# HeewoongNoh/DOSTransformer

Measured on AMD Instinct MI355X. Metric: crystals/sec training throughput (Phonon DOS, hidden=128), higher is better.
Workload: dtype f32; 1 GPU; phonon_h128_b64: phonon DOSTransformer layers=3 transformer=2 hidden=128, 64 crystals/GPU, full train step (fwd+loss+bwd+AdamW), 8 distinct pre-collated HBM-resident batches; global_batch=64, parallelism=dp1, launch=replay

## Files before the change

### dostransformer_amd/_lib.py

```python
from __future__ import annotations

import ctypes as C
import os
from typing import Optional

_HERE = os.path.dirname(os.path.abspath(__file__))


def from_environ(name: str, default: str = "") -> str:
    return os.environ.get(name, default)


LIB_PATH = from_environ("DOSX_LIB") or os.path.join(_HERE, "csrc", "libdosx.so")

c_float_p = C.POINTER(C.c_float)
c_int_p = C.POINTER(C.c_int32)
BIG = 1 << 30


class DosxUnavailable(RuntimeError):
    pass


class DosxError(RuntimeError):
# ... 61 lines not shown
        ("dkv_accumulate", C.c_int32),
        ("partials_q", C.c_void_p), ("partials_kv", C.c_void_p), ("drop_mask", C.c_void_p), ("dkv_part", C.c_void_p), ("dkv_cnt", C.c_void_p),
        ("ln1_gamma", C.c_void_p), ("ln1_beta", C.c_void_p), ("ln1_out", C.c_void_p),
        ("key_ptr", C.c_void_p),
    ]


class FfnBwd(C.Structure):
    _fields_ = [
        ("M", C.c_int32), ("H", C.c_int32),
        ("dy", C.c_void_p), ("lddy", C.c_int32),
        ("h", C.c_void_p), ("ldh", C.c_int32),
        ("x", C.c_void_p), ("ldx", C.c_int32),
        ("stats", C.c_void_p),
        ("gamma", C.c_void_p),
        ("w1", C.c_void_p), ("w2", C.c_void_p),
        ("dh", C.c_void_p), ("lddh", C.c_int32),
        ("dx", C.c_void_p), ("lddx", C.c_int32),
        ("partials", C.c_void_p), ("partial_ld", C.c_int32),
        ("fin_gamma", C.c_void_p), ("fin_xhat", C.c_void_p), ("fin_rstd", C.c_void_p),
        ("fin_dy", C.c_void_p),
        ("fin_ddos", C.c_void_p), ("fin_w", C.c_void_p), ("fin_beta", C.c_void_p),
        ("fin_S", C.c_int32), ("fin_Bq", C.c_int32),
        ("att_x", C.c_void_p), ("att_ldxin", C.c_int32),
        ("att_kvhat", C.c_void_p), ("att_gamma0", C.c_void_p), ("att_beta0", C.c_void_p),
        ("att_probs", C.c_void_p), ("att_qstats", C.c_void_p), ("att_mask", C.c_void_p),
        ("att_dxin", C.c_void_p), ("att_lddxin", C.c_int32),
        ("att_partials_q", C.c_void_p), ("att_partials_kv", C.c_void_p), ("att_dkv_part", C.c_void_p), ("att_dkv_cnt", C.c_void_p),
        ("att_dkvhat", C.c_void_p), ("att_dkv_accumulate", C.c_int32),
        ("att_Nk", C.c_int32), ("att_Bk", C.c_int32), ("att_Bq", C.c_int32), ("att_Sq", C.c_int32), ("att_qs", C.c_int32), ("att_qb", C.c_int32),
        ("att_key_ptr", C.c_void_p),
    ]


class Ffn(C.Structure):
    _fields_ = [
        ("M", C.c_int32), ("H", C.c_int32),
        ("x", C.c_void_p), ("ldx", C.c_int32),
        ("stats", C.c_void_p),
        ("gamma", C.c_void_p), ("beta", C.c_void_p),
        ("w1", C.c_void_p), ("b1", C.c_void_p),
        ("w2", C.c_void_p), ("b2", C.c_void_p),
        ("h", C.c_void_p), ("ldh", C.c_int32),
        ("out", C.c_void_p), ("ldo", C.c_int32),
        ("fin_gamma", C.c_void_p), ("fin_beta", C.c_void_p),
        ("fin_xhat", C.c_void_p), ("fin_rstd", C.c_void_p),
        ("fin_w", C.c_void_p), ("fin_b", C.c_void_p), ("fin_dos", C.c_void_p),
        ("fin_S", C.c_int32), ("fin_Bq", C.c_int32),
        ("att_kvhat", C.c_void_p), ("att_gamma0", C.c_void_p), ("att_beta0", C.c_void_p), ("att_mask", C.c_void_p),
        ("att_probs", C.c_void_p), ("att_qstats", C.c_void_p), ("att_x1", C.c_void_p), ("att_st1", C.c_void_p),
        ("att_Nk", C.c_int32), ("att_Bk", C.c_int32), ("att_Bq", C.c_int32), ("att_Sq", C.c_int32),
        ("att_qs", C.c_int32), ("att_qb", C.c_int32), ("att_ldx1", C.c_int32), ("att_aligned", C.c_int32),
        ("att_key_ptr", C.c_void_p),
    ]


class MlpLn(C.Structure):
    _fields_ = [
        ("M", C.c_int32), ("K", C.c_int32), ("NH", C.c_int32), ("NO", C.c_int32), ("k0", C.c_int32),
        ("a0", C.c_void_p), ("lda0", C.c_int32),
        ("a1", C.c_void_p), ("lda1", C.c_int32),
        ("w1", C.c_void_p), ("b1", C.c_void_p),
        ("gamma", C.c_void_p), ("beta", C.c_void_p),
        ("alpha", C.c_void_p),
        ("w2", C.c_void_p), ("b2", C.c_void_p),
        ("res", C.c_void_p), ("ldres", C.c_int32),
        ("xhat", C.c_void_p), ("rstd", C.c_void_p),
        ("out", C.c_void_p), ("ldo", C.c_int32),
        ("w3", C.c_void_p), ("ldw3", C.c_int32), ("n3", C.c_int32), ("nb3", C.c_int32),
        ("pq", C.c_void_p), ("ldpq", C.c_int32),
        ("cs_buf", C.c_void_p), ("cs_cnt", C.c_void_p),
    ]


class MlpLnBwd(C.Structure):
    _fields_ = [
        ("M", C.c_int32), ("K", C.c_int32), ("NH", C.c_int32), ("NO", C.c_int32),
        ("dy", C.c_void_p), ("lddy", C.c_int32),
        ("xhat", C.c_void_p), ("rstd", C.c_void_p),
        ("w1", C.c_void_p), ("w2", C.c_void_p),
        ("gamma", C.c_void_p), ("beta", C.c_void_p), ("alpha", C.c_void_p),
        ("dz", C.c_void_p),
        ("dcat", C.c_void_p), ("lddcat", C.c_int32),
        ("partials", C.c_void_p), ("partial_ld", C.c_int32), ("add_dy", C.c_int32),
        ("cs_buf", C.c_void_p), ("cs_cnt", C.c_void_p),
        ("pre", C.c_int32), ("pre_dy", C.c_void_p),
        ("pre_dz", C.c_void_p), ("pre_rowptr_src", C.c_void_p), ("pre_perm_src", C.c_void_p), ("pre_aggd", C.c_void_p),
        ("pre_w", C.c_void_p), ("pre_ldw", C.c_int32),
        ("pre_res", C.c_void_p), ("pre_ldres", C.c_int32), ("pre_res2", C.c_void_p), ("pre_ldres2", C.c_int32),
        ("pre_aggs", C.c_void_p),
        ("pre_dkv", C.c_void_p), ("pre_kvhat", C.c_void_p), ("pre_rstd_nodes", C.c_void_p), ("pre_dense_row", C.c_void_p),
        ("pre_dpool", C.c_void_p), ("pre_ld_dpool", C.c_int32), ("pre_node_graph", C.c_void_p), ("pre_num_graphs", C.c_int32),
        ("pre_ghost_row", C.c_int32),
    ]


class EncCs(C.Structure):
    _fields_ = [
        ("M", C.c_int32), ("Fa", C.c_int32), ("H", C.c_int32),
        ("x", C.c_void_p), ("ldx", C.c_int32),
        ("w0", C.c_void_p), ("ldw0", C.c_int32), ("b0", C.c_void_p),
        ("alpha", C.c_void_p),
        ("w2", C.c_void_p), ("b2", C.c_void_p),
        ("z", C.c_void_p), ("out", C.c_void_p), ("ldo", C.c_int32),
        ("w3", C.c_void_p), ("ldw3", C.c_int32), ("n3", C.c_int32), ("nb3", C.c_int32),
        ("pq", C.c_void_p), ("ldpq", C.c_int32),
# ... 139 lines not shown
    "dosx_gemm_kernel_name": [C.POINTER(Gemm), C.c_char_p, _I],
    "dosx_wgrad_splits": [_I, _I, _I],
    "dosx_wgrad_tiles": [_I, _I],
    "dosx_wgrad_scratch_floats": [_I, _I, _I],
    "dosx_wgrad": [C.POINTER(Wgrad), _P],
    "dosx_grad_flush": [C.POINTER(Wgrad), _I, C.POINTER(ReduceJob), _I, _P],
    "dosx_wgrad_grouped": [C.POINTER(Wgrad), _I, _P],
    "dosx_reduce_partials": [C.POINTER(ReduceJob), _I, _P],
    "dosx_edge_feat_sh1": [_P, _P, _I, _F, _P],
    "dosx_edge_embed_sh1": [_P, _P, _P, _P, _P, _I, _I, _F, _P],
    "dosx_segment_reduce": [_P, _P, _P, _P, _P, _P, _I, _I, _I, _P],
    "dosx_segment_reduce_perm": [_P, _P, _P, _P, _I, _I, _I, _P],
    "dosx_edge_grad_combine": [_P, _I, _P, _I, _P, _P, _P, _I, _I, _P],
    "dosx_gather_bwd": [_P, _P, _I, _P, _P, _P, _P, _P, _P, _P, _I, _I, _I, _P],
    "dosx_graph_pool": [_P, _P, _P, _I, _I, _I, _P],
    "dosx_graph_pool_bwd": [_P, _I, _P, _P, _I, _I, _I, _I, _P],
    "dosx_dense_normalize": [_P, _P, _P, _P, _I, _I, _I, _P],
    "dosx_dense_normalize_slots": [_P, _P, _P, _P, _I, _I, _I, _P],
    "dosx_dense_normalize_bwd": [_P, _P, _P, _P, _P, _I, _I, _I, _I, _P],
    "dosx_dense_normalize_pool_bwd": [_P, _P, _P, _P, _P, _I, _P, _I, _P, _I, _I, _I, _I, _P],
    "dosx_dense_slots": [_P, _P, _P, _I, _I, _I, _P],
    "dosx_dense_slots_bwd": [_P, _P, _P, _I, _I, _I, _I, _P],
    "dosx_ln_prelu_bwd": [_P, _P, _P, _P, _P, _P, _P, _P, _I, _I, _P],
    "dosx_ln_prelu_bwd_gather": [_P, _P, _P, _P, _P, _P, _P, _P, _P, _P, _I, _I, _P],
    "dosx_act_segment_sum": [_P, _P, _P, _P, _P, _P, _P, _P, _P, _I, _I, _I, _P],
    "dosx_seg_count_scale": [_P, _I, _P, _I, _P, _I, _I, _P],
    "dosx_gather_add_rownorm": [_P, _P, _I, _P, _I, _P, _P, _P, _P, _I, _I, _P],
    "dosx_rownorm": [_P, _P, _P, _I, _I, _P],
    "dosx_rownorm_bwd": [_P, _P, _P, _P, _I, _I, _I, _P],
    "dosx_mask_residual": [_P, _I, _P, _P, _I, _P, _I, _P, _I, _I, _P],
    "dosx_rownorm_bwd_act": [_P, _P, _P, _P, _P, _F, _P, _I, _I, _P],
    "dosx_layernorm": [_P, _P, _P, _P, _P, _P, _I, _I, _P],
    "dosx_layernorm_bwd": [_P, _P, _P, _P, _P, _P, _I, _I, _P],
    "dosx_attention_pkv_supported": [_I, _I],
    "dosx_attention_aligned_mode": [_I],
    "dosx_attention_fwd": [C.POINTER(Attn), _P],
    "dosx_attention_bwd": [C.POINTER(Attn), _P],
    "dosx_attn_pv": [_P, _P, _P, _P, _I, _I, _I, _I, _I, _P],
    "dosx_attn_tv": [_P, _P, _P, _P, _I, _I, _I, _I, _I, _I, _P],
    "dosx_attn_dp": [_P, _P, _P, _I, _I, _I, _I, _I, _P],
    "dosx_softmax_bwd": [_P, _P, _P, _P, _L, _I, _F, _P],
    "dosx_softmax_fwd": [_P, _P, _L, _I, _F, _P],
    "dosx_ln_rowdot": [_P, _P, _P, _P, _P, _P, _P, _P, _I, _I, _I, _P],
    "dosx_ln_rowdot_bwd": [_P, _P, _P, _P, _P, _P, _P, _P, _I, _I, _I, _P],
    "dosx_rowdot": [_P, _P, _P, _P, _I, _I, _I, _P],
    "dosx_rowdot_bwd": [_P, _P, _P, _P, _P, _I, _I, _I, _P],
    "dosx_sse2": [_P, _P, _P, _P, _I, _P],
    "dosx_loss_phonon_bwd": [_P, _P, _P, _P, _F, _D, _P, _P, _P, _I, _P],
    "dosx_loss_phonon": [_P, _P, _P, _P, _F, _P, _P, _P, _I, _P],
    "dosx_loss_edos": [_P, _P, _P, _F, _I, _I, _I, _P, _P, _P, _P],
    "dosx_sum": [_P, _I, _P, _P],
    "dosx_adamw": [_P, _P, _P, _P, _L, _F, _F, _F, _F, _F, _I, _F, _P],
    "dosx_ffn_supported": [_I],
    "dosx_ffn_att_supported": [_I, _I],
    "dosx_ffn_att_aligned_supported": [_I, _I],
    "dosx_ffn_fwd": [C.POINTER(Ffn), _P],
    "dosx_ffn_fwd_multi": [C.POINTER(Ffn), _I, _P],
    "dosx_ffn_bwd_partial_rows": [_I],
    "dosx_ffn_att_bwd_supported": [_I, _I, _I, _I],
    "dosx_ffn_att_bwd_partial_rows": [_I, _I],
    "dosx_ffn_att_aligned_rows": [_I, _I],
    "dosx_ffn_bwd": [C.POINTER(FfnBwd), _P],
    "dosx_mlp_ln_supported": [_I, _I, _I],
    "dosx_mlp_ln_cs_supported": [_I, _I, _I],
    "dosx_mlp_ln_cs_tiles": [_I],
    "dosx_mlp_ln_cs_scratch_floats": [_I, _I],
    "dosx_mlp_ln_fwd": [C.POINTER(MlpLn), _P],
    "dosx_mlp_ln_bwd_partial_rows": [_I],
    "dosx_mlp_ln_bwd": [C.POINTER(MlpLnBwd), _P],
    "dosx_enc_cs_supported": [_I, _I],
    "dosx_enc_cs_fwd": [C.POINTER(EncCs), _P],
    "dosx_edge_enc_supported": [_I],
    "dosx_edge_enc_fwd": [C.POINTER(EdgeEnc), _P],
    "dosx_heads_bwd_supported": [_I],
    "dosx_heads_bwd": [C.POINTER(HeadsBwd), _P],
    "dosx_gemm_bf16x3_supported": [_I, _I, _I],
    "dosx_gemm_bf16x3": [_P, _I, _P, _I, _I, _P, _P, _I, _I, _I, _I, _I, _P, _I, _P, _I, _P],
    "dosx_edge_mlp_supported": [_I],
    "dosx_edge_mlp_fwd": [C.POINTER(EdgeMlp), _P],
    "dosx_edge_mlp_bwd": [C.POINTER(EdgeMlpBwd), _P],
    "dosx_node_grad": [C.POINTER(NodeGrad), _P],
    "dosx_csr_workspace_bytes": [_I, C.POINTER(C.c_size_t)],
    "dosx_csr_build": [_P, _P, _I, _I, _I, _P, _P, _P, _P, _P, _P, _P, _P, _P, _P, _P, _P, C.c_size_t, _P],
    "dosx_collate": [_P] * 5 + [_I] * 3 + [_P] * 18 + [_P],
    "dosx_collate_padded": [C.POINTER(Collate), _P],
    "dosx_collate_padded_f64": [C.POINTER(Collate), _P],
    "dosx_neighbor_count": [_P, _P, _P, _P, _I, _L, _D, _I, _I, _P, _P],
    "dosx_neighbor_fill": [_P, _P, _P, _P, _I, _L, _D, _I, _I, _P, _P, _P, _P, _P, _P, _P],
    "dosx_knn_graph": [C.POINTER(Knn), _P],
    "dosx_replay_op": [C.c_char_p, C.POINTER(C.c_int), C.POINTER(C.c_int)],
    "dosx_replay": [C.POINTER(Call), _I, C.POINTER(C.c_int)],
    "dosx_replay_timed": [C.POINTER(Call), _I, C.POINTER(C.c_float), C.POINTER(C.c_int)],
    "dosx_dropout_mask": [_P, _L, _F, _P, _L, _P],
    "dosx_copy_many": [C.POINTER(CopyJob), _I, _P],
    "dosx_fill": [_P, _F, _L, _P],
    "dosx_embed_rows": [_P, _P, _P, _I, _I, _P],
    "dosx_embed_rows_bwd": [_P, _I, _P, _P, _I, _I, _I, _P],
    "dosx_reduce_rows": [_P, _I, _P, _I, _I, _I, _I, _I, _I, _I, _P],
    "dosx_act_bwd": [_P, _P, _F, _P, _L, _P],
    "dosx_gemm_f64": [C.POINTER(Gemm64), _P],
    "dosx_wgrad_f64": [C.POINTER(Wgrad64), _P],
    "dosx_colsum_f64": [_P, _I, _I, _I, _P, _P, _I, _P],
    "dosx_layernorm_f64": [_P, _P, _P, _P, _P, _P, _P, _I, _I, _P],
    "dosx_layernorm_bwd_f64": [_P, _P, _P, _P, _P, _P, _P, _P, _I, _I, _P],
    "dosx_act_bwd_f64": [_P, _P, _I, _I, _P, _P, _P, _I, _I, _P],
    "dosx_edge_feat_sh1_f64": [_P, _P, _I, _D, _P],
# ... 63 lines not shown
```

### dostransformer_amd/_models.py

```python
from __future__ import annotations

from typing import Optional, Tuple

import torch

from . import functional as Fn
from . import functional64 as F64
from ._fused import FusedModel, is_dead_param
from ._lib import DosxError


_SEED_MOD = 2 ** 62


def rank_seed_offset() -> int:
    import torch.distributed as td
    if td.is_available() and td.is_initialized():
        return (0x9E3779B97F4A7C15 * (td.get_rank() + 1)) % _SEED_MOD
    return 0


def dos_device(P):
    return P["embeddings.weight"].device

# ... 28 lines not shown
                            f"Predictor(model, per_crystal_keys=True) and Trainer(model, per_crystal_keys=True)")
        object.__setattr__(self, "_per_crystal_keys", bool(flag))
        return self

    def _check_f64_program(self) -> None:
        name = type(self).__name__
        if self._cfg.kind != "phonon":
            raise DosxError(f"{name}: only DOSTransformer_phonon has a float64 program (the eDOS reference trains in fp32)")
        dts = {p.dtype for n, p in self.named_parameters() if not is_dead_param(n)}
        if dts != {torch.float64}:
            raise DosxError(f"{name}: the float64 program needs every live parameter float64 (.double()), got "
                            f"{sorted(str(d) for d in dts)}")
        if self._cfg.H > F64.MAX_HIDDEN:
            raise DosxError(f"{name}: the float64 program takes hidden <= {F64.MAX_HIDDEN}, got {self._cfg.H}")

    def _flat_dtype(self, g=None) -> torch.dtype:
        if self._program_dtype != torch.float64:
            return torch.float32
        self._check_f64_program()
        return torch.float64

    def _wanted_flat_dtype(self):
        return self._program_dtype

    def _require_fp32_program(self, who: str) -> None:
        if self._program_dtype == torch.float64:
            raise DosxError(f"{who} runs the fp32 program; {type(self).__name__} is set to float64 (set_program_dtype): train "
                            f"it with train64.Trainer64, or with model(batch), loss.backward() and torch.optim.AdamW")

    def _require_f64_program(self, who: str) -> None:
        ours = isinstance(self, DOSTransformerBase)
        if not (ours and self._cfg.kind == "phonon" and self._program_dtype == torch.float64):
            raise DosxError(f"{who} drives a DOSTransformer_phonon set to the float64 program "
                            f"(model.double().set_program_dtype(torch.float64)), got {type(self).__name__}"
                            + (f" with program_dtype {self._program_dtype}" if ours else "")
                            + ": the fp32 program is train.Trainer's / predict.Predictor's")

    def _check_train_flags(self):
        pass

    def _dropout(self, device, bump: bool):
        p = float(getattr(self, "_attn_drop", 0.0) or 0.0)
        if not self.training or p <= 0.0:
            return None
        seed = getattr(self, "_drop_seed", None)
        if seed is None or seed.device != device:
            val = (int(torch.randint(0, _SEED_MOD, (1,), dtype=torch.int64).item()) + rank_seed_offset()) % _SEED_MOD
            seed = torch.tensor([val], dtype=torch.int64).to(device)
            object.__setattr__(self, "_drop_seed", seed)
        elif bump:
            seed.add_(1)
        return p, seed

    def _program_fwd(self, P, g, m, bump_seed: bool = True, per_crystal_keys: bool = False):
        if P["embeddings.weight"].dtype == torch.float64:
            dos, xL, ctx = F64.dostransformer_phonon_fwd(P, self._cfg, g, m, drop=self._dropout(dos_device(P), bump_seed),
                                                         per_crystal_keys=self._per_crystal_keys)
            B = m.num_graphs
            return dos[:B], xL, dos[B:], (ctx, dos)
        dos, xL, ctx = Fn.dostransformer_fwd(P, self._cfg, g, m, drop=self._dropout(dos_device(P), bump_seed),
                                             per_crystal_keys=per_crystal_keys)
        B = m.num_graphs
        return dos[:B], xL, dos[B:], (ctx, dos)

    def _program_bwd(self, P, G, m, saved, grads, sink):
        ctx, dos = saved
        dg, dx, ds = grads
        B = m.num_graphs
        ddos = torch.zeros_like(dos)
        if dg is not None:
            ddos[:B].copy_(dg)
        if ds is not None:
            ddos[B:].copy_(ds)
        if dos.dtype == torch.float64:
            F64.dostransformer_phonon_bwd(P, G, self._cfg, m, ctx, ddos, dx)
            return
        Fn.dostransformer_bwd(P, G, self._cfg, m, ctx, ddos, None if dx is None else dx.float().contiguous(), sink)

    def forward(self, g):
        self._check_train_flags()
        return self._run(g)


class GraphnetworkBase(FusedModel):
    _cfg: Fn.ModelCfg
    _returns_x: bool
    _has_f64_program = True

    def _extra_dead(self, g) -> Tuple[str, ...]:
        expected = 118 if self._cfg.kind == "phonon" else 200
        width = g.x.shape[1] if g is not None else expected
        unused = "GN_encoder.node_encoder_prompt" if width == expected else "GN_encoder.node_encoder"
        return tuple(f"{unused}.{s}" for s in ("0.weight", "0.bias", "1.weight", "2.weight", "2.bias"))

    def _program_fwd(self, P, g, m):
        if P["embeddings.weight"].dtype == torch.float64:
            dos, ctx = F64.graphnetwork_phonon_fwd(P, self._cfg, g, m)
            return dos, ctx
        dos, xL, ctx = Fn.graphnetwork_fwd(P, self._cfg, g, m)
        return (dos, xL, ctx) if self._returns_x else (dos, ctx)

    def _program_bwd(self, P, G, m, saved, grads, sink):
        ddos = grads[0]
        if P["embeddings.weight"].dtype == torch.float64:
            if ddos is None:
                ddos = torch.zeros(m.num_graphs, self._cfg.S, device=P["embeddings.weight"].device, dtype=torch.float64)
            F64.graphnetwork_phonon_bwd(P, G, self._cfg, m, saved, ddos)
            return
        dx = grads[1] if self._returns_x else None
        if ddos is None:
            ddos = torch.zeros(m.num_graphs, self._cfg.S, device=P["embeddings.weight"].device)
        Fn.graphnetwork_bwd(P, G, self._cfg, m, saved, ddos.float().contiguous(),
                            None if dx is None else dx.float().contiguous(), sink)

# ... 4 lines not shown
```

### dostransformer_amd/csrc/common.h

```cpp
#pragma once
#include <hip/hip_runtime.h>
#include <stdint.h>
#include <stdio.h>

#include "../../include/dosx.h"

typedef float f32x16 __attribute__((ext_vector_type(16)));
typedef float f32x4 __attribute__((ext_vector_type(4)));

#define DOSX_WAVE 64

#ifndef DOSX_MAIN_PRIO
#define DOSX_MAIN_PRIO 0
#endif
#define DOSX_SET_MAIN_PRIO() do { if (DOSX_MAIN_PRIO) __builtin_amdgcn_s_setprio(DOSX_MAIN_PRIO); } while (0)

void dosx_set_error(const char* fmt, ...);

#define DOSX_CHECK_ARG(cond, ...)   \
  do {                              \
    if (!(cond)) {                  \
      dosx_set_error(__VA_ARGS__);  \
      return -22;                   \
    }                               \
// ... 65 lines not shown
  __device__ __forceinline__ explicit UDiv(int d_) : d(d_), sh((d_ & (d_ - 1)) == 0 ? __builtin_ctz(d_) : -1) {}
  __device__ __forceinline__ int div(int x) const { return sh >= 0 ? (x >> sh) : x / d; }
};

__device__ __forceinline__ float4 ld4(const float* p) { return *reinterpret_cast<const float4*>(p); }
__device__ __forceinline__ void st4(float* p, float4 v) { *reinterpret_cast<float4*>(p) = v; }
__device__ __forceinline__ float4 f4zero() { return make_float4(0.f, 0.f, 0.f, 0.f); }
__device__ __forceinline__ float4 f4add(float4 a, float4 b) {
  return make_float4(a.x + b.x, a.y + b.y, a.z + b.z, a.w + b.w);
}
__device__ __forceinline__ float f4get(const float4& v, int i) {
  return i == 0 ? v.x : i == 1 ? v.y : i == 2 ? v.z : v.w;
}

template <bool KP>
__device__ __forceinline__ int dosx_live_keys(const int32_t* key_ptr, int bk, int Nk) {
  if constexpr (KP) return min(max(key_ptr[bk + 1] - key_ptr[bk], 0), Nk);
  else return Nk;
}
template <bool KP>
__device__ __forceinline__ int dosx_live_keys_fwd(const int32_t* key_ptr, int bk, int Nk) {
  if constexpr (KP) return min(max(key_ptr[bk + 1] - key_ptr[bk], 0), Nk);
  else return key_ptr ? min(key_ptr[bk + 1] - key_ptr[bk], Nk) : Nk;
}
template <bool KP>
__device__ __forceinline__ float dosx_key_entry(const float* base, size_t row0, int j, int nk, int Nk, float other) {
  if constexpr (KP) return j < nk ? base[row0 + j] : other;
  else return base[row0 + (j < Nk ? j : 0)];
}
template <bool KP>
__device__ __forceinline__ float dosx_softmax_inv(float s) {
  if constexpr (KP) return s > 0.f ? 1.f / s : 0.f;
  else return 1.f / s;
}
template <bool KP, int SH>
__device__ __forceinline__ int dosx_live_tiles(int nk, int all) {
  if constexpr (KP) return (nk + (1 << SH) - 1) >> SH;
  else return all;
}
template <bool KP>
__device__ __forceinline__ float dosx_psum_one(int nk) {
  if constexpr (KP) return nk > 0 ? 1.f : 0.f;
  else return 1.f;
}

#define DOSX_LN_EPS 1e-5f

#ifndef DOSX_TICKET_ORDER
#define DOSX_TICKET_ORDER __ATOMIC_RELAXED
#endif
__device__ __forceinline__ int dosx_ticket(int* counter) {
  return __hip_atomic_fetch_add(counter, 1, DOSX_TICKET_ORDER, __HIP_MEMORY_SCOPE_AGENT);
}
```

### dostransformer_amd/csrc/ffn.hip

```cpp
#include <stdlib.h>

#include "common.h"
#include "mma16.h"

typedef int v4i32 __attribute__((ext_vector_type(4)));

#ifdef DOSX_STAMPS
__device__ unsigned long long dosx_ffn_stamp_buf[64];
extern "C" int dosx_debug_read_ffn_stamps(unsigned long long* host64) {
  return (int)hipMemcpyFromSymbol(host64, HIP_SYMBOL(dosx_ffn_stamp_buf), sizeof(unsigned long long) * 64);
}
#define FSTAMP(slot) do { if (threadIdx.x == 0 && blockIdx.x == 0) dosx_ffn_stamp_buf[(slot)] = __builtin_amdgcn_s_memtime(); } while (0)
#define FSTAMP_S(slot) do { if (threadIdx.x == 256 && blockIdx.x == 0) dosx_ffn_stamp_buf[32 + (slot)] = __builtin_amdgcn_s_memtime(); } while (0)
#else
#define FSTAMP(slot) do { } while (0)
#define FSTAMP_S(slot) do { } while (0)
#endif

namespace {

constexpr int FBN = 128;

template <bool KP>
__device__ __forceinline__ void ffn_att_row(const DosxFfn& a, float* __restrict__ Xs, const int LDX, const int lr, const int m0,
// ... 249 lines not shown
  FSTAMP(13);
  __syncthreads();
  {
    const int nct = H >> 4, njobs = (R / 16) * nct;
    const UDiv dnct(nct);
    for (int job = wave; job < njobs; job += 8) {
      const int rt = dnct.div(job), ct = job - rt * nct;
      const f32x4 acc = mma_kn<4>(Sc + (16 * rt + l15) * 68 + 4 * g4, Ks + (4 * g4) * LDK + 16 * ct + l15, LDK, nctL);
#pragma unroll
      for (int i = 0; i < 4; ++i) Qs[(16 * rt + 4 * g4 + i) * LDK + 16 * ct + l15] = acc[i];
    }
  }
  FSTAMP(14);
  __syncthreads();
  FSTAMP(15);
  if (rowok) {
    float4 x1[2];
    float t = 0.f;
#pragma unroll
    for (int k = 0; k < 2; ++k) {
      const int c = q16 * 4 + 64 * k;
      x1[k] = f4zero();
      if (!on[k]) continue;
      const float4 o = ld4(Qs + lr * LDK + c);
      x1[k] = make_float4(o.x * g0[k].x + b0[k].x * psum + xr[k].x, o.y * g0[k].y + b0[k].y * psum + xr[k].y,
                          o.z * g0[k].z + b0[k].z * psum + xr[k].z, o.w * g0[k].w + b0[k].w * psum + xr[k].w);
      if (rv) st4(a.att_x1 + (size_t)r * a.att_ldx1 + c, x1[k]);
      t += (x1[k].x + x1[k].y) + (x1[k].z + x1[k].w);
    }
    const float mean1 = row16_sum(t) * invH;
    t = 0.f;
#pragma unroll
    for (int k = 0; k < 2; ++k) {
      if (!on[k]) continue;
      const float p0 = x1[k].x - mean1, p1 = x1[k].y - mean1, p2 = x1[k].z - mean1, p3 = x1[k].w - mean1;
      t += (p0 * p0 + p1 * p1) + (p2 * p2 + p3 * p3);
    }
    const float rstd1 = rsqrtf(row16_sum(t) * invH + DOSX_LN_EPS);
    if (rv && q16 == 0) {
      a.att_qstats[2 * (size_t)r] = mean; a.att_qstats[2 * (size_t)r + 1] = rstd;
      a.att_st1[2 * (size_t)r] = mean1;   a.att_st1[2 * (size_t)r + 1] = rstd1;
    }
#pragma unroll
    for (int k = 0; k < 2; ++k) {
      if (!on[k]) continue;
      const float4 vv = x1[k];
      st4(Xs + lr * LDX + q16 * 4 + 64 * k,
          make_float4((vv.x - mean1) * rstd1 * g1[k].x + bb1[k].x, (vv.y - mean1) * rstd1 * g1[k].y + bb1[k].y,
                      (vv.z - mean1) * rstd1 * g1[k].z + bb1[k].z, (vv.w - mean1) * rstd1 * g1[k].w + bb1[k].w));
    }
  }
}

template <bool HALF, int KB, int ATTK>
__device__ __forceinline__ void ffn_fwd_body(const DosxFfn& a, float* __restrict__ sm) {
  constexpr int ATT = ATTK >= 3 ? ATTK - 2 : ATTK;
  constexpr bool KP = ATTK >= 3;
  constexpr int FBK = KB, FLDW = KB + 4;
  constexpr int R = HALF ? 16 : 32;
  constexpr int ER = R / 8;
  const int H = a.H, H4 = 4 * a.H, M = a.M;
  const int LDX = H + 4, LDT = H4 + 4;
  float* Xs = sm;
  float* T = Xs + R * LDX;
  float* ST = T + R * LDT;
  constexpr int STG = FBN * FLDW;
  const int tid = threadIdx.x, lane = tid & 63, wave = tid >> 6, l31 = lane & 31, hh = lane >> 5;
  const int l15 = lane & 15, g4 = lane >> 4;
  const int wave_u = __builtin_amdgcn_readfirstlane(wave);
  const int m0 = blockIdx.x * R;
  int al_bq = 0, al_s0 = 0;
  if constexpr (ATT == 2) {
    const int tpc = (a.att_Sq + R - 1) / R;
    al_bq = (int)blockIdx.x / tpc;
    al_s0 = ((int)blockIdx.x % tpc) * R;
  }
  auto grow = [&](const int lr) -> int {
    if constexpr (ATT == 2) {
      const int s = al_s0 + lr;
      return s < a.att_Sq ? s * a.att_Bq + al_bq : -1;
    } else {
      const int r = m0 + lr;
      return r < M ? r : -1;
    }
  };
  auto growc = [&](const int lr) -> int {
    const int r = grow(lr);
    return r >= 0 ? r : grow(0);
  };
  FSTAMP(0);
  const int nk1 = H / FBK, nb1 = H4 / FBN, n1 = nb1 * nk1, n2 = H4 / FBK, nch = n1 + n2;

  const int c0 = lane * 4;
  const bool con = c0 < H;
  float4 xres[ER], bias2 = f4zero();
  if (con) bias2 = ld4(a.b2 + c0);
  if constexpr (ATT == 0) {
#pragma unroll
    for (int i = 0; i < ER; ++i) {
      const int r = growc(wave * ER + i);
      xres[i] = ld4(a.x + (size_t)r * a.ldx + (con ? c0 : 0));
    }
  }
  if constexpr (ATT == 2) {
  }
  float* const attKs = ST;
  float* const attSc = ST + ((a.att_Nk + 15) & ~15) * (H + 4);
// ... 191 lines not shown
    FSTAMP(4);
    float* Cs = ST;
    const int col = wave * 32 + l31;
#pragma unroll
    for (int r = 0; r < 16; ++r) Cs[((r & 3) + 8 * (r >> 2) + 4 * hh) * (FBN + 4) + col] = acc[r];
    }
  }
  __syncthreads();
  FSTAMP(5);
  if constexpr (ATT != 0) {
#pragma unroll
    for (int i = 0; i < ER; ++i) {
      const int r = growc(wave * ER + i);
      xres[i] = ld4(a.att_x1 + (size_t)r * a.att_ldx1 + (con ? c0 : 0));
    }
  }
  {
    const float* Cs = ST;
    const bool fin = a.fin_gamma != nullptr;
    const bool fdot = fin && a.fin_dos != nullptr;
    float4 fg = f4zero(), fb = f4zero(), fw = f4zero();
    if (fin && con) { fg = ld4(a.fin_gamma + c0); fb = ld4(a.fin_beta + c0); }
    if (fdot && con) fw = ld4(a.fin_w + c0);
    const float fbias = fdot ? a.fin_b[0] : 0.f;
    const float invH = 1.f / (float)H;
#pragma unroll
    for (int i = 0; i < ER; ++i) {
      const int lr = wave * ER + i, r = grow(lr);
      const bool ok = con && r >= 0;
      float4 o = f4zero();
      if (ok) {
        const float4 v = ld4(Cs + lr * (FBN + 4) + c0);
        o = make_float4(v.x + bias2.x + xres[i].x, v.y + bias2.y + xres[i].y, v.z + bias2.z + xres[i].z,
                        v.w + bias2.w + xres[i].w);
      }
      if (!fin) {
        if (ok) st4(a.out + (size_t)r * a.ldo + c0, o);
        continue;
      }
      const float mean = wave_sum(o.x + o.y + o.z + o.w) * invH;
      const float4 d = ok ? make_float4(o.x - mean, o.y - mean, o.z - mean, o.w - mean) : f4zero();
      const float rstd = rsqrtf(wave_sum(d.x * d.x + d.y * d.y + d.z * d.z + d.w * d.w) * invH + DOSX_LN_EPS);
      float dot = 0.f;
      if (ok) {
        const float4 xh = make_float4(d.x * rstd, d.y * rstd, d.z * rstd, d.w * rstd);
        const float4 y = make_float4(xh.x * fg.x + fb.x, xh.y * fg.y + fb.y, xh.z * fg.z + fb.z, xh.w * fg.w + fb.w);
        st4(a.fin_xhat + (size_t)r * H + c0, xh);
        if (a.out) st4(a.out + (size_t)r * a.ldo + c0, y);
        if (lane == 0) a.fin_rstd[r] = rstd;
        dot = y.x * fw.x + y.y * fw.y + y.z * fw.z + y.w * fw.w;
      }
      if (fdot) {
        dot = wave_sum(dot);
        if (lane == 0 && r >= 0) a.fin_dos[(size_t)(r % a.fin_Bq) * a.fin_S + (r / a.fin_Bq)] = dot + fbias;
      }
    }
  }
  FSTAMP(6);
}

template <bool HALF, int KB, int ATT>
__global__ __launch_bounds__(512) void ffn_fwd_kernel(const DosxFfn a) {
  DOSX_SET_MAIN_PRIO();
  extern __shared__ __align__(16) float sm[];
  ffn_fwd_body<HALF, KB, ATT>(a, sm);
}

constexpr int FFN_MULTI_MAX = 2;
struct FfnMulti {
  DosxFfn d[FFN_MULTI_MAX];
  int n;
};
template <bool HALF, int KB, int ATT>
__global__ __launch_bounds__(512) void ffn_fwd_multi_kernel(const FfnMulti A) {
  DOSX_SET_MAIN_PRIO();
  extern __shared__ __align__(16) float sm[];
  ffn_fwd_body<HALF, KB, ATT>(A.d[0], sm);
  asm volatile("s_waitcnt vmcnt(0)" ::: "memory");
  __syncthreads();
  ffn_fwd_body<HALF, KB, ATT>(A.d[1], sm);
}


struct AttBwdSm {
  float *Os, *Ds, *Ql, *Sp, *Ks, *Sc, *Ss, *Ps2, *Pp;
};

template <bool KP>
__device__ __forceinline__ void ffn_dkv_reduce(const DosxFfnBwd& a, const int nqt, const int bk, float* __restrict__ Pp, const int tid) {
  const int lane = tid & 63, q16 = lane & 15, slot = tid >> 4;
  const int H = a.H, Nk = a.att_Nk, rep = a.att_Bq / a.att_Bk, ngroups = (Nk + 15) / 16;
  const int nk = dosx_live_keys<KP>(a.att_key_ptr, bk, Nk);
  const int np = (KP && slot >= nk) ? 0 : rep * nqt;
  const UDiv dnqt(nqt);
  const size_t pstride = (size_t)Nk * H;
  const __amdgpu_buffer_rsrc_t rP = __builtin_amdgcn_make_buffer_rsrc((void*)a.att_dkv_part, 0, 0x7fffffff, 0x00020000);
  float4 g0[2], d[2][2], kh[2][2], d0[2][2];
  bool jv[2];
  size_t krow[2];
#pragma unroll
  for (int k = 0; k < 2; ++k) g0[k] = ld4(a.att_gamma0 + ((q16 * 4 + 64 * k) < H ? (q16 * 4 + 64 * k) : 0));
#pragma unroll
  for (int p = 0; p < 2; ++p) {
    const int j = slot + 32 * p;
    jv[p] = j < nk;
    krow[p] = ((size_t)(jv[p] ? j : 0) * a.att_Bk + bk) * H;
#pragma unroll
    for (int k = 0; k < 2; ++k) {
      const int c = q16 * 4 + 64 * k, cc = c < H ? c : 0;
      kh[p][k] = (!KP || jv[p]) ? ld4(a.att_kvhat + krow[p] + cc) : f4zero();
      d0[p][k] = (a.att_dkv_accumulate && (!KP || jv[p])) ? ld4(a.att_dkvhat + krow[p] + cc) : f4zero();
      d[p][k] = f4zero();
    }
  }
  for (int p0 = 0; p0 < np; p0 += 4) {
    float4 v[2][4][2];
#pragma unroll
    for (int p = 0; p < 2; ++p)
#pragma unroll
      for (int u = 0; u < 4; ++u) {
        const int pi = min(p0 + u, np - 1), i = dnqt.div(pi), t = pi - i * nqt;
        const size_t off = ((size_t)(bk + i * a.att_Bk) * nqt + t) * pstride + (size_t)(jv[p] ? slot + 32 * p : 0) * H;
#pragma unroll
        for (int k = 0; k < 2; ++k) {
          const int c = q16 * 4 + 64 * k;
          v[p][u][k] = (KP && !jv[p]) ? f4zero()
                                      : __builtin_bit_cast(float4, __builtin_amdgcn_raw_buffer_load_b128(rP, (uint32_t)((off + (c < H ? c : 0)) * 4), 0, 16));
        }
      }
#pragma unroll
    for (int p = 0; p < 2; ++p)
#pragma unroll
      for (int u = 0; u < 4; ++u)
// ... 608 lines not shown
      float s = 0.f;
#pragma unroll
      for (int w = 0; w < 8; ++w) s += Ps[(w * npv + which) * FBN + col];
      prow[which * H + col] = s;
    }
    if (fdot && tid == 0) {
      float s = 0.f;
#pragma unroll
      for (int w = 0; w < 8; ++w) s += Ps[8 * 5 * FBN + w];
      prow[5 * H] = s;
    }
  }
  if constexpr (ATT == 2) {
    __syncthreads();
    AttBwdSm L;
    const int LDK = H + 4, NkP = (a.att_Nk + 15) & ~15;
    L.Os = sm;
    L.Ds = sm + R * LDK;
    L.Ql = L.Ds + R * LDK;
    L.Sc = L.Ql + R * LDK;
    L.Ss = L.Sc + R * 68;
    L.Ps2 = L.Ss + R * 68;
    L.Sp = L.Ps2 + R * 68;
    L.Ks = L.Sp + 3 * R * 68;
    L.Pp = L.Sp;
    (void)NkP;
    FSTAMP(16);
    ffn_att_bwd_tile<R, KP>(a, sm, L, attq, al_s0, al_bq, al_tile, al_tpc, tid);
    FSTAMP(29);
  }
}

}

static size_t ffn_att_bwd_floats(int H, int Nk, int R) {
  const size_t LDK = (size_t)H + 4, NkP = (size_t)((Nk + 15) & ~15);
  const size_t tiles = 3 * R * LDK + 6 * (size_t)R * 68 + NkP * LDK;
  const size_t pp = 3 * R * LDK + 3 * (size_t)R * 68 + 32 * 256;
  const size_t red = 64 * 256;
  size_t m = tiles > pp ? tiles : pp;
  return m > red ? m : red;
}

static int ffn_bwd_att_rows(int Sq, int Bq);

static int ffn_chunk(int H) {
  static int forced = -1;
  if (forced < 0) { const char* e = getenv("DOSX_FFN_KB"); forced = e ? atoi(e) : 0; }
  if (forced == 32) return 32;
  return (H % 64) == 0 ? 64 : 32;
}

extern "C" int dosx_ffn_supported(int H) { return (H % 32) == 0 && H >= 32 && H <= 128; }
extern "C" int dosx_ffn_att_supported(int H, int Nk) { return dosx_ffn_supported(H) && Nk >= 1 && Nk <= 16; }
extern "C" int dosx_ffn_att_aligned_supported(int H, int Nk) {
  if (!dosx_ffn_supported(H) || Nk < 1 || Nk > 64) return 0;
  const int kb = ffn_chunk(H);
  return (size_t)((Nk + 15) & ~15) * (H + 4) + 32 * 68 <= 2 * (size_t)128 * (kb + 4);
}

struct FfnPlan { bool half; int kb, mode, grid; size_t smem; };
static int ffn_fwd_prepare(const DosxFfn& a, FfnPlan& pl) {
  DOSX_CHECK_ARG(dosx_ffn_supported(a.H), "dosx_ffn_fwd: H=%d unsupported (multiple of 32, <= 128)", a.H);
  const bool att = a.att_kvhat != nullptr;
  DOSX_CHECK_ARG(a.x && (a.stats || att) && a.gamma && a.beta && a.w1 && a.b1 && a.w2 && a.b2 && a.h && (a.out || a.fin_dos), "dosx_ffn_fwd: null operand");
  if (att)
    DOSX_CHECK_ARG((a.att_aligned ? dosx_ffn_att_aligned_supported(a.H, a.att_Nk) : dosx_ffn_att_supported(a.H, a.att_Nk)) && a.att_gamma0 && a.att_beta0 && a.att_probs && a.att_qstats && a.att_x1 &&
                       a.att_st1 && a.att_Bk > 0 && a.att_Bq > 0 && a.att_Bq % a.att_Bk == 0 && a.att_Sq > 0 &&
                       a.att_Sq * a.att_Bq == a.M && (a.att_ldx1 & 3) == 0 && a.att_ldx1 >= a.H && a.att_qs >= 0 && a.att_qb >= 0,
                   "dosx_ffn_fwd: fused attention needs <= 16 keys, gamma0 / beta0 / probs / qstats / x1 / st1 and Sq * Bq == M");
  if (a.fin_dos) DOSX_CHECK_ARG(a.fin_gamma && a.fin_w && a.fin_b && a.fin_S > 0 && a.fin_Bq > 0 && a.fin_S * a.fin_Bq == a.M,
                                "dosx_ffn_fwd: output-layer epilogue needs the final LayerNorm, w, b and S * Bq == M");
  DOSX_CHECK_ARG((a.ldx & 3) == 0 && (a.ldh & 3) == 0 && (a.ldo & 3) == 0, "dosx_ffn_fwd: leading dimensions must be multiples of 4");
  if (a.fin_gamma) DOSX_CHECK_ARG(a.fin_beta && a.fin_xhat && a.fin_rstd, "dosx_ffn_fwd: final LayerNorm needs beta / xhat / rstd");
  const long long span = (const char*)a.w1 > (const char*)a.w2 ? (const char*)a.w1 - (const char*)a.w2 : (const char*)a.w2 - (const char*)a.w1;
  DOSX_CHECK_ARG(span + (long long)16 * a.H * a.H < 0x7fffffffLL, "dosx_ffn_fwd: fc1 / fc2 weights more than 2 GiB apart");
  const int H = a.H, H4 = 4 * H;
  static int half_max = -1;
  if (half_max < 0) { const char* e = getenv("DOSX_FFN_HALF_MAX"); half_max = e ? atoi(e) : 128; }
  const bool aligned = att && a.att_aligned != 0;
  pl.half = aligned ? ffn_bwd_att_rows(a.att_Sq, a.att_Bq) == 16 : ceil_div(a.M, 32) <= half_max;
  const int R = pl.half ? 16 : 32;
  pl.kb = ffn_chunk(H);
  pl.mode = aligned ? 2 : (att ? 1 : 0);
  if (att && a.att_key_ptr) pl.mode += 2;
  pl.smem = sizeof(float) * ((size_t)R * (H + 4) + (size_t)R * (H4 + 4) + 2 * (size_t)FBN * (pl.kb + 4));
  if (aligned)
    DOSX_CHECK_ARG(a.att_Nk <= 64 && ((size_t)((a.att_Nk + 15) & ~15) * (H + 4) + (size_t)R * 68) <= 2 * (size_t)FBN * (pl.kb + 4),
                   "dosx_ffn_fwd: crystal-aligned attention needs <= 64 keys that fit the stage buffers (Nk=%d, H=%d)", a.att_Nk, H);
  pl.grid = aligned ? a.att_Bq * ceil_div(a.att_Sq, R) : ceil_div(a.M, R);
  static bool attr_set = false;
  if (!attr_set) {
#define DOSX_FFN_ATTR(HALF_, KB_, ATT_) \
    (void)hipFuncSetAttribute(reinterpret_cast<const void*>(&ffn_fwd_kernel<HALF_, KB_, ATT_>), hipFuncAttributeMaxDynamicSharedMemorySize, 160 * 1024)
#define DOSX_FFN_ATTR2(HALF_, KB_, ATT_) \
    (void)hipFuncSetAttribute(reinterpret_cast<const void*>(&ffn_fwd_multi_kernel<HALF_, KB_, ATT_>), hipFuncAttributeMaxDynamicSharedMemorySize, 160 * 1024)
    DOSX_FFN_ATTR(false, 32, 0); DOSX_FFN_ATTR(true, 32, 0); DOSX_FFN_ATTR(false, 64, 0); DOSX_FFN_ATTR(true, 64, 0);
    DOSX_FFN_ATTR(false, 32, 1); DOSX_FFN_ATTR(true, 32, 1); DOSX_FFN_ATTR(false, 64, 1); DOSX_FFN_ATTR(true, 64, 1);
    DOSX_FFN_ATTR(false, 32, 2); DOSX_FFN_ATTR(true, 32, 2); DOSX_FFN_ATTR(false, 64, 2); DOSX_FFN_ATTR(true, 64, 2);
    DOSX_FFN_ATTR2(false, 32, 1); DOSX_FFN_ATTR2(true, 32, 1); DOSX_FFN_ATTR2(false, 64, 1); DOSX_FFN_ATTR2(true, 64, 1);
    DOSX_FFN_ATTR2(false, 32, 2); DOSX_FFN_ATTR2(true, 32, 2); DOSX_FFN_ATTR2(false, 64, 2); DOSX_FFN_ATTR2(true, 64, 2);
    DOSX_FFN_ATTR(false, 32, 3); DOSX_FFN_ATTR(true, 32, 3); DOSX_FFN_ATTR(false, 64, 3); DOSX_FFN_ATTR(true, 64, 3);
    DOSX_FFN_ATTR(false, 32, 4); DOSX_FFN_ATTR(true, 32, 4); DOSX_FFN_ATTR(false, 64, 4); DOSX_FFN_ATTR(true, 64, 4);
    DOSX_FFN_ATTR2(false, 32, 3); DOSX_FFN_ATTR2(true, 32, 3); DOSX_FFN_ATTR2(false, 64, 3); DOSX_FFN_ATTR2(true, 64, 3);
    DOSX_FFN_ATTR2(false, 32, 4); DOSX_FFN_ATTR2(true, 32, 4); DOSX_FFN_ATTR2(false, 64, 4); DOSX_FFN_ATTR2(true, 64, 4);
#undef DOSX_FFN_ATTR
#undef DOSX_FFN_ATTR2
    attr_set = true;
  }
  return 0;
}

#define DOSX_FFN_DISPATCH(KERNEL, ARG)                                                                                    \
  do {                                                                                                                     \
    const dim3 grid_(pl.grid);                                                                                             \
    hipStream_t st_ = to_stream(stream);                                                                                   \
    if (pl.half && pl.kb == 64) { if (pl.mode == 4) hipLaunchKernelGGL((KERNEL<true, 64, 4>), grid_, dim3(512), pl.smem, st_, ARG); else if (pl.mode == 3) hipLaunchKernelGGL((KERNEL<true, 64, 3>), grid_, dim3(512), pl.smem, st_, ARG); else if (pl.mode == 2) hipLaunchKernelGGL((KERNEL<true, 64, 2>), grid_, dim3(512), pl.smem, st_, ARG); else if (pl.mode == 1) hipLaunchKernelGGL((KERNEL<true, 64, 1>), grid_, dim3(512), pl.smem, st_, ARG); else hipLaunchKernelGGL((KERNEL<true, 64, 0>), grid_, dim3(512), pl.smem, st_, ARG); } \
    else if (pl.half) { if (pl.mode == 4) hipLaunchKernelGGL((KERNEL<true, 32, 4>), grid_, dim3(512), pl.smem, st_, ARG); else if (pl.mode == 3) hipLaunchKernelGGL((KERNEL<true, 32, 3>), grid_, dim3(512), pl.smem, st_, ARG); else if (pl.mode == 2) hipLaunchKernelGGL((KERNEL<true, 32, 2>), grid_, dim3(512), pl.smem, st_, ARG); else if (pl.mode == 1) hipLaunchKernelGGL((KERNEL<true, 32, 1>), grid_, dim3(512), pl.smem, st_, ARG); else hipLaunchKernelGGL((KERNEL<true, 32, 0>), grid_, dim3(512), pl.smem, st_, ARG); } \
    else if (pl.kb == 64) { if (pl.mode == 4) hipLaunchKernelGGL((KERNEL<false, 64, 4>), grid_, dim3(512), pl.smem, st_, ARG); else if (pl.mode == 3) hipLaunchKernelGGL((KERNEL<false, 64, 3>), grid_, dim3(512), pl.smem, st_, ARG); else if (pl.mode == 2) hipLaunchKernelGGL((KERNEL<false, 64, 2>), grid_, dim3(512), pl.smem, st_, ARG); else if (pl.mode == 1) hipLaunchKernelGGL((KERNEL<false, 64, 1>), grid_, dim3(512), pl.smem, st_, ARG); else hipLaunchKernelGGL((KERNEL<false, 64, 0>), grid_, dim3(512), pl.smem, st_, ARG); } \
    else { if (pl.mode == 4) hipLaunchKernelGGL((KERNEL<false, 32, 4>), grid_, dim3(512), pl.smem, st_, ARG); else if (pl.mode == 3) hipLaunchKernelGGL((KERNEL<false, 32, 3>), grid_, dim3(512), pl.smem, st_, ARG); else if (pl.mode == 2) hipLaunchKernelGGL((KERNEL<false, 32, 2>), grid_, dim3(512), pl.smem, st_, ARG); else if (pl.mode == 1) hipLaunchKernelGGL((KERNEL<false, 32, 1>), grid_, dim3(512), pl.smem, st_, ARG); else hipLaunchKernelGGL((KERNEL<false, 32, 0>), grid_, dim3(512), pl.smem, st_, ARG); } \
  } while (0)

extern "C" int dosx_ffn_fwd(const DosxFfn* ap, dosx_stream_t stream) {
  DOSX_CHECK_ARG(ap != nullptr, "dosx_ffn_fwd: null descriptor");
  const DosxFfn& a = *ap;
  if (a.M <= 0) return 0;
  FfnPlan pl;
  if (int rc = ffn_fwd_prepare(a, pl)) return rc;
  DOSX_FFN_DISPATCH(ffn_fwd_kernel, a);
  DOSX_LAUNCH_CHECK();
  return 0;
}

extern "C" int dosx_ffn_fwd_multi(const DosxFfn* descs, int n, dosx_stream_t stream) {
  DOSX_CHECK_ARG(descs != nullptr && n >= 1 && n <= FFN_MULTI_MAX, "dosx_ffn_fwd_multi: 1 .. %d layers per launch", FFN_MULTI_MAX);
  if (descs[0].M <= 0) return 0;
  if (n == 1) return dosx_ffn_fwd(descs, stream);
  FfnMulti A;
  A.n = n;
  FfnPlan pl;
  for (int l = 0; l < n; ++l) {
    FfnPlan p2;
    if (int rc = ffn_fwd_prepare(descs[l], p2)) return rc;
    if (l == 0) pl = p2;
    DOSX_CHECK_ARG(p2.half == pl.half && p2.kb == pl.kb && p2.mode == pl.mode && p2.grid == pl.grid && p2.smem == pl.smem && descs[l].M == descs[0].M,
                   "dosx_ffn_fwd_multi: layer %d has another launch plan than layer 0", l);
    DOSX_CHECK_ARG(p2.mode != 0, "dosx_ffn_fwd_multi: every layer must carry its attention half (row-local layers only)");
    if (l > 0) {
      const DosxFfn& p = descs[l - 1];
      const DosxFfn& c = descs[l];
      DOSX_CHECK_ARG(p.out != nullptr && c.x == p.out && c.ldx == p.ldo && c.att_qs == c.att_Bq && c.att_qb == 1,
                     "dosx_ffn_fwd_multi: layer %d must read layer %d's output rows (dense query rows)", l, l - 1);
    }
    A.d[l] = descs[l];
  }
  {
    const dim3 grid_(pl.grid);
    hipStream_t st_ = to_stream(stream);
#define DOSX_FFN_GO2(HALF_, KB_) \
    do { if (pl.mode == 4) hipLaunchKernelGGL((ffn_fwd_multi_kernel<HALF_, KB_, 4>), grid_, dim3(512), pl.smem, st_, A); \
         else if (pl.mode == 3) hipLaunchKernelGGL((ffn_fwd_multi_kernel<HALF_, KB_, 3>), grid_, dim3(512), pl.smem, st_, A); \
         else if (pl.mode == 2) hipLaunchKernelGGL((ffn_fwd_multi_kernel<HALF_, KB_, 2>), grid_, dim3(512), pl.smem, st_, A); \
         else hipLaunchKernelGGL((ffn_fwd_multi_kernel<HALF_, KB_, 1>), grid_, dim3(512), pl.smem, st_, A); } while (0)
    if (pl.half && pl.kb == 64) DOSX_FFN_GO2(true, 64);
    else if (pl.half) DOSX_FFN_GO2(true, 32);
    else if (pl.kb == 64) DOSX_FFN_GO2(false, 64);
    else DOSX_FFN_GO2(false, 32);
#undef DOSX_FFN_GO2
  }
  DOSX_LAUNCH_CHECK();
  return 0;
}

static int ffn_bwd_half(int M) {
  static int half_max = -1;
  if (half_max < 0) { const char* e = getenv("DOSX_FFN_HALF_MAX"); half_max = e ? atoi(e) : 128; }
  return ceil_div(M, 32) <= half_max;
}

extern "C" int dosx_ffn_bwd_partial_rows(int M) { return M <= 0 ? 0 : ceil_div(M, ffn_bwd_half(M) ? 16 : 32); }

static int ffn_bwd_att_rows(int Sq, int Bq) {
  static int half_max = -1;
  if (half_max < 0) { const char* e = getenv("DOSX_FFN_HALF_MAX"); half_max = e ? atoi(e) : 128; }
  return Bq * ceil_div(Sq, 32) <= half_max ? 16 : 32;
}
extern "C" int dosx_ffn_att_bwd_supported(int H, int Nk, int Sq, int Bq) {
  if (!dosx_ffn_supported(H) || ffn_chunk(H) != 64 || Nk < 1 || Nk > 64 || Sq < 1 || Bq < 1) return 0;
  const int R = ffn_bwd_att_rows(Sq, Bq);
  const size_t ffn = (size_t)R * (H + 4) + (size_t)R * (4 * H + 4) + 2 * (size_t)64 * (FBN + 4);
  const size_t att = ffn_att_bwd_floats(H, Nk, R);
  return (ffn > att ? ffn : att) * sizeof(float) <= 160 * 1024;
}
extern "C" int dosx_ffn_att_bwd_partial_rows(int Sq, int Bq) { return Bq * ceil_div(Sq, ffn_bwd_att_rows(Sq, Bq)); }
extern "C" int dosx_ffn_att_aligned_rows(int Sq, int Bq) { return (Sq < 1 || Bq < 1) ? 0 : ffn_bwd_att_rows(Sq, Bq); }

extern "C" int dosx_ffn_bwd(const DosxFfnBwd* ap, dosx_stream_t stream) {
  DOSX_CHECK_ARG(ap != nullptr, "dosx_ffn_bwd: null descriptor");
  const DosxFfnBwd& a = *ap;
  if (a.M <= 0) return 0;
  DOSX_CHECK_ARG(dosx_ffn_supported(a.H), "dosx_ffn_bwd: H=%d unsupported (multiple of 32, <= 128)", a.H);
  DOSX_CHECK_ARG((a.dy || a.fin_ddos) && a.h && a.x && a.stats && a.gamma && a.w1 && a.w2 && a.dh && (a.dx || a.att_kvhat) && a.partials, "dosx_ffn_bwd: null operand");
  DOSX_CHECK_ARG((a.lddy & 3) == 0 && (a.ldh & 3) == 0 && (a.ldx & 3) == 0 && (a.lddh & 3) == 0 && (a.lddx & 3) == 0,
                 "dosx_ffn_bwd: leading dimensions must be multiples of 4");
  const int npv = a.fin_gamma ? (a.fin_ddos ? 5 : 4) : 2;
  DOSX_CHECK_ARG(a.partial_ld >= npv * a.H + (a.fin_ddos ? 1 : 0), "dosx_ffn_bwd: partial_ld %d too small for %d column groups", a.partial_ld, npv);
  if (a.fin_gamma) DOSX_CHECK_ARG(a.fin_xhat && a.fin_rstd && a.fin_dy, "dosx_ffn_bwd: final LayerNorm backward needs xhat / rstd / fin_dy");
  if (a.fin_ddos) DOSX_CHECK_ARG(a.fin_gamma && a.fin_beta && a.fin_w && a.fin_S > 0 && a.fin_Bq > 0 && a.fin_S * a.fin_Bq == a.M,
                                 "dosx_ffn_bwd: output-layer backward needs gamma / beta / w and S * Bq == M");
  const long long span = (const char*)a.w1 > (const char*)a.w2 ? (const char*)a.w1 - (const char*)a.w2 : (const char*)a.w2 - (const char*)a.w1;
  DOSX_CHECK_ARG(span + (long long)16 * a.H * a.H < 0x7fffffffLL, "dosx_ffn_bwd: fc1 / fc2 weights more than 2 GiB apart");
  const int H = a.H, H4 = 4 * H;
  const bool att = a.att_kvhat != nullptr;
  if (att) {
    DOSX_CHECK_ARG(dosx_ffn_att_bwd_supported(H, a.att_Nk, a.att_Sq, a.att_Bq) && ffn_chunk(H) == 64, "dosx_ffn_bwd: fused attention backward unsupported for H=%d Nk=%d", H, a.att_Nk);
    DOSX_CHECK_ARG(a.att_x && a.att_gamma0 && a.att_beta0 && a.att_probs && a.att_qstats && a.att_dxin && a.att_partials_q && a.att_partials_kv &&
                       a.att_dkv_part && a.att_dkv_cnt && a.att_dkvhat && a.att_Bk > 0 && a.att_Bq % a.att_Bk == 0 && a.att_Sq * a.att_Bq == a.M &&
// ... 34 lines not shown
```

### dostransformer_amd/csrc/replay_thunks.inc

```

static int thunk_dosx_set_sliver_max_gf(const DosxCall& c) { return dosx_set_sliver_max_gf((double)c.farg[0]); }
static int thunk_dosx_gemm_partial_rows(const DosxCall& c) { return dosx_gemm_partial_rows((int)c.iarg[0], (int)c.iarg[1], (int)c.iarg[2]); }
static int thunk_dosx_gemm(const DosxCall& c) { return dosx_gemm((const DosxGemm*)(uintptr_t)c.iarg[0], (dosx_stream_t)(uintptr_t)c.iarg[1]); }
static int thunk_dosx_gemm_pair(const DosxCall& c) { return dosx_gemm_pair((const DosxGemm*)(uintptr_t)c.iarg[0], (const DosxGemm*)(uintptr_t)c.iarg[1], (dosx_stream_t)(uintptr_t)c.iarg[2]); }
static int thunk_dosx_gemm_kernel_name(const DosxCall& c) { return dosx_gemm_kernel_name((const DosxGemm*)(uintptr_t)c.iarg[0], (char*)(uintptr_t)c.iarg[1], (int)c.iarg[2]); }
static int thunk_dosx_wgrad_splits(const DosxCall& c) { return dosx_wgrad_splits((int)c.iarg[0], (int)c.iarg[1], (int)c.iarg[2]); }
static int thunk_dosx_wgrad_tiles(const DosxCall& c) { return dosx_wgrad_tiles((int)c.iarg[0], (int)c.iarg[1]); }
static int thunk_dosx_wgrad(const DosxCall& c) { return dosx_wgrad((const DosxWgrad*)(uintptr_t)c.iarg[0], (dosx_stream_t)(uintptr_t)c.iarg[1]); }
static int thunk_dosx_wgrad_grouped(const DosxCall& c) { return dosx_wgrad_grouped((const DosxWgrad*)(uintptr_t)c.iarg[0], (int)c.iarg[1], (dosx_stream_t)(uintptr_t)c.iarg[2]); }
static int thunk_dosx_reduce_partials(const DosxCall& c) { return dosx_reduce_partials((const DosxReduceJob*)(uintptr_t)c.iarg[0], (int)c.iarg[1], (dosx_stream_t)(uintptr_t)c.iarg[2]); }
static int thunk_dosx_grad_flush(const DosxCall& c) { return dosx_grad_flush((const DosxWgrad*)(uintptr_t)c.iarg[0], (int)c.iarg[1], (const DosxReduceJob*)(uintptr_t)c.iarg[2], (int)c.iarg[3], (dosx_stream_t)(uintptr_t)c.iarg[4]); }
static int thunk_dosx_edge_feat_sh1(const DosxCall& c) { return dosx_edge_feat_sh1((const float*)(uintptr_t)c.iarg[0], (float*)(uintptr_t)c.iarg[1], (int)c.iarg[2], (float)c.farg[0], (dosx_stream_t)(uintptr_t)c.iarg[3]); }
static int thunk_dosx_edge_embed_sh1(const DosxCall& c) { return dosx_edge_embed_sh1((const float*)(uintptr_t)c.iarg[0], (const float*)(uintptr_t)c.iarg[1], (const float*)(uintptr_t)c.iarg[2], (float*)(uintptr_t)c.iarg[3], (float*)(uintptr_t)c.iarg[4], (int)c.iarg[5], (int)c.iarg[6], (float)c.farg[0], (dosx_stream_t)(uintptr_t)c.iarg[7]); }
static int thunk_dosx_segment_reduce(const DosxCall& c) { return dosx_segment_reduce((const float*)(uintptr_t)c.iarg[0], (const int32_t*)(uintptr_t)c.iarg[1], (const float*)(uintptr_t)c.iarg[2], (float*)(uintptr_t)c.iarg[3], (const float*)(uintptr_t)c.iarg[4], (float*)(uintptr_t)c.iarg[5], (int)c.iarg[6], (int)c.iarg[7], (int)c.iarg[8], (dosx_stream_t)(uintptr_t)c.iarg[9]); }
static int thunk_dosx_segment_reduce_perm(const DosxCall& c) { return dosx_segment_reduce_perm((const float*)(uintptr_t)c.iarg[0], (const int32_t*)(uintptr_t)c.iarg[1], (const int32_t*)(uintptr_t)c.iarg[2], (float*)(uintptr_t)c.iarg[3], (int)c.iarg[4], (int)c.iarg[5], (int)c.iarg[6], (dosx_stream_t)(uintptr_t)c.iarg[7]); }
static int thunk_dosx_act_segment_sum(const DosxCall& c) { return dosx_act_segment_sum((const float*)(uintptr_t)c.iarg[0], (const int32_t*)(uintptr_t)c.iarg[1], (const float*)(uintptr_t)c.iarg[2], (const float*)(uintptr_t)c.iarg[3], (const float*)(uintptr_t)c.iarg[4], (const float*)(uintptr_t)c.iarg[5], (const float*)(uintptr_t)c.iarg[6], (float*)(uintptr_t)c.iarg[7], (float*)(uintptr_t)c.iarg[8], (int)c.iarg[9], (int)c.iarg[10], (int)c.iarg[11], (dosx_stream_t)(uintptr_t)c.iarg[12]); }
static int thunk_dosx_seg_count_scale(const DosxCall& c) { return dosx_seg_count_scale((const float*)(uintptr_t)c.iarg[0], (int)c.iarg[1], (const int32_t*)(uintptr_t)c.iarg[2], (int)c.iarg[3], (float*)(uintptr_t)c.iarg[4], (int)c.iarg[5], (int)c.iarg[6], (dosx_stream_t)(uintptr_t)c.iarg[7]); }
static int thunk_dosx_edge_grad_combine(const DosxCall& c) { return dosx_edge_grad_combine((const float*)(uintptr_t)c.iarg[0], (int)c.iarg[1], (const float*)(uintptr_t)c.iarg[2], (int)c.iarg[3], (const int32_t*)(uintptr_t)c.iarg[4], (const float*)(uintptr_t)c.iarg[5], (float*)(uintptr_t)c.iarg[6], (int)c.iarg[7], (int)c.iarg[8], (dosx_stream_t)(uintptr_t)c.iarg[9]); }
static int thunk_dosx_gather_bwd(const DosxCall& c) { return dosx_gather_bwd((const float*)(uintptr_t)c.iarg[0], (const float*)(uintptr_t)c.iarg[1], (int)c.iarg[2], (const float*)(uintptr_t)c.iarg[3], (const int32_t*)(uintptr_t)c.iarg[4], (const int32_t*)(uintptr_t)c.iarg[5], (const int32_t*)(uintptr_t)c.iarg[6], (const float*)(uintptr_t)c.iarg[7], (float*)(uintptr_t)c.iarg[8], (float*)(uintptr_t)c.iarg[9], (int)c.iarg[10], (int)c.iarg[11], (int)c.iarg[12], (dosx_stream_t)(uintptr_t)c.iarg[13]); }
static int thunk_dosx_graph_pool(const DosxCall& c) { return dosx_graph_pool((const float*)(uintptr_t)c.iarg[0], (const int32_t*)(uintptr_t)c.iarg[1], (float*)(uintptr_t)c.iarg[2], (int)c.iarg[3], (int)c.iarg[4], (int)c.iarg[5], (dosx_stream_t)(uintptr_t)c.iarg[6]); }
static int thunk_dosx_graph_pool_bwd(const DosxCall& c) { return dosx_graph_pool_bwd((const float*)(uintptr_t)c.iarg[0], (int)c.iarg[1], (const int32_t*)(uintptr_t)c.iarg[2], (float*)(uintptr_t)c.iarg[3], (int)c.iarg[4], (int)c.iarg[5], (int)c.iarg[6], (int)c.iarg[7], (dosx_stream_t)(uintptr_t)c.iarg[8]); }
static int thunk_dosx_dense_normalize(const DosxCall& c) { return dosx_dense_normalize((const float*)(uintptr_t)c.iarg[0], (const int32_t*)(uintptr_t)c.iarg[1], (float*)(uintptr_t)c.iarg[2], (float*)(uintptr_t)c.iarg[3], (int)c.iarg[4], (int)c.iarg[5], (int)c.iarg[6], (dosx_stream_t)(uintptr_t)c.iarg[7]); }
static int thunk_dosx_dense_normalize_slots(const DosxCall& c) { return dosx_dense_normalize_slots((const float*)(uintptr_t)c.iarg[0], (const int32_t*)(uintptr_t)c.iarg[1], (float*)(uintptr_t)c.iarg[2], (float*)(uintptr_t)c.iarg[3], (int)c.iarg[4], (int)c.iarg[5], (int)c.iarg[6], (dosx_stream_t)(uintptr_t)c.iarg[7]); }
static int thunk_dosx_dense_normalize_bwd(const DosxCall& c) { return dosx_dense_normalize_bwd((const float*)(uintptr_t)c.iarg[0], (const float*)(uintptr_t)c.iarg[1], (const float*)(uintptr_t)c.iarg[2], (const int32_t*)(uintptr_t)c.iarg[3], (float*)(uintptr_t)c.iarg[4], (int)c.iarg[5], (int)c.iarg[6], (int)c.iarg[7], (int)c.iarg[8], (dosx_stream_t)(uintptr_t)c.iarg[9]); }
static int thunk_dosx_dense_normalize_pool_bwd(const DosxCall& c) { return dosx_dense_normalize_pool_bwd((const float*)(uintptr_t)c.iarg[0], (const float*)(uintptr_t)c.iarg[1], (const float*)(uintptr_t)c.iarg[2], (const int32_t*)(uintptr_t)c.iarg[3], (const float*)(uintptr_t)c.iarg[4], (int)c.iarg[5], (const int32_t*)(uintptr_t)c.iarg[6], (int)c.iarg[7], (float*)(uintptr_t)c.iarg[8], (int)c.iarg[9], (int)c.iarg[10], (int)c.iarg[11], (int)c.iarg[12], (dosx_stream_t)(uintptr_t)c.iarg[13]); }
static int thunk_dosx_dense_slots(const DosxCall& c) { return dosx_dense_slots((const float*)(uintptr_t)c.iarg[0], (const int32_t*)(uintptr_t)c.iarg[1], (float*)(uintptr_t)c.iarg[2], (int)c.iarg[3], (int)c.iarg[4], (int)c.iarg[5], (dosx_stream_t)(uintptr_t)c.iarg[6]); }
static int thunk_dosx_dense_slots_bwd(const DosxCall& c) { return dosx_dense_slots_bwd((const float*)(uintptr_t)c.iarg[0], (const int32_t*)(uintptr_t)c.iarg[1], (float*)(uintptr_t)c.iarg[2], (int)c.iarg[3], (int)c.iarg[4], (int)c.iarg[5], (int)c.iarg[6], (dosx_stream_t)(uintptr_t)c.iarg[7]); }
static int thunk_dosx_gather_add_rownorm(const DosxCall& c) { return dosx_gather_add_rownorm((const float*)(uintptr_t)c.iarg[0], (const float*)(uintptr_t)c.iarg[1], (int)c.iarg[2], (const float*)(uintptr_t)c.iarg[3], (int)c.iarg[4], (const int32_t*)(uintptr_t)c.iarg[5], (const int32_t*)(uintptr_t)c.iarg[6], (float*)(uintptr_t)c.iarg[7], (float*)(uintptr_t)c.iarg[8], (int)c.iarg[9], (int)c.iarg[10], (dosx_stream_t)(uintptr_t)c.iarg[11]); }
static int thunk_dosx_rownorm(const DosxCall& c) { return dosx_rownorm((const float*)(uintptr_t)c.iarg[0], (float*)(uintptr_t)c.iarg[1], (float*)(uintptr_t)c.iarg[2], (int)c.iarg[3], (int)c.iarg[4], (dosx_stream_t)(uintptr_t)c.iarg[5]); }
static int thunk_dosx_rownorm_bwd(const DosxCall& c) { return dosx_rownorm_bwd((const float*)(uintptr_t)c.iarg[0], (const float*)(uintptr_t)c.iarg[1], (const float*)(uintptr_t)c.iarg[2], (float*)(uintptr_t)c.iarg[3], (int)c.iarg[4], (int)c.iarg[5], (int)c.iarg[6], (dosx_stream_t)(uintptr_t)c.iarg[7]); }
static int thunk_dosx_mask_residual(const DosxCall& c) { return dosx_mask_residual((const float*)(uintptr_t)c.iarg[0], (int)c.iarg[1], (const float*)(uintptr_t)c.iarg[2], (const float*)(uintptr_t)c.iarg[3], (int)c.iarg[4], (float*)(uintptr_t)c.iarg[5], (int)c.iarg[6], (float*)(uintptr_t)c.iarg[7], (int)c.iarg[8], (int)c.iarg[9], (dosx_stream_t)(uintptr_t)c.iarg[10]); }
static int thunk_dosx_rownorm_bwd_act(const DosxCall& c) { return dosx_rownorm_bwd_act((const float*)(uintptr_t)c.iarg[0], (const float*)(uintptr_t)c.iarg[1], (const float*)(uintptr_t)c.iarg[2], (const float*)(uintptr_t)c.iarg[3], (const float*)(uintptr_t)c.iarg[4], (float)c.farg[0], (float*)(uintptr_t)c.iarg[5], (int)c.iarg[6], (int)c.iarg[7], (dosx_stream_t)(uintptr_t)c.iarg[8]); }
static int thunk_dosx_layernorm(const DosxCall& c) { return dosx_layernorm((const float*)(uintptr_t)c.iarg[0], (const float*)(uintptr_t)c.iarg[1], (const float*)(uintptr_t)c.iarg[2], (float*)(uintptr_t)c.iarg[3], (float*)(uintptr_t)c.iarg[4], (float*)(uintptr_t)c.iarg[5], (int)c.iarg[6], (int)c.iarg[7], (dosx_stream_t)(uintptr_t)c.iarg[8]); }
static int thunk_dosx_ln_prelu_bwd(const DosxCall& c) { return dosx_ln_prelu_bwd((const float*)(uintptr_t)c.iarg[0], (const float*)(uintptr_t)c.iarg[1], (const float*)(uintptr_t)c.iarg[2], (const float*)(uintptr_t)c.iarg[3], (const float*)(uintptr_t)c.iarg[4], (const float*)(uintptr_t)c.iarg[5], (float*)(uintptr_t)c.iarg[6], (float*)(uintptr_t)c.iarg[7], (int)c.iarg[8], (int)c.iarg[9], (dosx_stream_t)(uintptr_t)c.iarg[10]); }
static int thunk_dosx_ln_prelu_bwd_gather(const DosxCall& c) { return dosx_ln_prelu_bwd_gather((const float*)(uintptr_t)c.iarg[0], (const int32_t*)(uintptr_t)c.iarg[1], (const float*)(uintptr_t)c.iarg[2], (const float*)(uintptr_t)c.iarg[3], (const float*)(uintptr_t)c.iarg[4], (const float*)(uintptr_t)c.iarg[5], (const float*)(uintptr_t)c.iarg[6], (const float*)(uintptr_t)c.iarg[7], (float*)(uintptr_t)c.iarg[8], (float*)(uintptr_t)c.iarg[9], (int)c.iarg[10], (int)c.iarg[11], (dosx_stream_t)(uintptr_t)c.iarg[12]); }
static int thunk_dosx_layernorm_bwd(const DosxCall& c) { return dosx_layernorm_bwd((const float*)(uintptr_t)c.iarg[0], (const float*)(uintptr_t)c.iarg[1], (const float*)(uintptr_t)c.iarg[2], (const float*)(uintptr_t)c.iarg[3], (float*)(uintptr_t)c.iarg[4], (float*)(uintptr_t)c.iarg[5], (int)c.iarg[6], (int)c.iarg[7], (dosx_stream_t)(uintptr_t)c.iarg[8]); }
static int thunk_dosx_attention_pkv_supported(const DosxCall& c) { return dosx_attention_pkv_supported((int)c.iarg[0], (int)c.iarg[1]); }
static int thunk_dosx_attention_aligned_mode(const DosxCall& c) { return dosx_attention_aligned_mode((int)c.iarg[0]); }
static int thunk_dosx_attention_fwd(const DosxCall& c) { return dosx_attention_fwd((const DosxAttn*)(uintptr_t)c.iarg[0], (dosx_stream_t)(uintptr_t)c.iarg[1]); }
static int thunk_dosx_attention_bwd(const DosxCall& c) { return dosx_attention_bwd((const DosxAttn*)(uintptr_t)c.iarg[0], (dosx_stream_t)(uintptr_t)c.iarg[1]); }
static int thunk_dosx_attn_pv(const DosxCall& c) { return dosx_attn_pv((const float*)(uintptr_t)c.iarg[0], (const float*)(uintptr_t)c.iarg[1], (const float*)(uintptr_t)c.iarg[2], (float*)(uintptr_t)c.iarg[3], (int)c.iarg[4], (int)c.iarg[5], (int)c.iarg[6], (int)c.iarg[7], (int)c.iarg[8], (dosx_stream_t)(uintptr_t)c.iarg[9]); }
static int thunk_dosx_attn_tv(const DosxCall& c) { return dosx_attn_tv((const float*)(uintptr_t)c.iarg[0], (const float*)(uintptr_t)c.iarg[1], (const float*)(uintptr_t)c.iarg[2], (float*)(uintptr_t)c.iarg[3], (int)c.iarg[4], (int)c.iarg[5], (int)c.iarg[6], (int)c.iarg[7], (int)c.iarg[8], (int)c.iarg[9], (dosx_stream_t)(uintptr_t)c.iarg[10]); }
static int thunk_dosx_attn_dp(const DosxCall& c) { return dosx_attn_dp((const float*)(uintptr_t)c.iarg[0], (const float*)(uintptr_t)c.iarg[1], (float*)(uintptr_t)c.iarg[2], (int)c.iarg[3], (int)c.iarg[4], (int)c.iarg[5], (int)c.iarg[6], (int)c.iarg[7], (dosx_stream_t)(uintptr_t)c.iarg[8]); }
static int thunk_dosx_softmax_bwd(const DosxCall& c) { return dosx_softmax_bwd((const float*)(uintptr_t)c.iarg[0], (const float*)(uintptr_t)c.iarg[1], (const float*)(uintptr_t)c.iarg[2], (float*)(uintptr_t)c.iarg[3], (long long)c.iarg[4], (int)c.iarg[5], (float)c.farg[0], (dosx_stream_t)(uintptr_t)c.iarg[6]); }
static int thunk_dosx_softmax_fwd(const DosxCall& c) { return dosx_softmax_fwd((const float*)(uintptr_t)c.iarg[0], (float*)(uintptr_t)c.iarg[1], (long long)c.iarg[2], (int)c.iarg[3], (float)c.farg[0], (dosx_stream_t)(uintptr_t)c.iarg[4]); }
static int thunk_dosx_ln_rowdot(const DosxCall& c) { return dosx_ln_rowdot((const float*)(uintptr_t)c.iarg[0], (const float*)(uintptr_t)c.iarg[1], (const float*)(uintptr_t)c.iarg[2], (const float*)(uintptr_t)c.iarg[3], (const float*)(uintptr_t)c.iarg[4], (float*)(uintptr_t)c.iarg[5], (float*)(uintptr_t)c.iarg[6], (float*)(uintptr_t)c.iarg[7], (int)c.iarg[8], (int)c.iarg[9], (int)c.iarg[10], (dosx_stream_t)(uintptr_t)c.iarg[11]); }
static int thunk_dosx_ln_rowdot_bwd(const DosxCall& c) { return dosx_ln_rowdot_bwd((const float*)(uintptr_t)c.iarg[0], (const float*)(uintptr_t)c.iarg[1], (const float*)(uintptr_t)c.iarg[2], (const float*)(uintptr_t)c.iarg[3], (const float*)(uintptr_t)c.iarg[4], (const float*)(uintptr_t)c.iarg[5], (float*)(uintptr_t)c.iarg[6], (float*)(uintptr_t)c.iarg[7], (int)c.iarg[8], (int)c.iarg[9], (int)c.iarg[10], (dosx_stream_t)(uintptr_t)c.iarg[11]); }
static int thunk_dosx_rowdot(const DosxCall& c) { return dosx_rowdot((const float*)(uintptr_t)c.iarg[0], (const float*)(uintptr_t)c.iarg[1], (const float*)(uintptr_t)c.iarg[2], (float*)(uintptr_t)c.iarg[3], (int)c.iarg[4], (int)c.iarg[5], (int)c.iarg[6], (dosx_stream_t)(uintptr_t)c.iarg[7]); }
static int thunk_dosx_rowdot_bwd(const DosxCall& c) { return dosx_rowdot_bwd((const float*)(uintptr_t)c.iarg[0], (const float*)(uintptr_t)c.iarg[1], (const float*)(uintptr_t)c.iarg[2], (float*)(uintptr_t)c.iarg[3], (float*)(uintptr_t)c.iarg[4], (int)c.iarg[5], (int)c.iarg[6], (int)c.iarg[7], (dosx_stream_t)(uintptr_t)c.iarg[8]); }
static int thunk_dosx_sse2(const DosxCall& c) { return dosx_sse2((const float*)(uintptr_t)c.iarg[0], (const float*)(uintptr_t)c.iarg[1], (const float*)(uintptr_t)c.iarg[2], (float*)(uintptr_t)c.iarg[3], (int)c.iarg[4], (dosx_stream_t)(uintptr_t)c.iarg[5]); }
static int thunk_dosx_loss_phonon_bwd(const DosxCall& c) { return dosx_loss_phonon_bwd((const float*)(uintptr_t)c.iarg[0], (const float*)(uintptr_t)c.iarg[1], (const float*)(uintptr_t)c.iarg[2], (const float*)(uintptr_t)c.iarg[3], (float)c.farg[0], (double)c.farg[1], (float*)(uintptr_t)c.iarg[4], (float*)(uintptr_t)c.iarg[5], (float*)(uintptr_t)c.iarg[6], (int)c.iarg[7], (dosx_stream_t)(uintptr_t)c.iarg[8]); }
static int thunk_dosx_loss_phonon(const DosxCall& c) { return dosx_loss_phonon((const float*)(uintptr_t)c.iarg[0], (const float*)(uintptr_t)c.iarg[1], (const float*)(uintptr_t)c.iarg[2], (float*)(uintptr_t)c.iarg[3], (float)c.farg[0], (float*)(uintptr_t)c.iarg[4], (float*)(uintptr_t)c.iarg[5], (float*)(uintptr_t)c.iarg[6], (int)c.iarg[7], (dosx_stream_t)(uintptr_t)c.iarg[8]); }
static int thunk_dosx_loss_edos(const DosxCall& c) { return dosx_loss_edos((const float*)(uintptr_t)c.iarg[0], (const float*)(uintptr_t)c.iarg[1], (const float*)(uintptr_t)c.iarg[2], (float)c.farg[0], (int)c.iarg[3], (int)c.iarg[4], (int)c.iarg[5], (float*)(uintptr_t)c.iarg[6], (float*)(uintptr_t)c.iarg[7], (float*)(uintptr_t)c.iarg[8], (dosx_stream_t)(uintptr_t)c.iarg[9]); }
static int thunk_dosx_sum(const DosxCall& c) { return dosx_sum((const float*)(uintptr_t)c.iarg[0], (int)c.iarg[1], (float*)(uintptr_t)c.iarg[2], (dosx_stream_t)(uintptr_t)c.iarg[3]); }
static int thunk_dosx_adamw(const DosxCall& c) { return dosx_adamw((float*)(uintptr_t)c.iarg[0], (const float*)(uintptr_t)c.iarg[1], (float*)(uintptr_t)c.iarg[2], (float*)(uintptr_t)c.iarg[3], (int64_t)c.iarg[4], (float)c.farg[0], (float)c.farg[1], (float)c.farg[2], (float)c.farg[3], (float)c.farg[4], (int)c.iarg[5], (float)c.farg[5], (dosx_stream_t)(uintptr_t)c.iarg[6]); }
static int thunk_dosx_ffn_supported(const DosxCall& c) { return dosx_ffn_supported((int)c.iarg[0]); }
static int thunk_dosx_ffn_att_supported(const DosxCall& c) { return dosx_ffn_att_supported((int)c.iarg[0], (int)c.iarg[1]); }
static int thunk_dosx_ffn_att_aligned_supported(const DosxCall& c) { return dosx_ffn_att_aligned_supported((int)c.iarg[0], (int)c.iarg[1]); }
static int thunk_dosx_ffn_fwd(const DosxCall& c) { return dosx_ffn_fwd((const DosxFfn*)(uintptr_t)c.iarg[0], (dosx_stream_t)(uintptr_t)c.iarg[1]); }
static int thunk_dosx_ffn_fwd_multi(const DosxCall& c) { return dosx_ffn_fwd_multi((const DosxFfn*)(uintptr_t)c.iarg[0], (int)c.iarg[1], (dosx_stream_t)(uintptr_t)c.iarg[2]); }
static int thunk_dosx_ffn_bwd_partial_rows(const DosxCall& c) { return dosx_ffn_bwd_partial_rows((int)c.iarg[0]); }
static int thunk_dosx_ffn_att_bwd_supported(const DosxCall& c) { return dosx_ffn_att_bwd_supported((int)c.iarg[0], (int)c.iarg[1], (int)c.iarg[2], (int)c.iarg[3]); }
static int thunk_dosx_ffn_att_bwd_partial_rows(const DosxCall& c) { return dosx_ffn_att_bwd_partial_rows((int)c.iarg[0], (int)c.iarg[1]); }
static int thunk_dosx_ffn_att_aligned_rows(const DosxCall& c) { return dosx_ffn_att_aligned_rows((int)c.iarg[0], (int)c.iarg[1]); }
static int thunk_dosx_ffn_bwd(const DosxCall& c) { return dosx_ffn_bwd((const DosxFfnBwd*)(uintptr_t)c.iarg[0], (dosx_stream_t)(uintptr_t)c.iarg[1]); }
static int thunk_dosx_edge_enc_supported(const DosxCall& c) { return dosx_edge_enc_supported((int)c.iarg[0]); }
static int thunk_dosx_edge_enc_fwd(const DosxCall& c) { return dosx_edge_enc_fwd((const DosxEdgeEnc*)(uintptr_t)c.iarg[0], (dosx_stream_t)(uintptr_t)c.iarg[1]); }
static int thunk_dosx_heads_bwd_supported(const DosxCall& c) { return dosx_heads_bwd_supported((int)c.iarg[0]); }
static int thunk_dosx_heads_bwd(const DosxCall& c) { return dosx_heads_bwd((const DosxHeadsBwd*)(uintptr_t)c.iarg[0], (dosx_stream_t)(uintptr_t)c.iarg[1]); }
static int thunk_dosx_gemm_bf16x3_supported(const DosxCall& c) { return dosx_gemm_bf16x3_supported((int)c.iarg[0], (int)c.iarg[1], (int)c.iarg[2]); }
static int thunk_dosx_gemm_bf16x3(const DosxCall& c) { return dosx_gemm_bf16x3((const float*)(uintptr_t)c.iarg[0], (int)c.iarg[1], (const float*)(uintptr_t)c.iarg[2], (int)c.iarg[3], (int)c.iarg[4], (const float*)(uintptr_t)c.iarg[5], (float*)(uintptr_t)c.iarg[6], (int)c.iarg[7], (int)c.iarg[8], (int)c.iarg[9], (int)c.iarg[10], (int)c.iarg[11], (const float*)(uintptr_t)c.iarg[12], (int)c.iarg[13], (const float*)(uintptr_t)c.iarg[14], (int)c.iarg[15], (dosx_stream_t)(uintptr_t)c.iarg[16]); }
static int thunk_dosx_mlp_ln_supported(const DosxCall& c) { return dosx_mlp_ln_supported((int)c.iarg[0], (int)c.iarg[1], (int)c.iarg[2]); }
static int thunk_dosx_mlp_ln_cs_supported(const DosxCall& c) { return dosx_mlp_ln_cs_supported((int)c.iarg[0], (int)c.iarg[1], (int)c.iarg[2]); }
static int thunk_dosx_mlp_ln_cs_tiles(const DosxCall& c) { return dosx_mlp_ln_cs_tiles((int)c.iarg[0]); }
static int thunk_dosx_mlp_ln_fwd(const DosxCall& c) { return dosx_mlp_ln_fwd((const DosxMlpLn*)(uintptr_t)c.iarg[0], (dosx_stream_t)(uintptr_t)c.iarg[1]); }
static int thunk_dosx_enc_cs_supported(const DosxCall& c) { return dosx_enc_cs_supported((int)c.iarg[0], (int)c.iarg[1]); }
static int thunk_dosx_enc_cs_fwd(const DosxCall& c) { return dosx_enc_cs_fwd((const DosxEncCs*)(uintptr_t)c.iarg[0], (dosx_stream_t)(uintptr_t)c.iarg[1]); }
static int thunk_dosx_mlp_ln_bwd_partial_rows(const DosxCall& c) { return dosx_mlp_ln_bwd_partial_rows((int)c.iarg[0]); }
static int thunk_dosx_mlp_ln_bwd(const DosxCall& c) { return dosx_mlp_ln_bwd((const DosxMlpLnBwd*)(uintptr_t)c.iarg[0], (dosx_stream_t)(uintptr_t)c.iarg[1]); }
static int thunk_dosx_edge_mlp_bwd(const DosxCall& c) { return dosx_edge_mlp_bwd((const DosxEdgeMlpBwd*)(uintptr_t)c.iarg[0], (dosx_stream_t)(uintptr_t)c.iarg[1]); }
static int thunk_dosx_node_grad(const DosxCall& c) { return dosx_node_grad((const DosxNodeGrad*)(uintptr_t)c.iarg[0], (dosx_stream_t)(uintptr_t)c.iarg[1]); }
static int thunk_dosx_edge_mlp_supported(const DosxCall& c) { return dosx_edge_mlp_supported((int)c.iarg[0]); }
static int thunk_dosx_edge_mlp_fwd(const DosxCall& c) { return dosx_edge_mlp_fwd((const DosxEdgeMlp*)(uintptr_t)c.iarg[0], (dosx_stream_t)(uintptr_t)c.iarg[1]); }
static int thunk_dosx_csr_workspace_bytes(const DosxCall& c) { return dosx_csr_workspace_bytes((int)c.iarg[0], (size_t*)(uintptr_t)c.iarg[1]); }
static int thunk_dosx_csr_build(const DosxCall& c) { return dosx_csr_build((const long long*)(uintptr_t)c.iarg[0], (const long long*)(uintptr_t)c.iarg[1], (int)c.iarg[2], (int)c.iarg[3], (int)c.iarg[4], (int32_t*)(uintptr_t)c.iarg[5], (int32_t*)(uintptr_t)c.iarg[6], (long long*)(uintptr_t)c.iarg[7], (int32_t*)(uintptr_t)c.iarg[8], (int32_t*)(uintptr_t)c.iarg[9], (int32_t*)(uintptr_t)c.iarg[10], (int32_t*)(uintptr_t)c.iarg[11], (int32_t*)(uintptr_t)c.iarg[12], (int32_t*)(uintptr_t)c.iarg[13], (float*)(uintptr_t)c.iarg[14], (int32_t*)(uintptr_t)c.iarg[15], (void*)(uintptr_t)c.iarg[16], (size_t)c.iarg[17], (dosx_stream_t)(uintptr_t)c.iarg[18]); }
static int thunk_dosx_collate_padded(const DosxCall& c) { return dosx_collate_padded((const DosxCollate*)(uintptr_t)c.iarg[0], (dosx_stream_t)(uintptr_t)c.iarg[1]); }
static int thunk_dosx_collate_padded_f64(const DosxCall& c) { return dosx_collate_padded_f64((const DosxCollate*)(uintptr_t)c.iarg[0], (dosx_stream_t)(uintptr_t)c.iarg[1]); }
static int thunk_dosx_neighbor_count(const DosxCall& c) { return dosx_neighbor_count((const double*)(uintptr_t)c.iarg[0], (const double*)(uintptr_t)c.iarg[1], (const int32_t*)(uintptr_t)c.iarg[2], (const long long*)(uintptr_t)c.iarg[3], (int)c.iarg[4], (long long)c.iarg[5], (double)c.farg[0], (int)c.iarg[6], (int)c.iarg[7], (int32_t*)(uintptr_t)c.iarg[8], (dosx_stream_t)(uintptr_t)c.iarg[9]); }
static int thunk_dosx_neighbor_fill(const DosxCall& c) { return dosx_neighbor_fill((const double*)(uintptr_t)c.iarg[0], (const double*)(uintptr_t)c.iarg[1], (const int32_t*)(uintptr_t)c.iarg[2], (const long long*)(uintptr_t)c.iarg[3], (int)c.iarg[4], (long long)c.iarg[5], (double)c.farg[0], (int)c.iarg[6], (int)c.iarg[7], (const long long*)(uintptr_t)c.iarg[8], (int32_t*)(uintptr_t)c.iarg[9], (int32_t*)(uintptr_t)c.iarg[10], (int32_t*)(uintptr_t)c.iarg[11], (int32_t*)(uintptr_t)c.iarg[12], (double*)(uintptr_t)c.iarg[13], (dosx_stream_t)(uintptr_t)c.iarg[14]); }
static int thunk_dosx_knn_graph(const DosxCall& c) { return dosx_knn_graph((const DosxKnn*)(uintptr_t)c.iarg[0], (dosx_stream_t)(uintptr_t)c.iarg[1]); }
static int thunk_dosx_dropout_mask(const DosxCall& c) { return dosx_dropout_mask((float*)(uintptr_t)c.iarg[0], (int64_t)c.iarg[1], (float)c.farg[0], (const unsigned long long*)(uintptr_t)c.iarg[2], (long long)c.iarg[3], (dosx_stream_t)(uintptr_t)c.iarg[4]); }
static int thunk_dosx_copy_many(const DosxCall& c) { return dosx_copy_many((const DosxCopyJob*)(uintptr_t)c.iarg[0], (int)c.iarg[1], (dosx_stream_t)(uintptr_t)c.iarg[2]); }
static int thunk_dosx_fill(const DosxCall& c) { return dosx_fill((float*)(uintptr_t)c.iarg[0], (float)c.farg[0], (int64_t)c.iarg[1], (dosx_stream_t)(uintptr_t)c.iarg[2]); }
static int thunk_dosx_embed_rows(const DosxCall& c) { return dosx_embed_rows((const float*)(uintptr_t)c.iarg[0], (const int32_t*)(uintptr_t)c.iarg[1], (float*)(uintptr_t)c.iarg[2], (int)c.iarg[3], (int)c.iarg[4], (dosx_stream_t)(uintptr_t)c.iarg[5]); }
static int thunk_dosx_embed_rows_bwd(const DosxCall& c) { return dosx_embed_rows_bwd((const float*)(uintptr_t)c.iarg[0], (int)c.iarg[1], (const int32_t*)(uintptr_t)c.iarg[2], (float*)(uintptr_t)c.iarg[3], (int)c.iarg[4], (int)c.iarg[5], (int)c.iarg[6], (dosx_stream_t)(uintptr_t)c.iarg[7]); }
static int thunk_dosx_reduce_rows(const DosxCall& c) { return dosx_reduce_rows((const float*)(uintptr_t)c.iarg[0], (int)c.iarg[1], (float*)(uintptr_t)c.iarg[2], (int)c.iarg[3], (int)c.iarg[4], (int)c.iarg[5], (int)c.iarg[6], (int)c.iarg[7], (int)c.iarg[8], (int)c.iarg[9], (dosx_stream_t)(uintptr_t)c.iarg[10]); }
static int thunk_dosx_act_bwd(const DosxCall& c) { return dosx_act_bwd((const float*)(uintptr_t)c.iarg[0], (const float*)(uintptr_t)c.iarg[1], (float)c.farg[0], (float*)(uintptr_t)c.iarg[2], (int64_t)c.iarg[3], (dosx_stream_t)(uintptr_t)c.iarg[4]); }
static int thunk_dosx_gemm_f64(const DosxCall& c) { return dosx_gemm_f64((const DosxGemm64*)(uintptr_t)c.iarg[0], (dosx_stream_t)(uintptr_t)c.iarg[1]); }
static int thunk_dosx_wgrad_f64(const DosxCall& c) { return dosx_wgrad_f64((const DosxWgrad64*)(uintptr_t)c.iarg[0], (dosx_stream_t)(uintptr_t)c.iarg[1]); }
static int thunk_dosx_colsum_f64(const DosxCall& c) { return dosx_colsum_f64((const double*)(uintptr_t)c.iarg[0], (int)c.iarg[1], (int)c.iarg[2], (int)c.iarg[3], (double*)(uintptr_t)c.iarg[4], (double*)(uintptr_t)c.iarg[5], (int)c.iarg[6], (dosx_stream_t)(uintptr_t)c.iarg[7]); }
static int thunk_dosx_layernorm_f64(const DosxCall& c) { return dosx_layernorm_f64((const double*)(uintptr_t)c.iarg[0], (const double*)(uintptr_t)c.iarg[1], (const double*)(uintptr_t)c.iarg[2], (const double*)(uintptr_t)c.iarg[3], (double*)(uintptr_t)c.iarg[4], (double*)(uintptr_t)c.iarg[5], (double*)(uintptr_t)c.iarg[6], (int)c.iarg[7], (int)c.iarg[8], (dosx_stream_t)(uintptr_t)c.iarg[9]); }
static int thunk_dosx_layernorm_bwd_f64(const DosxCall& c) { return dosx_layernorm_bwd_f64((const double*)(uintptr_t)c.iarg[0], (const double*)(uintptr_t)c.iarg[1], (const double*)(uintptr_t)c.iarg[2], (const double*)(uintptr_t)c.iarg[3], (const double*)(uintptr_t)c.iarg[4], (const double*)(uintptr_t)c.iarg[5], (double*)(uintptr_t)c.iarg[6], (double*)(uintptr_t)c.iarg[7], (int)c.iarg[8], (int)c.iarg[9], (dosx_stream_t)(uintptr_t)c.iarg[10]); }
static int thunk_dosx_act_bwd_f64(const DosxCall& c) { return dosx_act_bwd_f64((const double*)(uintptr_t)c.iarg[0], (const double*)(uintptr_t)c.iarg[1], (int)c.iarg[2], (int)c.iarg[3], (const double*)(uintptr_t)c.iarg[4], (double*)(uintptr_t)c.iarg[5], (double*)(uintptr_t)c.iarg[6], (int)c.iarg[7], (int)c.iarg[8], (dosx_stream_t)(uintptr_t)c.iarg[9]); }
static int thunk_dosx_edge_feat_sh1_f64(const DosxCall& c) { return dosx_edge_feat_sh1_f64((const double*)(uintptr_t)c.iarg[0], (double*)(uintptr_t)c.iarg[1], (int)c.iarg[2], (double)c.farg[0], (dosx_stream_t)(uintptr_t)c.iarg[3]); }
static int thunk_dosx_segment_mean_f64(const DosxCall& c) { return dosx_segment_mean_f64((const double*)(uintptr_t)c.iarg[0], (const int32_t*)(uintptr_t)c.iarg[1], (double*)(uintptr_t)c.iarg[2], (int)c.iarg[3], (int)c.iarg[4], (dosx_stream_t)(uintptr_t)c.iarg[5]); }
static int thunk_dosx_segment_mean_bwd_f64(const DosxCall& c) { return dosx_segment_mean_bwd_f64((const double*)(uintptr_t)c.iarg[0], (int)c.iarg[1], (const int32_t*)(uintptr_t)c.iarg[2], (const int32_t*)(uintptr_t)c.iarg[3], (const double*)(uintptr_t)c.iarg[4], (double*)(uintptr_t)c.iarg[5], (int)c.iarg[6], (int)c.iarg[7], (dosx_stream_t)(uintptr_t)c.iarg[8]); }
static int thunk_dosx_gather_bwd_f64(const DosxCall& c) { return dosx_gather_bwd_f64((const double*)(uintptr_t)c.iarg[0], (int)c.iarg[1], (const int32_t*)(uintptr_t)c.iarg[2], (const int32_t*)(uintptr_t)c.iarg[3], (const int32_t*)(uintptr_t)c.iarg[4], (const double*)(uintptr_t)c.iarg[5], (int)c.iarg[6], (const double*)(uintptr_t)c.iarg[7], (int)c.iarg[8], (double*)(uintptr_t)c.iarg[9], (int)c.iarg[10], (int)c.iarg[11], (dosx_stream_t)(uintptr_t)c.iarg[12]); }
static int thunk_dosx_graph_pool_f64(const DosxCall& c) { return dosx_graph_pool_f64((const double*)(uintptr_t)c.iarg[0], (const int32_t*)(uintptr_t)c.iarg[1], (double*)(uintptr_t)c.iarg[2], (int)c.iarg[3], (int)c.iarg[4], (dosx_stream_t)(uintptr_t)c.iarg[5]); }
static int thunk_dosx_rows_add_f64(const DosxCall& c) { return dosx_rows_add_f64((const double*)(uintptr_t)c.iarg[0], (int)c.iarg[1], (const int32_t*)(uintptr_t)c.iarg[2], (const double*)(uintptr_t)c.iarg[3], (int)c.iarg[4], (const int32_t*)(uintptr_t)c.iarg[5], (double*)(uintptr_t)c.iarg[6], (int)c.iarg[7], (int)c.iarg[8], (int)c.iarg[9], (dosx_stream_t)(uintptr_t)c.iarg[10]); }
// ... 14 lines not shown
  {"dosx_gemm_pair", thunk_dosx_gemm_pair, 3, 0},
  {"dosx_gemm_kernel_name", thunk_dosx_gemm_kernel_name, 3, 0},
  {"dosx_wgrad_splits", thunk_dosx_wgrad_splits, 3, 0},
  {"dosx_wgrad_tiles", thunk_dosx_wgrad_tiles, 2, 0},
  {"dosx_wgrad", thunk_dosx_wgrad, 2, 0},
  {"dosx_wgrad_grouped", thunk_dosx_wgrad_grouped, 3, 0},
  {"dosx_reduce_partials", thunk_dosx_reduce_partials, 3, 0},
  {"dosx_grad_flush", thunk_dosx_grad_flush, 5, 0},
  {"dosx_edge_feat_sh1", thunk_dosx_edge_feat_sh1, 4, 1},
  {"dosx_edge_embed_sh1", thunk_dosx_edge_embed_sh1, 8, 1},
  {"dosx_segment_reduce", thunk_dosx_segment_reduce, 10, 0},
  {"dosx_segment_reduce_perm", thunk_dosx_segment_reduce_perm, 8, 0},
  {"dosx_act_segment_sum", thunk_dosx_act_segment_sum, 13, 0},
  {"dosx_seg_count_scale", thunk_dosx_seg_count_scale, 8, 0},
  {"dosx_edge_grad_combine", thunk_dosx_edge_grad_combine, 10, 0},
  {"dosx_gather_bwd", thunk_dosx_gather_bwd, 14, 0},
  {"dosx_graph_pool", thunk_dosx_graph_pool, 7, 0},
  {"dosx_graph_pool_bwd", thunk_dosx_graph_pool_bwd, 9, 0},
  {"dosx_dense_normalize", thunk_dosx_dense_normalize, 8, 0},
  {"dosx_dense_normalize_slots", thunk_dosx_dense_normalize_slots, 8, 0},
  {"dosx_dense_normalize_bwd", thunk_dosx_dense_normalize_bwd, 10, 0},
  {"dosx_dense_normalize_pool_bwd", thunk_dosx_dense_normalize_pool_bwd, 14, 0},
  {"dosx_dense_slots", thunk_dosx_dense_slots, 7, 0},
  {"dosx_dense_slots_bwd", thunk_dosx_dense_slots_bwd, 8, 0},
  {"dosx_gather_add_rownorm", thunk_dosx_gather_add_rownorm, 12, 0},
  {"dosx_rownorm", thunk_dosx_rownorm, 6, 0},
  {"dosx_rownorm_bwd", thunk_dosx_rownorm_bwd, 8, 0},
  {"dosx_mask_residual", thunk_dosx_mask_residual, 11, 0},
  {"dosx_rownorm_bwd_act", thunk_dosx_rownorm_bwd_act, 9, 1},
  {"dosx_layernorm", thunk_dosx_layernorm, 9, 0},
  {"dosx_ln_prelu_bwd", thunk_dosx_ln_prelu_bwd, 11, 0},
  {"dosx_ln_prelu_bwd_gather", thunk_dosx_ln_prelu_bwd_gather, 13, 0},
  {"dosx_layernorm_bwd", thunk_dosx_layernorm_bwd, 9, 0},
  {"dosx_attention_pkv_supported", thunk_dosx_attention_pkv_supported, 2, 0},
  {"dosx_attention_aligned_mode", thunk_dosx_attention_aligned_mode, 1, 0},
  {"dosx_attention_fwd", thunk_dosx_attention_fwd, 2, 0},
  {"dosx_attention_bwd", thunk_dosx_attention_bwd, 2, 0},
  {"dosx_attn_pv", thunk_dosx_attn_pv, 10, 0},
  {"dosx_attn_tv", thunk_dosx_attn_tv, 11, 0},
  {"dosx_attn_dp", thunk_dosx_attn_dp, 9, 0},
  {"dosx_softmax_bwd", thunk_dosx_softmax_bwd, 7, 1},
  {"dosx_softmax_fwd", thunk_dosx_softmax_fwd, 5, 1},
  {"dosx_ln_rowdot", thunk_dosx_ln_rowdot, 12, 0},
  {"dosx_ln_rowdot_bwd", thunk_dosx_ln_rowdot_bwd, 12, 0},
  {"dosx_rowdot", thunk_dosx_rowdot, 8, 0},
  {"dosx_rowdot_bwd", thunk_dosx_rowdot_bwd, 9, 0},
  {"dosx_sse2", thunk_dosx_sse2, 6, 0},
  {"dosx_loss_phonon_bwd", thunk_dosx_loss_phonon_bwd, 9, 2},
  {"dosx_loss_phonon", thunk_dosx_loss_phonon, 9, 1},
  {"dosx_loss_edos", thunk_dosx_loss_edos, 10, 1},
  {"dosx_sum", thunk_dosx_sum, 4, 0},
  {"dosx_adamw", thunk_dosx_adamw, 7, 6},
  {"dosx_ffn_supported", thunk_dosx_ffn_supported, 1, 0},
  {"dosx_ffn_att_supported", thunk_dosx_ffn_att_supported, 2, 0},
  {"dosx_ffn_att_aligned_supported", thunk_dosx_ffn_att_aligned_supported, 2, 0},
  {"dosx_ffn_fwd", thunk_dosx_ffn_fwd, 2, 0},
  {"dosx_ffn_fwd_multi", thunk_dosx_ffn_fwd_multi, 3, 0},
  {"dosx_ffn_bwd_partial_rows", thunk_dosx_ffn_bwd_partial_rows, 1, 0},
  {"dosx_ffn_att_bwd_supported", thunk_dosx_ffn_att_bwd_supported, 4, 0},
  {"dosx_ffn_att_bwd_partial_rows", thunk_dosx_ffn_att_bwd_partial_rows, 2, 0},
  {"dosx_ffn_att_aligned_rows", thunk_dosx_ffn_att_aligned_rows, 2, 0},
  {"dosx_ffn_bwd", thunk_dosx_ffn_bwd, 2, 0},
  {"dosx_edge_enc_supported", thunk_dosx_edge_enc_supported, 1, 0},
  {"dosx_edge_enc_fwd", thunk_dosx_edge_enc_fwd, 2, 0},
  {"dosx_heads_bwd_supported", thunk_dosx_heads_bwd_supported, 1, 0},
  {"dosx_heads_bwd", thunk_dosx_heads_bwd, 2, 0},
  {"dosx_gemm_bf16x3_supported", thunk_dosx_gemm_bf16x3_supported, 3, 0},
  {"dosx_gemm_bf16x3", thunk_dosx_gemm_bf16x3, 17, 0},
  {"dosx_mlp_ln_supported", thunk_dosx_mlp_ln_supported, 3, 0},
  {"dosx_mlp_ln_cs_supported", thunk_dosx_mlp_ln_cs_supported, 3, 0},
  {"dosx_mlp_ln_cs_tiles", thunk_dosx_mlp_ln_cs_tiles, 1, 0},
  {"dosx_mlp_ln_fwd", thunk_dosx_mlp_ln_fwd, 2, 0},
  {"dosx_enc_cs_supported", thunk_dosx_enc_cs_supported, 2, 0},
  {"dosx_enc_cs_fwd", thunk_dosx_enc_cs_fwd, 2, 0},
  {"dosx_mlp_ln_bwd_partial_rows", thunk_dosx_mlp_ln_bwd_partial_rows, 1, 0},
  {"dosx_mlp_ln_bwd", thunk_dosx_mlp_ln_bwd, 2, 0},
  {"dosx_edge_mlp_bwd", thunk_dosx_edge_mlp_bwd, 2, 0},
  {"dosx_node_grad", thunk_dosx_node_grad, 2, 0},
  {"dosx_edge_mlp_supported", thunk_dosx_edge_mlp_supported, 1, 0},
  {"dosx_edge_mlp_fwd", thunk_dosx_edge_mlp_fwd, 2, 0},
  {"dosx_csr_workspace_bytes", thunk_dosx_csr_workspace_bytes, 2, 0},
  {"dosx_csr_build", thunk_dosx_csr_build, 19, 0},
  {"dosx_collate_padded", thunk_dosx_collate_padded, 2, 0},
  {"dosx_collate_padded_f64", thunk_dosx_collate_padded_f64, 2, 0},
  {"dosx_neighbor_count", thunk_dosx_neighbor_count, 10, 1},
  {"dosx_neighbor_fill", thunk_dosx_neighbor_fill, 15, 1},
  {"dosx_knn_graph", thunk_dosx_knn_graph, 2, 0},
  {"dosx_dropout_mask", thunk_dosx_dropout_mask, 5, 1},
  {"dosx_copy_many", thunk_dosx_copy_many, 3, 0},
  {"dosx_fill", thunk_dosx_fill, 3, 1},
  {"dosx_embed_rows", thunk_dosx_embed_rows, 6, 0},
  {"dosx_embed_rows_bwd", thunk_dosx_embed_rows_bwd, 8, 0},
  {"dosx_reduce_rows", thunk_dosx_reduce_rows, 11, 0},
  {"dosx_act_bwd", thunk_dosx_act_bwd, 5, 1},
  {"dosx_gemm_f64", thunk_dosx_gemm_f64, 2, 0},
  {"dosx_wgrad_f64", thunk_dosx_wgrad_f64, 2, 0},
  {"dosx_colsum_f64", thunk_dosx_colsum_f64, 8, 0},
  {"dosx_layernorm_f64", thunk_dosx_layernorm_f64, 10, 0},
  {"dosx_layernorm_bwd_f64", thunk_dosx_layernorm_bwd_f64, 11, 0},
  {"dosx_act_bwd_f64", thunk_dosx_act_bwd_f64, 10, 0},
  {"dosx_edge_feat_sh1_f64", thunk_dosx_edge_feat_sh1_f64, 4, 1},
  {"dosx_segment_mean_f64", thunk_dosx_segment_mean_f64, 6, 0},
  {"dosx_segment_mean_bwd_f64", thunk_dosx_segment_mean_bwd_f64, 9, 0},
  {"dosx_gather_bwd_f64", thunk_dosx_gather_bwd_f64, 13, 0},
  {"dosx_graph_pool_f64", thunk_dosx_graph_pool_f64, 6, 0},
  {"dosx_rows_add_f64", thunk_dosx_rows_add_f64, 11, 0},
// ... 11 lines not shown
```

### dostransformer_amd/csrc/rowops.hip

```cpp
#include <math.h>

#include "common.h"

namespace {

__global__ __launch_bounds__(256) void layernorm_kernel(const float* __restrict__ x, const float* __restrict__ gamma,
                                                        const float* __restrict__ beta, float* __restrict__ y,
                                                        float* __restrict__ xhat, float* __restrict__ rstd_out,
                                                        int M, int H) {
  const int lane = threadIdx.x & 63;
  const int r = blockIdx.x * 4 + (threadIdx.x >> 6);
  if (r >= M) return;
  const float* row = x + (size_t)r * H;
  float s1 = 0.f;
  for (int c = lane * 4; c < H; c += 256) {
    const float4 v = ld4(row + c);
    s1 += v.x + v.y + v.z + v.w;
  }
  const float mean = wave_sum(s1) / (float)H;
  float s2 = 0.f;
  for (int c = lane * 4; c < H; c += 256) {
    const float4 v = ld4(row + c);
    const float a = v.x - mean, b = v.y - mean, c2 = v.z - mean, d = v.w - mean;
    s2 += a * a + b * b + c2 * c2 + d * d;
// ... 372 lines not shown
      const float4 v = ld4(x + (size_t)r * H + c), ww = ld4(w + c);
      my[c] += dyr * v.x; my[c + 1] += dyr * v.y; my[c + 2] += dyr * v.z; my[c + 3] += dyr * v.w;
      st4(dx + (size_t)r * H + c, make_float4(dyr * ww.x, dyr * ww.y, dyr * ww.z, dyr * ww.w));
    }
  }
  if (lane == 0) my[H] = db;
  __syncthreads();
  float* prow = partials + (size_t)blockIdx.x * (H + 1);
  for (int c = threadIdx.x; c < H + 1; c += 256)
    prow[c] = sm[c] + sm[(H + 1) + c] + sm[2 * (H + 1) + c] + sm[3 * (H + 1) + c];
}

__global__ __launch_bounds__(1024) void sse2_kernel(const float* __restrict__ pg, const float* __restrict__ ps,
                                                    const float* __restrict__ y, float* __restrict__ sse, int count) {
  __shared__ float red[2][16];
  float a = 0.f, b = 0.f;
  for (int i = threadIdx.x; i < count; i += 1024) {
    const float t = y[i], d0 = pg[i] - t, d1 = ps[i] - t;
    a += d0 * d0;
    b += d1 * d1;
  }
  a = wave_sum(a);
  b = wave_sum(b);
  const int lane = threadIdx.x & 63, wave = threadIdx.x >> 6;
  if (lane == 0) { red[0][wave] = a; red[1][wave] = b; }
  __syncthreads();
  if (threadIdx.x == 0) {
    float s0 = 0.f, s1 = 0.f;
    for (int i = 0; i < 16; ++i) { s0 += red[0][i]; s1 += red[1][i]; }
    sse[0] = s0;
    sse[1] = s1;
  }
}

__global__ void loss_phonon_bwd_kernel(const float* __restrict__ pg, const float* __restrict__ ps,
                                       const float* __restrict__ y, const float* __restrict__ sse, float beta,
                                       float inv_count, float* __restrict__ dpg, float* __restrict__ dps,
                                       float* __restrict__ loss, int count) {
  const float r0 = sqrtf(sse[0] * inv_count), r1 = sqrtf(sse[1] * inv_count);
  const float k0 = inv_count / r0, k1 = beta * inv_count / r1;
  const int i = blockIdx.x * blockDim.x + threadIdx.x;
  if (i == 0 && loss) loss[0] = r0 + beta * r1;
  if (i < count) {
    const float t = y[i];
    dpg[i] = (pg[i] - t) * k0;
    dps[i] = (ps[i] - t) * k1;
  }
}

__global__ __launch_bounds__(1024) void loss_phonon_fused_kernel(const float* __restrict__ pg, const float* __restrict__ ps,
                                                                 const float* __restrict__ y, float* __restrict__ sse,
                                                                 float beta, float inv_count, float* __restrict__ dpg,
                                                                 float* __restrict__ dps, float* __restrict__ loss, int count) {
  __shared__ float red[2][16];
  __shared__ float tot[2];
  float a = 0.f, b = 0.f;
  for (int i = threadIdx.x; i < count; i += 1024) {
    const float t = y[i], d0 = pg[i] - t, d1 = ps[i] - t;
    a += d0 * d0;
    b += d1 * d1;
  }
  a = wave_sum(a);
  b = wave_sum(b);
  const int lane = threadIdx.x & 63, wave = threadIdx.x >> 6;
  if (lane == 0) { red[0][wave] = a; red[1][wave] = b; }
  __syncthreads();
  if (threadIdx.x == 0) {
    float s0 = 0.f, s1 = 0.f;
    for (int i = 0; i < 16; ++i) { s0 += red[0][i]; s1 += red[1][i]; }
    tot[0] = s0; tot[1] = s1;
    if (sse) { sse[0] = s0; sse[1] = s1; }
  }
  __syncthreads();
  const float r0 = sqrtf(tot[0] * inv_count), r1 = sqrtf(tot[1] * inv_count);
  const float k0 = inv_count / r0, k1 = beta * inv_count / r1;
  if (threadIdx.x == 0 && loss) loss[0] = r0 + beta * r1;
  for (int i = threadIdx.x; i < count; i += 1024) {
    const float t = y[i];
    dpg[i] = (pg[i] - t) * k0;
    dps[i] = (ps[i] - t) * k1;
  }
}

__global__ __launch_bounds__(256) void loss_edos_kernel(const float* __restrict__ pg, const float* __restrict__ ps,
                                                        const float* __restrict__ y_ft, float beta, int B, int S,
                                                        float inv_bglobal, float* __restrict__ dpg,
                                                        float* __restrict__ dps, float* __restrict__ loss_partial) {
  const int lane = threadIdx.x & 63;
  const int b = blockIdx.x * 4 + (threadIdx.x >> 6);
  if (b >= B) return;
  const size_t o = (size_t)b * S;
  float a = 0.f, c = 0.f;
  for (int s = lane; s < S; s += 64) {
    const float t = fmaxf(y_ft[o + s], 0.f);
    const float d0 = t - pg[o + s], d1 = t - ps[o + s];
    a += d0 * d0;
    c += d1 * d1;
  }
  a = wave_sum(a);
  c = wave_sum(c);
  const float r0 = sqrtf(a / (float)S), r1 = sqrtf(c / (float)S);
  const float k0 = inv_bglobal / ((float)S * r0), k1 = beta * inv_bglobal / ((float)S * r1);
  for (int s = lane; s < S; s += 64) {
    const float t = fmaxf(y_ft[o + s], 0.f);
    dpg[o + s] = (pg[o + s] - t) * k0;
    dps[o + s] = (ps[o + s] - t) * k1;
  }
  if (lane == 0) loss_partial[b] = (r0 + beta * r1) * inv_bglobal;
}

__global__ __launch_bounds__(256) void sum_kernel(const float* __restrict__ src, int n, float* __restrict__ dst) {
  __shared__ float red[4];
  float s = 0.f;
  for (int i = threadIdx.x; i < n; i += 256) s += src[i];
  s = wave_sum(s);
  if ((threadIdx.x & 63) == 0) red[threadIdx.x >> 6] = s;
  __syncthreads();
  if (threadIdx.x == 0) dst[0] = (red[0] + red[1]) + (red[2] + red[3]);
}

__global__ void adamw_kernel(float* __restrict__ p, const float* __restrict__ g, float* __restrict__ m,
                             float* __restrict__ v, size_t n, float decay, float beta1, float beta2, float eps,
                             float step_size, float inv_bc2s, float gscale) {
  const size_t n4 = n >> 2;
  for (size_t i = (size_t)blockIdx.x * blockDim.x + threadIdx.x; i < n4; i += (size_t)gridDim.x * blockDim.x) {
    float4 pp = ld4(p + 4 * i), gg = ld4(g + 4 * i), mm = ld4(m + 4 * i), vv = ld4(v + 4 * i);
    float* P = &pp.x; float* G = &gg.x; float* Mm = &mm.x; float* V = &vv.x;
#pragma unroll
    for (int j = 0; j < 4; ++j) {
      const float gr = G[j] * gscale;
      float pj = P[j] * decay;
      const float mj = Mm[j] + (gr - Mm[j]) * (1.f - beta1);
      const float vj = V[j] * beta2 + (1.f - beta2) * gr * gr;
      const float denom = sqrtf(vj) * inv_bc2s + eps;
// ... 308 lines not shown
```

### dostransformer_amd/functional.py

```python
from __future__ import annotations

from typing import Dict, List, Optional, Sequence, Tuple

import torch

from . import ops
from ._lib import Attn, Seg, from_environ
from ._lib import load as _lib_load
from .batch import GraphMeta
from .ops import (ACT_LEAKY, ACT_RELU, EPI_LN, EPI_PRELU_BWD, EPI_PRELU_LN_BWD, EPI_PRELU_LN_BWD_SEG, EPI_RELU_MASK, EPI_ROWLN_BWD, EPI_SEGSUM,
                  PRO_LN_PRELU, PRO_PRELU, PRO_ROWLN, GradSink, rowmap, seg)

Params = Dict[str, torch.Tensor]


def _empty(dev, *shape):
    return ops.alloc(dev, *shape)


def _rows32(m: int) -> int:
    return (m + 31) // 32


class SegList:

    def __init__(self, segs: Sequence[Seg], keep: Sequence[torch.Tensor], plain: Optional[Sequence[torch.Tensor]] = None):
        self.segs = list(segs)
        self.keep = list(keep)
        self.K = sum(s.width for s in segs)
        self.plain = plain
        self.factor = None
        self.aggsum = None


def pack_params(P: Params) -> Params:
    ptrs = [t.data_ptr() for t in P.values()]
    if not ptrs or max(ptrs) - min(ptrs) < (1 << 30):
        return P
    flat = torch.empty(sum((t.numel() + 3) // 4 * 4 for t in P.values()), device=next(iter(P.values())).device)
    out, o = {}, 0
    for k, t in P.items():
        v = flat[o:o + t.numel()].view(t.shape)
        v.copy_(t)
        out[k] = v
        o += (t.numel() + 3) // 4 * 4
    return out


_FACTOR_EDGE_WGRAD = True
_FACTOR_MIN_GF = 0.5
_FACTOR_FUSED = True
_EDGE_ONE_LAUNCH = True
_EDGE_ONE_LAUNCH_BWD = True
_FACTOR_LAST = True
_FACTOR_LAST_MIN_GF = 1.3
_FACTOR_HEADS = True
_FACTOR_HEADS_MIN_GF = 1.0
_FUSED_ATT_FFN = True
_ATT_FFN_MAX_ROWS = 4096
_ATT_ALIGNED = True
_ATT_ALIGNED_MAX_WGS = 256
_ATT_ROWS_FIRST = True
_FUSED_ATT_BWD = True
_FFN_MULTI = True
_FUSED_FIN_BWD = True
_FUSED_HEAD_FWD = True
_FFN_BF16X3 = from_environ("DOSX_FFN_BF16X3", "0") == "1"

_TAIL_SPLITS = 32
_MID_HOOK_LATE_MAX_H = 128
_FFN_TAIL_MAX = 2048


def _wgrad_linear(sink: GradSink, G: Params, wkey: str, bkey: Optional[str], M: int, N: int, dy: Seg,
                  segs: Sequence[Seg], keep=(), tail: bool = False, dst: Optional[torch.Tensor] = None, **pro) -> None:
    if wkey not in G:
        return
    K = sum(s.width for s in segs)
    ns = ops.wgrad_splits(M, N, K)
    if tail:
        ns = max(ns, min(_TAIL_SPLITS, max(M // 128, 1)))
    nsc = ops.wgrad_scratch_floats(N, K, ns)
    slab = sink.scratch(nsc) if nsc else None
    slab_b = sink.scratch(ns * ((N + 63) // 64) * 64) if (bkey is not None and ns > 1) else None
    kw = dict(dst=G[wkey] if dst is None else dst, dst_bias=G[bkey] if bkey is not None else None, **pro)
    keep = tuple(keep) + tuple(t for t in pro.values() if isinstance(t, torch.Tensor))
    sink.defer_wgrad(ops.wgrad_desc(M, N, dy, segs, slab, slab_b, ns, **kw), keep)


def mlp_prelu_fwd(P: Params, key: str, a: SegList, M: int, H: int, z: Optional[torch.Tensor] = None):
    dev = P[key + ".0.weight"].device
    if z is None:
        z = _empty(dev, M, H)
        ops.gemm(M, H, a.segs, P[key + ".0.weight"], z, bias=P[key + ".0.bias"])
    y = _empty(dev, M, H)
    ops.gemm(M, H, [seg(z)], P[key + ".2.weight"], y, pro=PRO_PRELU, pro_alpha=P[key + ".1.weight"],
             bias=P[key + ".2.bias"])
    return y, (a, z, M, H)


def mlp_prelu_bwd(P: Params, G: Params, key: str, ctx, dy: torch.Tensor, sink: GradSink, dy_seg: Optional[Seg] = None,
                  tail: bool = False):
    a, z, M, H = ctx
    dev = z.device
    alpha = P[key + ".1.weight"]
    dys = dy_seg if dy_seg is not None else seg(dy)
    _wgrad_linear(sink, G, key + ".2.weight", key + ".2.bias", M, H, dys, [seg(z)], keep=(dy,) if dy is not None else (),
                  tail=tail, pro=PRO_PRELU, pro_alpha=alpha)
    rows = ops.gemm_partial_rows(M, H, EPI_PRELU_BWD)
    part = sink.scratch(rows, 1)
    dz = _empty(dev, M, H)
    ops.gemm(M, H, [dys], P[key + ".2.weight"], dz, w_layout=1, epi=EPI_PRELU_BWD, aux=z, epi_alpha=alpha,
             partials=part, partial_ld=1)
    sink.add(part, 0, G[key + ".1.weight"], rows, 1, 1)
    _wgrad_linear(sink, G, key + ".0.weight", key + ".0.bias", M, H, seg(dz), a.segs, keep=(dz,), tail=tail)


def mlp_prelu_bwd_pair(P: Params, G: Params, first, second, sink: GradSink, tail: bool = False):
    descs, later = [], []
# ... 342 lines not shown
                sink._keep.extend([dcat_n, dx, dcat_e[4], aggD])
                if src_job is not None:
                    src_job()
                if early:
                    dx, de = dx_old, de_new
                    continue
                if l == 0 and sink.wside is not None:
                    flush_side(l)
            elif _factor_fused(m, H):
                if fold_dx:
                    ops.gemm(N, H, [seg(aggS), seg(aggD)], W0[:, :H], dx_old, w_layout=1, w_seg_off=H, res=dcat_n[:, :H])
                else:
                    t1 = _empty(dev, N, H)
                    ops.gemm(N, H, [seg(aggS), seg(aggD)], W0[:, :H], t1, w_layout=1, w_seg_off=H, res=dx)
                    ops.mask_residual(dcat_n[:, :H], None, t1, dx_old, None, N, H)
                    sink._keep.append(t1)
                sink._keep.extend([dcat_n, dx])
            else:
                t1, t2 = _empty(dev, N, H), _empty(dev, N, H)
                ops.gemm(N, H, [seg(aggS)], W0[:, :H], t1, w_layout=1, res=dx)
                ops.gemm(N, H, [seg(aggD)], W0[:, H:2 * H], t2, w_layout=1, res=t1)
                ops.mask_residual(dcat_n[:, :H], None, t2, dx_old, None, N, H)
                sink._keep.extend([dcat_n, t1, t2, dx])
            dx, de = dx_old, de_new
            if sink.side is not None and l == 1:
                flush_side(l)
            continue
        ops.gather_bwd(dcat_e, dcat_n.data_ptr(), 2 * H, dx, m.rowptr_dst, m.rowptr_src, m.perm_src, None, dx_old,
                       None, N, E, H)
        sink._keep.append(dcat_n)
        dx, de = dx_old, dcat_e[:, 2 * H:]
        if sink.side is not None and l == 1:
            flush_side(l)
    return dx, de


def _attn_desc(Sq, Bq, Nk, Bk, H, qs, qb, x, kvhat, gam, bet) -> Attn:
    a = Attn()
    a.Sq, a.Bq, a.Nk, a.Bk, a.H = Sq, Bq, Nk, Bk, H
    a.q_stride_s, a.q_stride_b, a.flags = qs, qb, 0
    a.x, a.kvhat, a.gamma0, a.beta0 = x.data_ptr(), kvhat.data_ptr(), gam.data_ptr(), bet.data_ptr()
    return a


DROP_MASK_LOG: Optional[list] = None
EDROP_MASK_LOG: Optional[list] = None
FDROP_MASK_LOG: Optional[list] = None


def head_fused_fwd(H: int, T: int) -> bool:
    return bool(ops.ffn_supported(H) and _FUSED_HEAD_FWD and T > 0)


def encoder_fwd(P: Params, pre: str, x: torch.Tensor, Sq: int, Bq: int, qs: int, qb: int, kvhat: torch.Tensor,
                Nk: int, Bk: int, H: int, T: int, final_ln: bool = True, drop=None, head=None, fdrop=None, key_ptr=None):
    dev = kvhat.device
    rows = Sq * Bq
    lay = []
    fin_fused = None
    if fdrop is not None and not (fdrop[0] > 0.0 or fdrop[1] > 0.0):
        fdrop = None
    assert fdrop is None or head is None
    stack = [] if _FFN_MULTI else None
    for t in range(T):
        lp = f"{pre}.layers.{t}"
        g0, b0 = P[lp + ".layer_norms.0.weight"], P[lp + ".layer_norms.0.bias"]
        x1 = _empty(dev, rows, H)
        probs = _empty(dev, Bq, Sq, Nk)
        qstats = _empty(dev, rows, 2)
        st1 = _empty(dev, rows, 2)
        a = _attn_desc(Sq, Bq, Nk, Bk, H, qs, qb, x, kvhat, g0, b0)
        a.out, a.probs, a.qstats, a.out_stats = x1.data_ptr(), probs.data_ptr(), qstats.data_ptr(), st1.data_ptr()
        if key_ptr is not None:
            assert key_ptr.dtype == torch.int32 and key_ptr.numel() >= Bk + 1 and fdrop is None
            a.key_ptr = key_ptr.data_ptr()
        mask = None
        if drop is not None and drop[0] > 0.0:
            mask = _empty(dev, Bq, Sq, Nk)
            ops.dropout_mask(mask, drop[0], drop[1], drop[2] + t)
            a.drop_mask = mask.data_ptr()
            if DROP_MASK_LOG is not None:
                DROP_MASK_LOG.append((pre, t, mask))
        fm = None
        if fdrop is not None:
            p_relu, p_res, fseed, fbase = fdrop

            def draw(shape, p, k):
                if p <= 0.0:
                    return None
                m_ = _empty(dev, *shape)
                ops.dropout_mask(m_, p, fseed, fbase + 3 * t + k)
                if FDROP_MASK_LOG is not None:
                    FDROP_MASK_LOG.append((pre, t, ("res1", "relu", "res2")[k], m_))
                return m_
            m1, m2, m3 = draw((rows, H), p_res, 0), draw((rows, 4 * H), p_relu, 1), draw((rows, H), p_res, 2)
            fm = (m1, m2, m3)
            a.flags |= 2
            att = _empty(dev, rows, H)
            a.out = att.data_ptr()
            ops.attention_fwd(a)
            assert qs == Bq and qb == 1, "relu / res dropout: dense query rows only (layers.TransformerEncoder)"
            ops.mask_residual(att, m1, x, x1, st1, rows, H)
            h = _empty(dev, rows, 4 * H)
            ops.gemm(rows, 4 * H, [seg(x1)], P[lp + ".fc1.weight"], h, pro=PRO_ROWLN,
                     pro_gamma=P[lp + ".layer_norms.1.weight"], pro_beta=P[lp + ".layer_norms.1.bias"], pro_stats=st1,
                     bias=P[lp + ".fc1.bias"], act=ACT_RELU)
            if m2 is not None:
                ops.mask_residual(h, m2, None, h, None, rows, 4 * H)
            y2 = _empty(dev, rows, H)
            ops.gemm(rows, H, [seg(h)], P[lp + ".fc2.weight"], y2, bias=P[lp + ".fc2.bias"])
            x2 = _empty(dev, rows, H)
            ops.mask_residual(y2, m3, x1, x2, None, rows, H)
            lay.append((x, qs, qb, x1, probs, qstats, st1, h, mask, fm))
            x, qs, qb = x2, Bq, 1
            continue
        att_fused = _FUSED_ATT_FFN and rows <= _ATT_FFN_MAX_ROWS and ops.ffn_att_supported(H, Nk)
        att_aligned = False
        if _FUSED_ATT_FFN and _ATT_ALIGNED and fdrop is None and ops.ffn_supported(H) and ops.ffn_att_aligned_supported(H, Nk):
            r_al = _lib_load().dosx_ffn_att_aligned_rows(int(Sq), int(Bq))
            if Bq * ((Sq + r_al - 1) // r_al) <= _ATT_ALIGNED_MAX_WGS and not (att_fused and _ATT_ROWS_FIRST):
                att_fused = att_aligned = True
        xln = None
        if not att_fused:
            if stack:
                ops.ffn_fwd_multi(stack)
                stack.clear()
            if not ops.ffn_supported(H) and Nk <= 320:
                xln = _empty(dev, rows, H)
                a.ln1_gamma, a.ln1_beta = P[lp + ".layer_norms.1.weight"].data_ptr(), P[lp + ".layer_norms.1.bias"].data_ptr()
                a.ln1_out = xln.data_ptr()
                x1._dosx_ln1 = xln
            ops.attention_fwd(a)
        h = _empty(dev, rows, 4 * H)
        x2 = _empty(dev, rows, H)
        if ops.ffn_supported(H):
            fin_args = None
            if final_ln and t == T - 1:
                fin_fused = (_empty(dev, rows, H), _empty(dev, rows))
                fin_args = (P[pre + ".layer_norm.weight"], P[pre + ".layer_norm.bias"]) + fin_fused
            elif head is not None and t == T - 1:
                assert not final_ln and head_fused_fwd(H, T)
                hg, hb, hw, hbias, hxh, hrs, hdos = head
                fin_args = (hg, hb, hxh, hrs, hw, hbias, hdos, Sq, Bq)
                x2 = None
            att_args = None
            if att_fused:
                att_args = dict(kvhat=kvhat, gamma0=g0, beta0=b0, Nk=Nk, Bk=Bk, Bq=Bq, Sq=Sq, qs=qs, qb=qb, probs=probs,
                                qstats=qstats, x1=x1, st1=st1, mask=mask, aligned=att_aligned, key_ptr=key_ptr)
            ops.ffn_fwd(rows, H, x if att_fused else x1, None if att_fused else st1, P[lp + ".layer_norms.1.weight"],
                        P[lp + ".layer_norms.1.bias"], P[lp + ".fc1.weight"], P[lp + ".fc1.bias"], P[lp + ".fc2.weight"],
                        P[lp + ".fc2.bias"], h, x2, fin=fin_args, att=att_args, defer=stack if att_fused else None)
        else:
            def ffn_rows(r0, r1, x1=x1, st1=st1, h=h, x2=x2, lp=lp, xln=xln):
                if xln is not None and _bf16x3_ok(r1 - r0, 4 * H, H):
                    ops.gemm_bf16x3(xln[r0:r1], P[lp + ".fc1.weight"], h[r0:r1], bias=P[lp + ".fc1.bias"], act=ACT_RELU)
                elif xln is not None:
                    ops.gemm(r1 - r0, 4 * H, [seg(xln[r0:r1])], P[lp + ".fc1.weight"], h[r0:r1], bias=P[lp + ".fc1.bias"], act=ACT_RELU)
                else:
                    ops.gemm(r1 - r0, 4 * H, [seg(x1[r0:r1])], P[lp + ".fc1.weight"], h[r0:r1], pro=PRO_ROWLN,
                             pro_gamma=P[lp + ".layer_norms.1.weight"], pro_beta=P[lp + ".layer_norms.1.bias"], pro_stats=st1[r0:r1],
                             bias=P[lp + ".fc1.bias"], act=ACT_RELU)
                if _bf16x3_ok(r1 - r0, H, 4 * H):
                    ops.gemm_bf16x3(h[r0:r1], P[lp + ".fc2.weight"], x2[r0:r1], bias=P[lp + ".fc2.bias"], res=x1[r0:r1])
                else:
                    ops.gemm(r1 - r0, H, [seg(h[r0:r1])], P[lp + ".fc2.weight"], x2[r0:r1], bias=P[lp + ".fc2.bias"], res=x1[r0:r1])
            mt = _ffn_tail_start(rows, H)
            if mt:
                ops.concurrent(dev, lambda: ffn_rows(mt, rows), lambda: ffn_rows(0, mt))
            else:
                ffn_rows(0, rows)
        lay.append((x, qs, qb, x1, probs, qstats, st1, h, mask, None))
        x, qs, qb = x2, Bq, 1
    if stack:
        ops.ffn_fwd_multi(stack)
    fin = None
    if final_ln and fin_fused is not None:
        fin = fin_fused
    elif final_ln:
        y = _empty(dev, rows, H)
        xhat = _empty(dev, rows, H)
        rstd = _empty(dev, rows)
        ops.layernorm(x, P[pre + ".layer_norm.weight"], P[pre + ".layer_norm.bias"], y, xhat, rstd, rows, H)
        fin = (xhat, rstd)
        x = y
    return x, (lay, fin, Sq, Bq, Nk, Bk, H, T, kvhat, key_ptr)


def _bf16x3_ok(rows: int, n: int, k: int) -> bool:
    return _FFN_BF16X3 and ops.gemm_bf16x3_supported(rows, n, k)


def _ffn_tail_start(rows: int, H: int) -> int:
    gy = (H + 127) // 128
    if 256 % gy:
        return 0
    per_round = 256 // gy * 64
    mt = rows // per_round * per_round
    return mt if mt > 0 and 0 < rows - mt <= _FFN_TAIL_MAX else 0


def head_fused_bwd(H: int, T: int) -> bool:
    return bool(ops.ffn_supported(H) and _FUSED_FIN_BWD and T > 0)


# ... 356 lines not shown


def gnn_trunk_bwd(P: Params, G: Params, cfg: ModelCfg, m: GraphMeta, ctx, dxL: torch.Tensor, du_seg: Optional[Seg],
                  sink: GradSink, dx_pre=None):
    with ops.graph_rows():
        _gnn_trunk_bwd(P, G, cfg, m, ctx, dxL, du_seg, sink, dx_pre)


def _gnn_trunk_bwd(P: Params, G: Params, cfg: ModelCfg, m: GraphMeta, ctx, dxL: torch.Tensor, du_seg: Optional[Seg],
                   sink: GradSink, dx_pre=None):
    cn, ce, cu, cg, node_key = ctx
    dx0, de0 = gnn_bwd(P, G, m, cg, dxL, sink, cfg.L, cfg.mean, cfg.H, dx_pre=dx_pre)
    if de0 is not None and cn[3] == ce[3]:
        mlp_prelu_bwd_pair(P, G, (node_key, cn, dx0), ("GN_encoder.edge_encoder", ce, de0), sink, tail=True)
        if cu is not None and du_seg is not None:
            mlp_prelu_bwd(P, G, "GN_encoder.global_encoder", cu, None, sink, dy_seg=du_seg, tail=True)
        return
    mlp_prelu_bwd(P, G, node_key, cn, dx0, sink, tail=True)
    mlp_prelu_bwd(P, G, "GN_encoder.edge_encoder", ce, de0, sink, tail=True)
    if cu is not None and du_seg is not None:
        mlp_prelu_bwd(P, G, "GN_encoder.global_encoder", cu, None, sink, dy_seg=du_seg, tail=True)


def decoder_fwd(P: Params, cfg: ModelCfg, m: GraphMeta, xL: torch.Tensor, u: Optional[torch.Tensor]):
    H, B = cfg.H, m.num_graphs
    dev = xL.device
    pooled = _empty(dev, B, H)
    ops.graph_pool(xL, m.graph_ptr, pooled.data_ptr(), H, B, H)
    segs = SegList([seg(pooled)], [pooled]) if u is None else SegList([seg(u), seg(pooled)], [u, pooled])
    graph = _empty(dev, B, H)
    ops.gemm(B, H, segs.segs, P["GN_decoder.mlp.0.weight"], graph, bias=P["GN_decoder.mlp.0.bias"])
    return graph, segs


def decoder_dgrad(P: Params, cfg: ModelCfg, m: GraphMeta, segs: SegList, dgraph: torch.Tensor) -> torch.Tensor:
    dcat = _empty(dgraph.device, m.num_graphs, segs.K)
    ops.gemm(m.num_graphs, segs.K, [seg(dgraph)], P["GN_decoder.mlp.0.weight"], dcat, w_layout=1)
    return dcat


def decoder_bwd(P: Params, G: Params, cfg: ModelCfg, m: GraphMeta, segs: SegList, dgraph: torch.Tensor, dxL: Optional[torch.Tensor],
                sink: GradSink, dcat: Optional[torch.Tensor] = None) -> Optional[Seg]:
    H, B, N = cfg.H, m.num_graphs, m.num_nodes
    _wgrad_linear(sink, G, "GN_decoder.mlp.0.weight", "GN_decoder.mlp.0.bias", B, H, seg(dgraph), segs.segs, keep=(dgraph,))
    K = segs.K
    if dcat is None:
        dcat = decoder_dgrad(P, cfg, m, segs, dgraph)
    if dxL is not None:
        ops.graph_pool_bwd(dcat.data_ptr() + 4 * (K - H), K, m.node_graph, dxL, N, H, True, num_graphs=B)
    sink._keep.append(dcat)
    return seg(dcat, width=H, col=0) if K == 2 * H else None


def dostransformer_fwd(P: Params, cfg: ModelCfg, g, m: GraphMeta, drop=None, per_crystal_keys: bool = False):
    dr = (lambda base: None) if drop is None else (lambda base: (drop[0], drop[1], base))
    H, S, T, B, N = cfg.H, cfg.S, cfg.T, m.num_graphs, m.num_nodes
    if per_crystal_keys and H > ops.ATTN_MAX_H:
        from ._lib import DosxError
        raise DosxError(f"per_crystal_keys: hidden <= {ops.ATTN_MAX_H} (the attention kernels' row width), got {H}")
    kp = m.graph_ptr if per_crystal_keys else None
    if H > ops.ATTN_MAX_H:
        return _dostransformer_fwd_wide(P, cfg, g, m, dr)
    nmax = m.n_max
    dev = P["embeddings.weight"].device
    xL, u, ctrunk = gnn_trunk_fwd(P, cfg, g, m)
    kvhat = _empty(dev, nmax * B + 1, H)
    rstd_n = _empty(dev, N)
    ops.dense_normalize_slots(xL, m.graph_ptr, kvhat, rstd_n, B, nmax, H)
    emb = P["embeddings.weight"]
    sysidx = _i32(g.system)
    hp = H // 2
    side = ops.GradSink(dev)
    box = {}

    fh = _factor_heads(S * B, H)

    def _decoder_branch():
        box["graph"], box["segs"] = decoder_fwd(P, cfg, m, xL, u)
        box["prow"] = _empty(dev, B, hp)
        ops.embed_rows(P[cfg.prompt_key], sysidx, box["prow"], B, hp)
        if fh:
            box["qg"], box["qs"] = _empty(dev, B, H), _empty(dev, B, H)
            ops.gemm(B, H, [seg(box["graph"])], P["fc.weight"][:, H:], box["qg"])
            ops.gemm(B, H, [seg(box["graph"]), seg(box["prow"])], P["fc_prompt.weight"][:, H:], box["qs"])
    side.on_side(_decoder_branch)
    E1, c1 = encoder_fwd(P, "transformer", emb, S, B, 1, 0, kvhat, nmax, B, H, T, drop=dr(0), key_ptr=kp)
    side.join()
    graph, dec_segs, prow = box["graph"], box["segs"], box["prow"]
    dosin = _empty(dev, S * 2 * B, H)
    modB = rowmap(d=B, m=0, c=1)
    a_g = SegList([seg(E1), seg(graph, rmap=modB)], [E1, graph])
    a_s = SegList([seg(E1), seg(graph, rmap=modB), seg(prow, rmap=modB)], [E1, graph, prow])
    kvs = _empty(dev, S * 2 * B, H)
    rstd_s = _empty(dev, S * 2 * B)
    nk = dict(norm_out=kvs, norm_rstd=rstd_s)
    if fh:
        hg = dict(segs=[seg(E1)], w=P["fc.weight"][:, :H], res=box["qg"], res_map=modB, res_pre=True)
        hs = dict(segs=[seg(E1)], w=P["fc_prompt.weight"][:, :H], res=box["qs"], res_map=modB, res_pre=True)
    else:
        hg, hs = dict(segs=a_g.segs, w=P["fc.weight"]), dict(segs=a_s.segs, w=P["fc_prompt.weight"])
    ops.gemm_pair(dict(M=S * B, N=H, out=dosin, bias=P["fc.bias"], act=ACT_LEAKY, act_slope=0.01,
                       out_map=rowmap(d=B, m=2 * B, c=1, off=0), **hg, **nk),
                  dict(M=S * B, N=H, out=dosin, bias=P["fc_prompt.bias"], act=ACT_LEAKY,
                       act_slope=0.01, out_map=rowmap(d=B, m=2 * B, c=1, off=B), **hs, **nk))
    hs, c2 = encoder_fwd(P, "transformer_self", dosin, S, 2 * B, 2 * B, 1, kvs, S, 2 * B, H, T, drop=dr(64))
    xhat_f = _empty(dev, S * 2 * B, H)
    rstd_f = _empty(dev, S * 2 * B)
    dos = _empty(dev, 2 * B, S)
    gf, bf = P["transformer_source.layer_norm.weight"], P["transformer_source.layer_norm.bias"]
    if head_fused_fwd(H, T):
        _, c3 = encoder_fwd(P, "transformer_source", hs, S, 2 * B, 2 * B, 1, kvhat, nmax, B, H, T, final_ln=False,
                            drop=dr(128), head=(gf, bf, P["out_layer.weight"], P["out_layer.bias"], xhat_f, rstd_f, dos), key_ptr=kp)
    else:
        hsrc, c3 = encoder_fwd(P, "transformer_source", hs, S, 2 * B, 2 * B, 1, kvhat, nmax, B, H, T, final_ln=False,
                               drop=dr(128), key_ptr=kp)
        ops.ln_rowdot(hsrc, gf, bf, P["out_layer.weight"], P["out_layer.bias"], xhat_f, rstd_f, dos, S, 2 * B, H)
    a_g.keep.extend(t for t in (box.get("qg"), box.get("qs")) if t is not None)
    ctx = (ctrunk, kvhat, rstd_n, c1, dec_segs, sysidx, prow, dosin, a_g, a_s, kvs, rstd_s, c2, c3, xhat_f, rstd_f, xL)
    return dos, xL, ctx


def dostransformer_bwd(P: Params, G: Params, cfg: ModelCfg, m: GraphMeta, ctx, ddos: torch.Tensor,
                       dx_ext: Optional[torch.Tensor], sink: GradSink, mid_hook=None) -> None:
    if ctx[0] == "wide":
        return _dostransformer_bwd_wide(P, G, cfg, m, ctx, ddos, dx_ext, sink, mid_hook)
    (ctrunk, kvhat, rstd_n, c1, dec_segs, sysidx, prow, dosin, a_g, a_s, kvs, rstd_s, c2, c3, xhat_f, rstd_f, xL) = ctx
    H, S, B, N = cfg.H, cfg.S, m.num_graphs, m.num_nodes
    nmax = m.n_max
    dev = ddos.device
    rows2 = S * 2 * B
    r32 = _rows32(rows2)
    gf, bf = P["transformer_source.layer_norm.weight"], P["transformer_source.layer_norm.bias"]
    head = None
    if head_fused_bwd(H, cfg.T) and ddos.is_contiguous():
        dx = None
        head = (gf, bf, xhat_f, rstd_f, ddos, P["out_layer.weight"],
                ("transformer_source.layer_norm.weight", "transformer_source.layer_norm.bias", "out_layer.weight", "out_layer.bias"))
    else:
        pld = 3 * H + 1
        part = sink.scratch(r32, pld)
        dx = _empty(dev, rows2, H)
        ops.ln_rowdot_bwd(ddos, xhat_f, rstd_f, gf, bf, P["out_layer.weight"], dx, part, S, 2 * B, H)
        sink.add(part, 0, G["transformer_source.layer_norm.weight"], r32, pld, H)
        sink.add(part, H, G["transformer_source.layer_norm.bias"], r32, pld, H)
        sink.add(part, 2 * H, G["out_layer.weight"], r32, pld, H)
        sink.add(part, 3 * H, G["out_layer.bias"], r32, pld, 1)
    dkv = _empty(dev, nmax * B + 1, H)
    dhs = encoder_bwd(P, G, "transformer_source", c3, dx, dkv, sink, dkv_fresh=True, head=head)
    if sink.wside is not None:
        sink.flush_on_side()
    dkvs = _empty(dev, rows2, H)
    ddosin = encoder_bwd(P, G, "transformer_self", c2, dhs, dkvs, sink, dkv_fresh=True, kv_needed_next=True)
    late_flush = len(a_g.keep) <= 2
    if sink.wside is not None and not late_flush:
        sink.flush_on_side()
    sink.join()
    dpre = _empty(dev, rows2, H)
    Wfc, Wfp = P["fc.weight"], P["fc_prompt.weight"]
    heads_one = H <= 128 and ops.heads_bwd_supported(H) and ddosin.is_contiguous() and dkvs.is_contiguous()
    dE1 = _empty(dev, S * B, H)
    if heads_one:
        ops.heads_bwd(S, B, H, dkvs, kvs, rstd_s, ddosin, dosin, 0.01, dpre, Wfc, Wfp, dE1)
    else:
        ops.rownorm_bwd_act(dkvs, kvs, rstd_s, ddosin, dosin, 0.01, dpre, rows2, H)
    map0, map1 = rowmap(d=B, m=2 * B, c=1, off=0), rowmap(d=B, m=2 * B, c=1, off=B)
# ... 206 lines not shown
```

### dostransformer_amd/ops.py

```python
from __future__ import annotations

import contextlib
import ctypes as C
from typing import List, Optional, Sequence, Tuple

import numpy as np
import torch

from . import _lib
from ._lib import Ffn, BIG, Attn, Gemm, ReduceJob, RowMap, Seg, Wgrad

PRO_NONE, PRO_PRELU, PRO_LN_PRELU, PRO_ROWLN = 0, 1, 2, 3
EPI_BIAS_ACT, EPI_LN, EPI_PRELU_LN_BWD, EPI_RELU_MASK, EPI_ROWLN_BWD, EPI_PRELU_BWD, EPI_SEGSUM, EPI_PRELU_LN_BWD_SEG = 0, 1, 2, 3, 4, 5, 6, 7
ACT_NONE, ACT_RELU, ACT_LEAKY = 0, 1, 2


class _KernelTimer:

    def __init__(self):
        self.enabled = False
        self.records = []

    def reset(self, enabled: bool):
        self.enabled = enabled
# ... 298 lines not shown
    g = Gemm()
    g.M, g.N = int(M), int(N)
    g.K = int(sum(s.width for s in segs))
    g.nseg = len(segs)
    _set_segs(g.a, segs)
    g.pro = pro
    g.pro_gamma, g.pro_beta, g.pro_alpha, g.pro_stats = _p(pro_gamma), _p(pro_beta), _p(pro_alpha), _p(pro_stats)
    assert w.dim() == 2 and w.stride(1) == 1
    g.w, g.ldw, g.w_layout = w.data_ptr(), int(w.stride(0)), int(w_layout)
    g.epi, g.act, g.act_slope = epi, act, float(act_slope)
    g.bias = _p(bias)
    g.out, g.ldo = (out.data_ptr(), int(out.stride(0))) if out is not None else (None, int(N))
    g.out_map = out_map if out_map is not None else ident()
    g.res = _p(res)
    g.ldr = int(res.stride(0)) if res is not None else 0
    g.res_map = res_map if res_map is not None else ident()
    g.stats_out, g.aux_out = _p(stats_out), _p(aux_out)
    if norm_out is not None:
        assert norm_rstd is not None and out is not None and norm_out.stride(0) == out.stride(0)
        g.norm_out, g.norm_rstd = norm_out.data_ptr(), norm_rstd.data_ptr()
    g.aux = _p(aux)
    g.ldaux = int(aux.stride(0)) if aux is not None else 0
    g.aux_stats = _p(aux_stats)
    g.epi_gamma, g.epi_beta, g.epi_alpha = _p(epi_gamma), _p(epi_beta), _p(epi_alpha)
    g.partials, g.partial_ld = _p(partials), int(partial_ld)
    g.res_col0 = int(res_col0)
    g.res_pre = 1 if res_pre else 0
    g.w_seg_off = int(w_seg_off)
    if add_p is not None:
        assert add_q is not None and add_ip is not None and add_iq is not None and add_p.stride(0) == add_q.stride(0)
        assert add_ip.dtype == torch.int32 and add_iq.dtype == torch.int32
        g.add_p, g.add_ip, g.add_q, g.add_iq = add_p.data_ptr(), add_ip.data_ptr(), add_q.data_ptr(), add_iq.data_ptr()
        g.ld_add = int(add_p.stride(0))
    if seg_tile is not None:
        assert seg_tile.dim() == 2 and seg_tile.shape[0] == 3 and seg_tile.is_contiguous()
        g.seg_tile, g.seg_ntiles = seg_tile.data_ptr(), int(seg_tile.shape[1]) - 1
        g.seg_rowptr, g.seg_scale, g.seg_agg = _p(seg_rowptr), _p(seg_scale), _p(seg_agg)
        part = alloc(w.device, g.seg_ntiles, g.N)
        g.seg_part, g.seg_cnt = part.data_ptr(), COUNTERS.take(w.device, g.seg_ntiles)
    return g


def _gemm_work(g: Gemm):
    buf = C.create_string_buffer(96)
    _lib.load().dosx_gemm_kernel_name(C.byref(g), buf, 96)
    sym = buf.value.decode()
    return (f"gemm[N{g.N},K{g.K},{sym[11:]}]", sym, "mfma", 2.0 * _real(g.M) * g.N * g.K)


def ffn_supported(H: int) -> bool:
    return bool(_lib.load().dosx_ffn_supported(int(H)))


def ffn_att_supported(H: int, Nk: int) -> bool:
    return bool(_lib.load().dosx_ffn_att_supported(int(H), int(Nk)))


def ffn_att_aligned_supported(H: int, Nk: int) -> bool:
    return bool(_lib.load().dosx_ffn_att_aligned_supported(int(H), int(Nk)))


def ffn_fwd(M: int, H: int, x: torch.Tensor, stats: Optional[torch.Tensor], gamma, beta, w1, b1, w2, b2, h: torch.Tensor,
            out: torch.Tensor, fin=None, att=None, defer: Optional[list] = None) -> None:
    a = Ffn()
    a.M, a.H = int(M), int(H)
    a.x, a.ldx = x.data_ptr(), int(x.stride(0))
    a.stats = _p(stats)
    a.gamma, a.beta = gamma.data_ptr(), beta.data_ptr()
    a.w1, a.b1, a.w2, a.b2 = w1.data_ptr(), b1.data_ptr(), w2.data_ptr(), b2.data_ptr()
    a.h, a.ldh = h.data_ptr(), int(h.stride(0))
    if out is not None:
        a.out, a.ldo = out.data_ptr(), int(out.stride(0))
    nk_att = 0
    if att is not None:
        a.att_kvhat, a.att_gamma0, a.att_beta0 = att["kvhat"].data_ptr(), att["gamma0"].data_ptr(), att["beta0"].data_ptr()
        a.att_mask = _p(att.get("mask"))
        a.att_probs, a.att_qstats = att["probs"].data_ptr(), att["qstats"].data_ptr()
        a.att_x1, a.att_ldx1, a.att_st1 = att["x1"].data_ptr(), int(att["x1"].stride(0)), att["st1"].data_ptr()
        a.att_Nk, a.att_Bk, a.att_Bq, a.att_Sq = int(att["Nk"]), int(att["Bk"]), int(att["Bq"]), int(att["Sq"])
        a.att_qs, a.att_qb = int(att["qs"]), int(att["qb"])
        a.att_aligned = int(bool(att.get("aligned", False)))
        if att.get("key_ptr") is not None:
            a.att_key_ptr = att["key_ptr"].data_ptr()
        nk_att = a.att_Nk
    if fin is not None:
        a.fin_gamma, a.fin_beta, a.fin_xhat, a.fin_rstd = (t.data_ptr() for t in fin[:4])
        if len(fin) > 4:
            a.fin_w, a.fin_b, a.fin_dos, a.fin_S, a.fin_Bq = fin[4].data_ptr(), fin[5].data_ptr(), fin[6].data_ptr(), int(fin[7]), int(fin[8])
    if defer is not None:
        defer.append((a, 16.0 * M * H * H + 4.0 * M * nk_att * H))
        return
    _call("dosx_ffn_fwd", C.byref(a), _stream(),
          w=lambda: (f"ffn_fwd[H{H}{',att' if nk_att else ''}]", "ffn_fwd_kernel", "mfma", 16.0 * M * H * H + 4.0 * M * nk_att * H))


FFN_MULTI_MAX = 2


def ffn_fwd_multi(deferred: list) -> None:
    for i in range(0, len(deferred), FFN_MULTI_MAX):
        grp = deferred[i:i + FFN_MULTI_MAX]
        arr = (Ffn * len(grp))(*[d for d, _ in grp])
        work = sum(w for _, w in grp)
        H = grp[0][0].H
        if len(grp) == 1:
            _call("dosx_ffn_fwd", C.byref(arr[0]), _stream(), w=lambda H=H, work=work: (f"ffn_fwd[H{H},att]", "ffn_fwd_kernel", "mfma", work))
        else:
            _call("dosx_ffn_fwd_multi", arr, len(grp), _stream(),
                  w=lambda H=H, work=work, n=len(grp): (f"ffn_fwd[H{H},att,x{n}]", "ffn_fwd_multi_kernel", "mfma", work))


def ffn_bwd_partial_rows(M: int) -> int:
    return _lib.load().dosx_ffn_bwd_partial_rows(int(M))


def ffn_att_bwd_supported(H: int, Nk: int, Sq: int, Bq: int) -> bool:
    return bool(_lib.load().dosx_ffn_att_bwd_supported(int(H), int(Nk), int(Sq), int(Bq)))


def ffn_att_bwd_partial_rows(Sq: int, Bq: int) -> int:
    return _lib.load().dosx_ffn_att_bwd_partial_rows(int(Sq), int(Bq))


def ffn_bwd(M: int, H: int, dy: torch.Tensor, h: torch.Tensor, x: torch.Tensor, stats: torch.Tensor, gamma, w1, w2,
            dh: torch.Tensor, dx: Optional[torch.Tensor], partials: torch.Tensor, fin=None, att=None) -> None:
    a = _lib.FfnBwd()
    if fin is not None:
        a.fin_gamma, a.fin_xhat, a.fin_rstd, a.fin_dy = (t.data_ptr() for t in fin[:4])
        if len(fin) > 4:
            a.fin_ddos, a.fin_w, a.fin_beta, a.fin_S, a.fin_Bq = fin[4].data_ptr(), fin[5].data_ptr(), fin[6].data_ptr(), int(fin[7]), int(fin[8])
    a.M, a.H = int(M), int(H)
    if dy is not None:
        a.dy, a.lddy = dy.data_ptr(), int(dy.stride(0))
    else:
        a.lddy = int(fin[3].stride(0))
    a.h, a.ldh = h.data_ptr(), int(h.stride(0))
    a.x, a.ldx = x.data_ptr(), int(x.stride(0))
    a.stats, a.gamma = stats.data_ptr(), gamma.data_ptr()
    a.w1, a.w2 = w1.data_ptr(), w2.data_ptr()
    a.dh, a.lddh = dh.data_ptr(), int(dh.stride(0))
    if dx is not None:
# ... 1190 lines not shown
```

### dostransformer_amd/train.py

```python
from __future__ import annotations

from collections import OrderedDict
from typing import Optional

import torch

from . import functional as Fn
from . import ops
from ._lib import DosxError, from_environ
from ._models import DOSTransformerBase, _SEED_MOD, rank_seed_offset
from .batch import CrystalBatch, bucket_sizes, graph_meta, pad_batch
from .slots import Slot, SlotCache

_DP_MID_BUCKET = from_environ("DOSX_DP_MID_BUCKET", "0") == "1"
_DP_CHECK = from_environ("DOSX_DP_CHECK", "0") == "1"


class _AdamWState:

    def _state(self, fp):
        if self._fp is not fp:
            m, v = torch.zeros_like(fp.flat), torch.zeros_like(fp.flat)
            old = self._fp
            if old is not None and self._m is not None:
# ... 39 lines not shown
            val = (int(sd["drop_seed_base"]) + rank_seed_offset()) % _SEED_MOD
        elif sd.get("drop_seed") is not None:
            val = int(sd["drop_seed"])
        if val is not None:
            object.__setattr__(self.model, "_drop_seed", torch.tensor([val], dtype=torch.int64, device=m.device))
        h = sd.get("hyper", {})
        self.lr, self.eps, self.wd = h.get("lr", self.lr), h.get("eps", self.eps), h.get("weight_decay", self.wd)
        self.betas, self.beta = tuple(h.get("betas", self.betas)), h.get("beta", self.beta)

    def _bump_dropout_seed(self) -> None:
        seed = getattr(self.model, "_drop_seed", None)
        if seed is not None and self.model.training and getattr(self.model, "_attn_drop", 0.0) > 0.0:
            seed.add_(1)


class Trainer(_AdamWState, SlotCache):

    def __init__(self, model: DOSTransformerBase, lr: float = 1e-4, beta: float = 1.0, weight_decay: float = 1e-2,
                 betas=(0.9, 0.999), eps: float = 1e-8, dist=None, graph: bool = False, replay: bool = False,
                 bucket=(8, 128), max_slots: int = 32, promote: float = 0.0, per_crystal_keys: bool = False):
        if not isinstance(model, DOSTransformerBase):
            raise TypeError("Trainer drives DOSTransformer / DOSTransformer_phonon modules")
        model._require_fp32_program("Trainer")
        if per_crystal_keys and dist is not None:
            raise DosxError("Trainer(per_crystal_keys=True) is a single-GPU mode: not with dist (data parallelism)")
        self._per_crystal_keys = bool(per_crystal_keys)
        self.model, self.lr, self.beta, self.wd, self.betas, self.eps = model, lr, beta, weight_decay, betas, eps
        self.dist = dist
        self.graph = graph
        self.replay = replay
        self.bucket = tuple(bucket)
        self.bucketed = dist is not None and not graph
        self._early_work = None
        self._mid_work = None
        self._early_side = None
        self._rec_parts = []
        self.step_count = 0
        self._m = self._v = None
        self._fp = None
        self.kind = model._cfg.kind
        self.last_outputs = None
        self._slots: "OrderedDict[tuple, Slot]" = OrderedDict()
        self.max_slots = int(max_slots)
        self.slot_hits = self.slot_misses = self.slot_promoted = 0
        self.promote = float(promote)
        self._seen = {}
        self.kernel_timer = None
        self._ds_checked = []

    @property
    def per_crystal_keys(self) -> bool:
        return self._per_crystal_keys

    def _part_a(self, fp, g, m, st_n_global: Optional[int] = None):
        if st_n_global is None:
            st_n_global = m.num_graphs
        model, dev, cfg = self.model, fp.flat.device, self.model._cfg
        B, S = m.num_graphs, cfg.S
        dg, xL, ds, (ctx, dos) = model._program_fwd(fp.P, g, m, bump_seed=False,
                                                    per_crystal_keys=self._per_crystal_keys)
        st = {"ctx": ctx, "dos": dos, "out": (dg, xL, ds), "B": B, "S": S}
        if self.kind == "phonon":
            st["y"] = Fn._f32(g.phdos).reshape(B, S)
            st["sse"] = Fn._empty(dev, 2)
            st["split_loss"] = self.dist is not None or int(st_n_global) != B
            if st["split_loss"]:
                ops.sse2(dos[:B], dos[B:], st["y"], st["sse"], B * S)
        else:
            st["y"] = Fn._f32(g.y_ft).reshape(-1)
        return st

    def _part_b(self, fp, m, st, n_global: int):
        dev, cfg = fp.flat.device, self.model._cfg
        B, S, dos = st["B"], st["S"], st["dos"]
        ddos = Fn._empty(dev, *dos.shape)
        if self.kind == "phonon":
            loss = Fn._empty(dev, 1)
            if st["split_loss"] or int(n_global) != B:
                if not st["split_loss"]:
                    raise RuntimeError("n_global differs between the two halves of the step")
                ops.loss_phonon_bwd(dos[:B], dos[B:], st["y"], st["sse"], self.beta, float(n_global * S), ddos[:B],
                                    ddos[B:], loss, B * S)
            else:
                ops.loss_phonon(dos[:B], dos[B:], st["y"], st["sse"], self.beta, ddos[:B], ddos[B:], loss, B * S)
            loss = loss[0]
        else:
            lp = Fn._empty(dev, B + 1)
            ops.loss_edos(dos[:B], dos[B:], st["y"], self.beta, B, S, n_global, ddos[:B], ddos[B:], lp)
            ops.sum_to(lp, B, lp[B:])
            loss = lp[B]
        sink = ops.GradSink(dev)
        sink.gnn_hook = self._gnn_hook(fp)
        Fn.dostransformer_bwd(fp.P, fp.G, cfg, m, st["ctx"], ddos, None, sink, mid_hook=self._mid_hook(fp))
        sink.release()
        return loss

    def _mid_hook(self, fp):
        if self.dist is None:
            return lambda sink: sink.flush_on_side()
        if not self.bucketed or fp.n_late <= 0 or fp.n_late >= fp.total:
            return None

        def hook(sink):
            sink.flush_on_side()
            rec = ops.RECORDER.active
            if rec:
                self._rec_parts.append((ops.RECORDER.end(), "early"))
            self._start_early(fp, sink.wside)
            if rec:
                ops.RECORDER.begin()
        return hook

    def _gnn_hook(self, fp):
        if self.dist is None or not self.bucketed or not (0 < fp.n_late < fp.total) or not (0 < fp.n_last < fp.n_late) or not _DP_MID_BUCKET:
            return None

        def hook(sink):
            rec = ops.RECORDER.active
            if rec:
                self._rec_parts.append((ops.RECORDER.end(), "mid"))
            self._start_mid(fp, sink.wside)
            if rec:
                ops.RECORDER.begin()
        return hook

    def _start_early(self, fp, side) -> None:
        stream = side if side is not None else torch.cuda.current_stream()
        with torch.cuda.stream(stream):
            self._early_work = self.dist.all_reduce_grads_async(fp.grad[fp.n_late:])
        self._early_side = side

    def _start_mid(self, fp, side) -> None:
        stream = side if side is not None else torch.cuda.current_stream()
        with torch.cuda.stream(stream):
            self._mid_work = self.dist.all_reduce_grads_async(fp.grad[fp.n_last:fp.n_late])

    def _n_global(self, B: int, n_global: Optional[int], g=None) -> int:
        if n_global is not None:
            return int(n_global)
# ... 192 lines not shown
```

### include/dosx.h

```cpp
#ifndef DOSX_H
#define DOSX_H

#include <stddef.h>
#include <stdint.h>

#ifdef __cplusplus
extern "C" {
#endif

typedef void* dosx_stream_t;

typedef struct DosxRowMap {
  int32_t d, m, c, off;
  const int32_t* idx;
} DosxRowMap;

typedef struct DosxSeg {
  const float* p;
  int32_t ld;
  int32_t width;
  DosxRowMap map;
} DosxSeg;

enum {
// ... 204 lines not shown
int dosx_attention_bwd(const DosxAttn* a, dosx_stream_t stream);

int dosx_attn_pv(const float* A, const float* mask, const float* V, float* out, int Sq, int Bq, int Nk, int Bk, int H,
                 dosx_stream_t stream);
int dosx_attn_tv(const float* A, const float* mask, const float* X, float* out, int Sq, int Bq, int Nk, int Bk, int H,
                 int accumulate, dosx_stream_t stream);
int dosx_attn_dp(const float* X, const float* V, float* dP, int Sq, int Bq, int Nk, int Bk, int H, dosx_stream_t stream);
int dosx_softmax_bwd(const float* P, const float* mask, const float* dPd, float* dS, long long rows, int Nk, float scale,
                     dosx_stream_t stream);
int dosx_softmax_fwd(const float* S, float* P, long long rows, int Nk, float scale, dosx_stream_t stream);

int dosx_ln_rowdot(const float* x, const float* gamma, const float* beta, const float* w, const float* b,
                   float* xhat, float* rstd, float* dos, int S, int Bq, int H, dosx_stream_t stream);
int dosx_ln_rowdot_bwd(const float* ddos, const float* xhat, const float* rstd, const float* gamma,
                       const float* beta, const float* w, float* dx, float* partials, int S, int Bq, int H,
                       dosx_stream_t stream);
int dosx_rowdot(const float* x, const float* w, const float* b, float* dos, int S, int Bq, int H,
                dosx_stream_t stream);
int dosx_rowdot_bwd(const float* ddos, const float* x, const float* w, float* dx, float* partials, int S,
                    int Bq, int H, dosx_stream_t stream);

int dosx_sse2(const float* pg, const float* ps, const float* y, float* sse, int count, dosx_stream_t stream);
int dosx_loss_phonon_bwd(const float* pg, const float* ps, const float* y, const float* sse, float beta,
                         double count_global, float* dpg, float* dps, float* loss, int count,
                         dosx_stream_t stream);
int dosx_loss_phonon(const float* pg, const float* ps, const float* y, float* sse, float beta, float* dpg, float* dps,
                     float* loss, int count, dosx_stream_t stream);
int dosx_loss_edos(const float* pg, const float* ps, const float* y_ft, float beta, int B, int S, int B_global,
                   float* dpg, float* dps, float* loss_partial, dosx_stream_t stream);

int dosx_sum(const float* src, int n, float* dst, dosx_stream_t stream);

int dosx_adamw(float* p, const float* g, float* m, float* v, int64_t n, float lr, float beta1, float beta2,
               float eps, float weight_decay, int step, float grad_scale, dosx_stream_t stream);

typedef struct DosxFfn {
  int32_t M, H;
  const float* x; int32_t ldx;
  const float* stats;
  const float* gamma; const float* beta;
  const float* w1; const float* b1;
  const float* w2; const float* b2;
  float* h; int32_t ldh;
  float* out; int32_t ldo;
  const float* fin_gamma; const float* fin_beta;
  float* fin_xhat; float* fin_rstd;
  const float* fin_w; const float* fin_b; float* fin_dos;
  int32_t fin_S, fin_Bq;
  const float* att_kvhat; const float* att_gamma0; const float* att_beta0; const float* att_mask;
  float* att_probs; float* att_qstats; float* att_x1; float* att_st1;
  int32_t att_Nk, att_Bk, att_Bq, att_Sq, att_qs, att_qb, att_ldx1;
  int32_t att_aligned;
  const int32_t* att_key_ptr;
} DosxFfn;
int dosx_ffn_supported(int H);
int dosx_ffn_att_supported(int H, int Nk);
int dosx_ffn_att_aligned_supported(int H, int Nk);
int dosx_ffn_fwd(const DosxFfn* a, dosx_stream_t stream);
int dosx_ffn_fwd_multi(const DosxFfn* descs, int n, dosx_stream_t stream);

typedef struct DosxFfnBwd {
  int32_t M, H;
  const float* dy; int32_t lddy;
  const float* h; int32_t ldh;
  const float* x; int32_t ldx;
  const float* stats;
  const float* gamma;
  const float* w1; const float* w2;
  float* dh; int32_t lddh;
  float* dx; int32_t lddx;
  float* partials; int32_t partial_ld;
  const float* fin_gamma; const float* fin_xhat; const float* fin_rstd;
  float* fin_dy;
  const float* fin_ddos; const float* fin_w; const float* fin_beta;
  int32_t fin_S, fin_Bq;
  const float* att_x; int32_t att_ldxin;
  const float* att_kvhat; const float* att_gamma0; const float* att_beta0;
  const float* att_probs; const float* att_qstats; const float* att_mask;
  float* att_dxin; int32_t att_lddxin;
  float* att_partials_q; float* att_partials_kv; float* att_dkv_part; int32_t* att_dkv_cnt;
  float* att_dkvhat; int32_t att_dkv_accumulate;
  int32_t att_Nk, att_Bk, att_Bq, att_Sq, att_qs, att_qb;
  const int32_t* att_key_ptr;
} DosxFfnBwd;
int dosx_ffn_bwd_partial_rows(int M);
int dosx_ffn_att_bwd_supported(int H, int Nk, int Sq, int Bq);
int dosx_ffn_att_bwd_partial_rows(int Sq, int Bq);
int dosx_ffn_att_aligned_rows(int Sq, int Bq);
int dosx_ffn_bwd(const DosxFfnBwd* a, dosx_stream_t stream);

typedef struct DosxEdgeEnc {
  int32_t E, H;
  const float* vec;
  float inv_rmax;
  const float* w0; const float* b0;
  const float* alpha;
  const float* w2; const float* b2;
  float* attr; float* z;
  float* out; int32_t ldo;
} DosxEdgeEnc;
int dosx_edge_enc_supported(int H);
int dosx_edge_enc_fwd(const DosxEdgeEnc* a, dosx_stream_t stream);

typedef struct DosxHeadsBwd {
  int32_t S, B, H;
  const float* dkvs; const float* kvs; const float* rstd;
  const float* ddosin; const float* dosin;
  float slope;
// ... 334 lines not shown
```

Before: 61990 crystals/s.

## Fuse phonon loss and its gradient into the last FFN forward kernel

Adds a last-block-arrives tail to the final fused FFN/head forward kernel. The last workgroup, chosen through an atomic ticket counter, computes the phonon RMSE loss and the dos gradient. This removes the separate loss kernel launch and its dependency gap on the single-GPU path. In exchange, head outputs are written with coherent atomic stores and the loss is computed by one workgroup, which serialises that tail work.

```diff
diff --git a/dostransformer_amd/_lib.py b/dostransformer_amd/_lib.py
--- a/dostransformer_amd/_lib.py
+++ b/dostransformer_amd/_lib.py
@@ -137,6 +137,8 @@
         ("att_Nk", C.c_int32), ("att_Bk", C.c_int32), ("att_Bq", C.c_int32), ("att_Sq", C.c_int32),
         ("att_qs", C.c_int32), ("att_qb", C.c_int32), ("att_ldx1", C.c_int32), ("att_aligned", C.c_int32),
         ("att_key_ptr", C.c_void_p),
+        ("loss_y", C.c_void_p), ("loss_sse", C.c_void_p), ("loss_out", C.c_void_p), ("loss_ddos", C.c_void_p), ("loss_cnt", C.c_void_p),
+        ("loss_beta", C.c_float),
     ]
 
 
@@ -382,6 +384,7 @@
     "dosx_sum": [_P, _I, _P, _P],
     "dosx_adamw": [_P, _P, _P, _P, _L, _F, _F, _F, _F, _F, _I, _F, _P],
     "dosx_ffn_supported": [_I],
+    "dosx_ffn_loss_supported": [_I],
     "dosx_ffn_att_supported": [_I, _I],
     "dosx_ffn_att_aligned_supported": [_I, _I],
     "dosx_ffn_fwd": [C.POINTER(Ffn), _P],
diff --git a/dostransformer_amd/_models.py b/dostransformer_amd/_models.py
--- a/dostransformer_amd/_models.py
+++ b/dostransformer_amd/_models.py
@@ -104,14 +104,15 @@
             seed.add_(1)
         return p, seed
 
-    def _program_fwd(self, P, g, m, bump_seed: bool = True, per_crystal_keys: bool = False):
+    def _program_fwd(self, P, g, m, bump_seed: bool = True, per_crystal_keys: bool = False, loss=None):
         if P["embeddings.weight"].dtype == torch.float64:
+            assert loss is None
             dos, xL, ctx = F64.dostransformer_phonon_fwd(P, self._cfg, g, m, drop=self._dropout(dos_device(P), bump_seed),
                                                          per_crystal_keys=self._per_crystal_keys)
             B = m.num_graphs
             return dos[:B], xL, dos[B:], (ctx, dos)
         dos, xL, ctx = Fn.dostransformer_fwd(P, self._cfg, g, m, drop=self._dropout(dos_device(P), bump_seed),
-                                             per_crystal_keys=per_crystal_keys)
+                                             per_crystal_keys=per_crystal_keys, loss=loss)
         B = m.num_graphs
         return dos[:B], xL, dos[B:], (ctx, dos)
 
diff --git a/dostransformer_amd/csrc/common.h b/dostransformer_amd/csrc/common.h
--- a/dostransformer_amd/csrc/common.h
+++ b/dostransformer_amd/csrc/common.h
@@ -141,3 +141,51 @@
 __device__ __forceinline__ int dosx_ticket(int* counter) {
   return __hip_atomic_fetch_add(counter, 1, DOSX_TICKET_ORDER, __HIP_MEMORY_SCOPE_AGENT);
 }
+
+template <int NT, bool COH>
+__device__ __forceinline__ void dosx_loss_phonon_body(const float* __restrict__ pg, const float* __restrict__ ps,
+                                                      const float* __restrict__ y, float* __restrict__ sse, const float beta,
+                                                      const float inv_count, float* __restrict__ dpg, float* __restrict__ dps,
+                                                      float* __restrict__ loss, const int count, float* __restrict__ red,
+                                                      float* __restrict__ tot) {
+  static_assert(NT % 64 == 0 && 1024 % NT == 0, "dosx_loss_phonon_body: NT divides 1024");
+  constexpr int V = 1024 / NT, NW = NT / 64;
+  auto pred = [](const float* p) -> float {
+    if constexpr (COH) return __hip_atomic_load(p, __ATOMIC_RELAXED, __HIP_MEMORY_SCOPE_AGENT);
+    else return *p;
+  };
+  const int tid = threadIdx.x, lane = tid & 63, wave = tid >> 6;
+  float a[V], b[V];
+#pragma unroll
+  for (int v = 0; v < V; ++v) {
+    a[v] = 0.f;
+    b[v] = 0.f;
+    for (int i = tid + v * NT; i < count; i += 1024) {
+      const float t = y[i], d0 = pred(pg + i) - t, d1 = pred(ps + i) - t;
+      a[v] += d0 * d0;
+      b[v] += d1 * d1;
+    }
+  }
+#pragma unroll
+  for (int v = 0; v < V; ++v) {
+    a[v] = wave_sum(a[v]);
+    b[v] = wave_sum(b[v]);
+    if (lane == 0) { red[wave + NW * v] = a[v]; red[16 + wave + NW * v] = b[v]; }
+  }
+  __syncthreads();
+  if (tid == 0) {
+    float s0 = 0.f, s1 = 0.f;
+    for (int i = 0; i < 16; ++i) { s0 += red[i]; s1 += red[16 + i]; }
+    tot[0] = s0; tot[1] = s1;
+    if (sse) { sse[0] = s0; sse[1] = s1; }
+  }
+  __syncthreads();
+  const float r0 = sqrtf(tot[0] * inv_count), r1 = sqrtf(tot[1] * inv_count);
+  const float k0 = inv_count / r0, k1 = beta * inv_count / r1;
+  if (tid == 0 && loss) loss[0] = r0 + beta * r1;
+  for (int i = tid; i < count; i += NT) {
+    const float t = y[i];
+    dpg[i] = (pred(pg + i) - t) * k0;
+    dps[i] = (pred(ps + i) - t) * k1;
+  }
+}
diff --git a/dostransformer_amd/csrc/ffn.hip b/dostransformer_amd/csrc/ffn.hip
--- a/dostransformer_amd/csrc/ffn.hip
+++ b/dostransformer_amd/csrc/ffn.hip
@@ -325,7 +325,21 @@
   }
 }
 
-template <bool HALF, int KB, int ATTK>
+__device__ __forceinline__ void ffn_loss_tail(const DosxFfn& a, float* __restrict__ sm) {
+  asm volatile("s_waitcnt vmcnt(0)" ::: "memory");
+  __syncthreads();
+  int* flag = reinterpret_cast<int*>(sm);
+  if (threadIdx.x == 0) *flag = dosx_ticket(a.loss_cnt);
+  __syncthreads();
+  if (*flag != (int)gridDim.x - 1) return;
+  __builtin_amdgcn_fence(__ATOMIC_ACQUIRE, "wavefront");
+  if (threadIdx.x == 0) __hip_atomic_store(a.loss_cnt, 0, __ATOMIC_RELAXED, __HIP_MEMORY_SCOPE_AGENT);
+  const int count = (a.fin_Bq >> 1) * a.fin_S;
+  dosx_loss_phonon_body<512, true>(a.fin_dos, a.fin_dos + count, a.loss_y, a.loss_sse, a.loss_beta, (float)(1.0 / (double)count),
+                                   a.loss_ddos, a.loss_ddos + count, a.loss_out, count, sm + 4, sm + 36);
+}
+
+template <bool HALF, int KB, int ATTK, bool LOSS = false>
 __device__ __forceinline__ void ffn_fwd_body(const DosxFfn& a, float* __restrict__ sm) {
   constexpr int ATT = ATTK >= 3 ? ATTK - 2 : ATTK;
   constexpr bool KP = ATTK >= 3;
@@ -623,11 +637,17 @@
       }
       if (fdot) {
         dot = wave_sum(dot);
-        if (lane == 0 && r >= 0) a.fin_dos[(size_t)(r % a.fin_Bq) * a.fin_S + (r / a.fin_Bq)] = dot + fbias;
+        if constexpr (LOSS) {
+          if (lane == 0 && r >= 0)
+            __hip_atomic_store(a.fin_dos + (size_t)(r % a.fin_Bq) * a.fin_S + (r / a.fin_Bq), dot + fbias, __ATOMIC_RELAXED, __HIP_MEMORY_SCOPE_AGENT);
+        } else {
+          if (lane == 0 && r >= 0) a.fin_dos[(size_t)(r % a.fin_Bq) * a.fin_S + (r / a.fin_Bq)] = dot + fbias;
+        }
       }
     }
   }
   FSTAMP(6);
+  if constexpr (LOSS) ffn_loss_tail(a, sm);
 }
 
 template <bool HALF, int KB, int ATT>
@@ -635,6 +655,12 @@
   DOSX_SET_MAIN_PRIO();
   extern __shared__ __align__(16) float sm[];
   ffn_fwd_body<HALF, KB, ATT>(a, sm);
+}
+template <bool HALF, int ATT>
+__global__ __launch_bounds__(512) void ffn_fwd_loss_kernel(const DosxFfn a) {
+  DOSX_SET_MAIN_PRIO();
+  extern __shared__ __align__(16) float sm[];
+  ffn_fwd_body<HALF, 64, ATT, true>(a, sm);
 }
 
 constexpr int FFN_MULTI_MAX = 2;
@@ -650,6 +676,15 @@
   asm volatile("s_waitcnt vmcnt(0)" ::: "memory");
   __syncthreads();
   ffn_fwd_body<HALF, KB, ATT>(A.d[1], sm);
+}
+template <bool HALF, int ATT>
+__global__ __launch_bounds__(512) void ffn_fwd_multi_loss_kernel(const FfnMulti A) {
+  DOSX_SET_MAIN_PRIO();
+  extern __shared__ __align__(16) float sm[];
+  ffn_fwd_body<HALF, 64, ATT>(A.d[0], sm);
+  asm volatile("s_waitcnt vmcnt(0)" ::: "memory");
+  __syncthreads();
+  ffn_fwd_body<HALF, 64, ATT, true>(A.d[1], sm);
 }
 
 
@@ -1364,6 +1399,7 @@
 }
 
 extern "C" int dosx_ffn_supported(int H) { return (H % 32) == 0 && H >= 32 && H <= 128; }
+extern "C" int dosx_ffn_loss_supported(int H) { return dosx_ffn_supported(H) && ffn_chunk(H) == 64; }
 extern "C" int dosx_ffn_att_supported(int H, int Nk) { return dosx_ffn_supported(H) && Nk >= 1 && Nk <= 16; }
 extern "C" int dosx_ffn_att_aligned_supported(int H, int Nk) {
   if (!dosx_ffn_supported(H) || Nk < 1 || Nk > 64) return 0;
@@ -1371,7 +1407,8 @@
   return (size_t)((Nk + 15) & ~15) * (H + 4) + 32 * 68 <= 2 * (size_t)128 * (kb + 4);
 }
 
-struct FfnPlan { bool half; int kb, mode, grid; size_t smem; };
+struct FfnPlan { bool half, loss; int kb, mode, grid; size_t smem; };
+static bool ffn_has_loss(const DosxFfn& a) { return a.loss_y || a.loss_sse || a.loss_out || a.loss_ddos || a.loss_cnt; }
 static int ffn_fwd_prepare(const DosxFfn& a, FfnPlan& pl) {
   DOSX_CHECK_ARG(dosx_ffn_supported(a.H), "dosx_ffn_fwd: H=%d unsupported (multiple of 32, <= 128)", a.H);
   const bool att = a.att_kvhat != nullptr;
@@ -1385,6 +1422,17 @@
                                 "dosx_ffn_fwd: output-layer epilogue needs the final LayerNorm, w, b and S * Bq == M");
   DOSX_CHECK_ARG((a.ldx & 3) == 0 && (a.ldh & 3) == 0 && (a.ldo & 3) == 0, "dosx_ffn_fwd: leading dimensions must be multiples of 4");
   if (a.fin_gamma) DOSX_CHECK_ARG(a.fin_beta && a.fin_xhat && a.fin_rstd, "dosx_ffn_fwd: final LayerNorm needs beta / xhat / rstd");
+  pl.loss = ffn_has_loss(a);
+  if (pl.loss) {
+    DOSX_CHECK_ARG(a.fin_dos != nullptr, "dosx_ffn_fwd: the loss block needs the fused model head (fin_dos)");
+    DOSX_CHECK_ARG(a.loss_cnt != nullptr, "dosx_ffn_fwd: the loss block needs its arrival counter (loss_cnt)");
+    DOSX_CHECK_ARG(a.loss_y && a.loss_out && a.loss_ddos, "dosx_ffn_fwd: the loss block needs y, loss_out and loss_ddos (only loss_sse may be NULL)");
+    DOSX_CHECK_ARG((a.fin_Bq & 1) == 0, "dosx_ffn_fwd: the loss block needs fin_dos rows [global | system]: fin_Bq=%d is odd", a.fin_Bq);
+    DOSX_CHECK_ARG(((reinterpret_cast<uintptr_t>(a.loss_y) | reinterpret_cast<uintptr_t>(a.loss_sse) | reinterpret_cast<uintptr_t>(a.loss_out) |
+                     reinterpret_cast<uintptr_t>(a.loss_ddos) | reinterpret_cast<uintptr_t>(a.loss_cnt) | reinterpret_cast<uintptr_t>(a.fin_dos)) & 3) == 0,
+                   "dosx_ffn_fwd: the loss block's buffers must be 4-byte aligned");
+    DOSX_CHECK_ARG(dosx_ffn_loss_supported(a.H), "dosx_ffn_fwd: the loss block needs hidden 64 / 128 (64-wide weight chunks), got H=%d", a.H);
+  }
   const long long span = (const char*)a.w1 > (const char*)a.w2 ? (const char*)a.w1 - (const char*)a.w2 : (const char*)a.w2 - (const char*)a.w1;
   DOSX_CHECK_ARG(span + (long long)16 * a.H * a.H < 0x7fffffffLL, "dosx_ffn_fwd: fc1 / fc2 weights more than 2 GiB apart");
   const int H = a.H, H4 = 4 * H;
@@ -1416,6 +1464,17 @@
     DOSX_FFN_ATTR(false, 32, 4); DOSX_FFN_ATTR(true, 32, 4); DOSX_FFN_ATTR(false, 64, 4); DOSX_FFN_ATTR(true, 64, 4);
     DOSX_FFN_ATTR2(false, 32, 3); DOSX_FFN_ATTR2(true, 32, 3); DOSX_FFN_ATTR2(false, 64, 3); DOSX_FFN_ATTR2(true, 64, 3);
     DOSX_FFN_ATTR2(false, 32, 4); DOSX_FFN_ATTR2(true, 32, 4); DOSX_FFN_ATTR2(false, 64, 4); DOSX_FFN_ATTR2(true, 64, 4);
+#define DOSX_FFN_ATTR_L(HALF_, ATT_) \
+    (void)hipFuncSetAttribute(reinterpret_cast<const void*>(&ffn_fwd_loss_kernel<HALF_, ATT_>), hipFuncAttributeMaxDynamicSharedMemorySize, 160 * 1024)
+#define DOSX_FFN_ATTR2_L(HALF_, ATT_) \
+    (void)hipFuncSetAttribute(reinterpret_cast<const void*>(&ffn_fwd_multi_loss_kernel<HALF_, ATT_>), hipFuncAttributeMaxDynamicSharedMemorySize, 160 * 1024)
+    DOSX_FFN_ATTR_L(false, 0); DOSX_FFN_ATTR_L(true, 0);
+    DOSX_FFN_ATTR_L(false, 1); DOSX_FFN_ATTR_L(true, 1); DOSX_FFN_ATTR_L(false, 2); DOSX_FFN_ATTR_L(true, 2);
+    DOSX_FFN_ATTR_L(false, 3); DOSX_FFN_ATTR_L(true, 3); DOSX_FFN_ATTR_L(false, 4); DOSX_FFN_ATTR_L(true, 4);
+    DOSX_FFN_ATTR2_L(false, 1); DOSX_FFN_ATTR2_L(true, 1); DOSX_FFN_ATTR2_L(false, 2); DOSX_FFN_ATTR2_L(true, 2);
+    DOSX_FFN_ATTR2_L(false, 3); DOSX_FFN_ATTR2_L(true, 3); DOSX_FFN_ATTR2_L(false, 4); DOSX_FFN_ATTR2_L(true, 4);
+#undef DOSX_FFN_ATTR_L
+#undef DOSX_FFN_ATTR2_L
 #undef DOSX_FFN_ATTR
 #undef DOSX_FFN_ATTR2
     attr_set = true;
@@ -1433,13 +1492,29 @@
     else { if (pl.mode == 4) hipLaunchKernelGGL((KERNEL<false, 32, 4>), grid_, dim3(512), pl.smem, st_, ARG); else if (pl.mode == 3) hipLaunchKernelGGL((KERNEL<false, 32, 3>), grid_, dim3(512), pl.smem, st_, ARG); else if (pl.mode == 2) hipLaunchKernelGGL((KERNEL<false, 32, 2>), grid_, dim3(512), pl.smem, st_, ARG); else if (pl.mode == 1) hipLaunchKernelGGL((KERNEL<false, 32, 1>), grid_, dim3(512), pl.smem, st_, ARG); else hipLaunchKernelGGL((KERNEL<false, 32, 0>), grid_, dim3(512), pl.smem, st_, ARG); } \
   } while (0)
 
+#define DOSX_FFN_GO_LOSS(KERNEL, HALF_, ARG, MODE0)                                                                           \
+  do {                                                                                                                        \
+    const dim3 grid_(pl.grid);                                                                                                \
+    hipStream_t st_ = to_stream(stream);                                                                                      \
+    if (pl.mode == 4) hipLaunchKernelGGL((KERNEL<HALF_, 4>), grid_, dim3(512), pl.smem, st_, ARG);                  \
+    else if (pl.mode == 3) hipLaunchKernelGGL((KERNEL<HALF_, 3>), grid_, dim3(512), pl.smem, st_, ARG);             \
+    else if (pl.mode == 2) hipLaunchKernelGGL((KERNEL<HALF_, 2>), grid_, dim3(512), pl.smem, st_, ARG);             \
+    else if (pl.mode == 1) hipLaunchKernelGGL((KERNEL<HALF_, 1>), grid_, dim3(512), pl.smem, st_, ARG);             \
+    else hipLaunchKernelGGL((KERNEL<HALF_, (MODE0) ? 0 : 1>), grid_, dim3(512), pl.smem, st_, ARG);                 \
+  } while (0)
+
 extern "C" int dosx_ffn_fwd(const DosxFfn* ap, dosx_stream_t stream) {
   DOSX_CHECK_ARG(ap != nullptr, "dosx_ffn_fwd: null descriptor");
   const DosxFfn& a = *ap;
   if (a.M <= 0) return 0;
   FfnPlan pl;
   if (int rc = ffn_fwd_prepare(a, pl)) return rc;
-  DOSX_FFN_DISPATCH(ffn_fwd_kernel, a);
+  if (pl.loss) {
+    if (pl.half) DOSX_FFN_GO_LOSS(ffn_fwd_loss_kernel, true, a, true);
+    else DOSX_FFN_GO_LOSS(ffn_fwd_loss_kernel, false, a, true);
+  } else {
+    DOSX_FFN_DISPATCH(ffn_fwd_kernel, a);
+  }
   DOSX_LAUNCH_CHECK();
   return 0;
 }
@@ -1448,6 +1523,8 @@
   DOSX_CHECK_ARG(descs != nullptr && n >= 1 && n <= FFN_MULTI_MAX, "dosx_ffn_fwd_multi: 1 .. %d layers per launch", FFN_MULTI_MAX);
   if (descs[0].M <= 0) return 0;
   if (n == 1) return dosx_ffn_fwd(descs, stream);
+  for (int l = 0; l + 1 < n; ++l)
+    DOSX_CHECK_ARG(!ffn_has_loss(descs[l]), "dosx_ffn_fwd_multi: only the last layer may carry the loss block (layer %d of %d)", l, n);
   FfnMulti A;
   A.n = n;
   FfnPlan pl;
@@ -1458,6 +1535,7 @@
     DOSX_CHECK_ARG(p2.half == pl.half && p2.kb == pl.kb && p2.mode == pl.mode && p2.grid == pl.grid && p2.smem == pl.smem && descs[l].M == descs[0].M,
                    "dosx_ffn_fwd_multi: layer %d has another launch plan than layer 0", l);
     DOSX_CHECK_ARG(p2.mode != 0, "dosx_ffn_fwd_multi: every layer must carry its attention half (row-local layers only)");
+    pl.loss = p2.loss;
     if (l > 0) {
       const DosxFfn& p = descs[l - 1];
       const DosxFfn& c = descs[l];
@@ -1474,7 +1552,9 @@
          else if (pl.mode == 3) hipLaunchKernelGGL((ffn_fwd_multi_kernel<HALF_, KB_, 3>), grid_, dim3(512), pl.smem, st_, A); \
          else if (pl.mode == 2) hipLaunchKernelGGL((ffn_fwd_multi_kernel<HALF_, KB_, 2>), grid_, dim3(512), pl.smem, st_, A); \
          else hipLaunchKernelGGL((ffn_fwd_multi_kernel<HALF_, KB_, 1>), grid_, dim3(512), pl.smem, st_, A); } while (0)
-    if (pl.half && pl.kb == 64) DOSX_FFN_GO2(true, 64);
+    if (pl.loss && pl.half) DOSX_FFN_GO_LOSS(ffn_fwd_multi_loss_kernel, true, A, false);
+    else if (pl.loss) DOSX_FFN_GO_LOSS(ffn_fwd_multi_loss_kernel, false, A, false);
+    else if (pl.half && pl.kb == 64) DOSX_FFN_GO2(true, 64);
     else if (pl.half) DOSX_FFN_GO2(true, 32);
     else if (pl.kb == 64) DOSX_FFN_GO2(false, 64);
     else DOSX_FFN_GO2(false, 32);
diff --git a/dostransformer_amd/csrc/replay_thunks.inc b/dostransformer_amd/csrc/replay_thunks.inc
--- a/dostransformer_amd/csrc/replay_thunks.inc
+++ b/dostransformer_amd/csrc/replay_thunks.inc
@@ -55,6 +55,7 @@
 static int thunk_dosx_sum(const DosxCall& c) { return dosx_sum((const float*)(uintptr_t)c.iarg[0], (int)c.iarg[1], (float*)(uintptr_t)c.iarg[2], (dosx_stream_t)(uintptr_t)c.iarg[3]); }
 static int thunk_dosx_adamw(const DosxCall& c) { return dosx_adamw((float*)(uintptr_t)c.iarg[0], (const float*)(uintptr_t)c.iarg[1], (float*)(uintptr_t)c.iarg[2], (float*)(uintptr_t)c.iarg[3], (int64_t)c.iarg[4], (float)c.farg[0], (float)c.farg[1], (float)c.farg[2], (float)c.farg[3], (float)c.farg[4], (int)c.iarg[5], (float)c.farg[5], (dosx_stream_t)(uintptr_t)c.iarg[6]); }
 static int thunk_dosx_ffn_supported(const DosxCall& c) { return dosx_ffn_supported((int)c.iarg[0]); }
+static int thunk_dosx_ffn_loss_supported(const DosxCall& c) { return dosx_ffn_loss_supported((int)c.iarg[0]); }
 static int thunk_dosx_ffn_att_supported(const DosxCall& c) { return dosx_ffn_att_supported((int)c.iarg[0], (int)c.iarg[1]); }
 static int thunk_dosx_ffn_att_aligned_supported(const DosxCall& c) { return dosx_ffn_att_aligned_supported((int)c.iarg[0], (int)c.iarg[1]); }
 static int thunk_dosx_ffn_fwd(const DosxCall& c) { return dosx_ffn_fwd((const DosxFfn*)(uintptr_t)c.iarg[0], (dosx_stream_t)(uintptr_t)c.iarg[1]); }
@@ -175,6 +176,7 @@
   {"dosx_sum", thunk_dosx_sum, 4, 0},
   {"dosx_adamw", thunk_dosx_adamw, 7, 6},
   {"dosx_ffn_supported", thunk_dosx_ffn_supported, 1, 0},
+  {"dosx_ffn_loss_supported", thunk_dosx_ffn_loss_supported, 1, 0},
   {"dosx_ffn_att_supported", thunk_dosx_ffn_att_supported, 2, 0},
   {"dosx_ffn_att_aligned_supported", thunk_dosx_ffn_att_aligned_supported, 2, 0},
   {"dosx_ffn_fwd", thunk_dosx_ffn_fwd, 2, 0},
diff --git a/dostransformer_amd/csrc/rowops.hip b/dostransformer_amd/csrc/rowops.hip
--- a/dostransformer_amd/csrc/rowops.hip
+++ b/dostransformer_amd/csrc/rowops.hip
@@ -448,34 +448,9 @@
                                                                  const float* __restrict__ y, float* __restrict__ sse,
                                                                  float beta, float inv_count, float* __restrict__ dpg,
                                                                  float* __restrict__ dps, float* __restrict__ loss, int count) {
-  __shared__ float red[2][16];
+  __shared__ float red[2 * 16];
   __shared__ float tot[2];
-  float a = 0.f, b = 0.f;
-  for (int i = threadIdx.x; i < count; i += 1024) {
-    const float t = y[i], d0 = pg[i] - t, d1 = ps[i] - t;
-    a += d0 * d0;
-    b += d1 * d1;
-  }
-  a = wave_sum(a);
-  b = wave_sum(b);
-  const int lane = threadIdx.x & 63, wave = threadIdx.x >> 6;
-  if (lane == 0) { red[0][wave] = a; red[1][wave] = b; }
-  __syncthreads();
-  if (threadIdx.x == 0) {
-    float s0 = 0.f, s1 = 0.f;
-    for (int i = 0; i < 16; ++i) { s0 += red[0][i]; s1 += red[1][i]; }
-    tot[0] = s0; tot[1] = s1;
-    if (sse) { sse[0] = s0; sse[1] = s1; }
-  }
-  __syncthreads();
-  const float r0 = sqrtf(tot[0] * inv_count), r1 = sqrtf(tot[1] * inv_count);
-  const float k0 = inv_count / r0, k1 = beta * inv_count / r1;
-  if (threadIdx.x == 0 && loss) loss[0] = r0 + beta * r1;
-  for (int i = threadIdx.x; i < count; i += 1024) {
-    const float t = y[i];
-    dpg[i] = (pg[i] - t) * k0;
-    dps[i] = (ps[i] - t) * k1;
-  }
+  dosx_loss_phonon_body<1024, false>(pg, ps, y, sse, beta, inv_count, dpg, dps, loss, count, red, tot);
 }
 
 __global__ __launch_bounds__(256) void loss_edos_kernel(const float* __restrict__ pg, const float* __restrict__ ps,
diff --git a/dostransformer_amd/functional.py b/dostransformer_amd/functional.py
--- a/dostransformer_amd/functional.py
+++ b/dostransformer_amd/functional.py
@@ -65,6 +65,7 @@
 _FFN_MULTI = True
 _FUSED_FIN_BWD = True
 _FUSED_HEAD_FWD = True
+_LOSS_IN_LAST_FWD = True
 _FFN_BF16X3 = from_environ("DOSX_FFN_BF16X3", "0") == "1"
 
 _TAIL_SPLITS = 32
@@ -513,8 +514,12 @@
     return bool(ops.ffn_supported(H) and _FUSED_HEAD_FWD and T > 0)
 
 
+def loss_in_last_fwd(H: int, T: int) -> bool:
+    return bool(_LOSS_IN_LAST_FWD and H <= ops.ATTN_MAX_H and head_fused_fwd(H, T) and ops.ffn_loss_supported(H))
+
+
 def encoder_fwd(P: Params, pre: str, x: torch.Tensor, Sq: int, Bq: int, qs: int, qb: int, kvhat: torch.Tensor,
-                Nk: int, Bk: int, H: int, T: int, final_ln: bool = True, drop=None, head=None, fdrop=None, key_ptr=None):
+                Nk: int, Bk: int, H: int, T: int, final_ln: bool = True, drop=None, head=None, fdrop=None, key_ptr=None, loss=None):
     dev = kvhat.device
     rows = Sq * Bq
     lay = []
@@ -522,6 +527,7 @@
     if fdrop is not None and not (fdrop[0] > 0.0 or fdrop[1] > 0.0):
         fdrop = None
     assert fdrop is None or head is None
+    assert loss is None or (head is not None and loss_in_last_fwd(H, T))
     stack = [] if _FFN_MULTI else None
     for t in range(T):
         lp = f"{pre}.layers.{t}"
@@ -610,7 +616,8 @@
                                 qstats=qstats, x1=x1, st1=st1, mask=mask, aligned=att_aligned, key_ptr=key_ptr)
             ops.ffn_fwd(rows, H, x if att_fused else x1, None if att_fused else st1, P[lp + ".layer_norms.1.weight"],
                         P[lp + ".layer_norms.1.bias"], P[lp + ".fc1.weight"], P[lp + ".fc1.bias"], P[lp + ".fc2.weight"],
-                        P[lp + ".fc2.bias"], h, x2, fin=fin_args, att=att_args, defer=stack if att_fused else None)
+                        P[lp + ".fc2.bias"], h, x2, fin=fin_args, att=att_args, defer=stack if att_fused else None,
+                        loss=loss if (head is not None and t == T - 1) else None)
         else:
             def ffn_rows(r0, r1, x1=x1, st1=st1, h=h, x2=x2, lp=lp, xln=xln):
                 if xln is not None and _bf16x3_ok(r1 - r0, 4 * H, H):
@@ -1073,7 +1080,8 @@
     return seg(dcat, width=H, col=0) if K == 2 * H else None
 
 
-def dostransformer_fwd(P: Params, cfg: ModelCfg, g, m: GraphMeta, drop=None, per_crystal_keys: bool = False):
+def dostransformer_fwd(P: Params, cfg: ModelCfg, g, m: GraphMeta, drop=None, per_crystal_keys: bool = False, loss=None):
+    assert loss is None or loss_in_last_fwd(cfg.H, cfg.T)
     dr = (lambda base: None) if drop is None else (lambda base: (drop[0], drop[1], base))
     H, S, T, B, N = cfg.H, cfg.S, cfg.T, m.num_graphs, m.num_nodes
     if per_crystal_keys and H > ops.ATTN_MAX_H:
@@ -1131,7 +1139,8 @@
     gf, bf = P["transformer_source.layer_norm.weight"], P["transformer_source.layer_norm.bias"]
     if head_fused_fwd(H, T):
         _, c3 = encoder_fwd(P, "transformer_source", hs, S, 2 * B, 2 * B, 1, kvhat, nmax, B, H, T, final_ln=False,
-                            drop=dr(128), head=(gf, bf, P["out_layer.weight"], P["out_layer.bias"], xhat_f, rstd_f, dos), key_ptr=kp)
+                            drop=dr(128), head=(gf, bf, P["out_layer.weight"], P["out_layer.bias"], xhat_f, rstd_f, dos), key_ptr=kp,
+                            loss=loss)
     else:
         hsrc, c3 = encoder_fwd(P, "transformer_source", hs, S, 2 * B, 2 * B, 1, kvhat, nmax, B, H, T, final_ln=False,
                                drop=dr(128), key_ptr=kp)
diff --git a/dostransformer_amd/ops.py b/dostransformer_amd/ops.py
--- a/dostransformer_amd/ops.py
+++ b/dostransformer_amd/ops.py
@@ -374,6 +374,10 @@
     return bool(_lib.load().dosx_ffn_supported(int(H)))
 
 
+def ffn_loss_supported(H: int) -> bool:
+    return bool(_lib.load().dosx_ffn_loss_supported(int(H)))
+
+
 def ffn_att_supported(H: int, Nk: int) -> bool:
     return bool(_lib.load().dosx_ffn_att_supported(int(H), int(Nk)))
 
@@ -383,7 +387,7 @@
 
 
 def ffn_fwd(M: int, H: int, x: torch.Tensor, stats: Optional[torch.Tensor], gamma, beta, w1, b1, w2, b2, h: torch.Tensor,
-            out: torch.Tensor, fin=None, att=None, defer: Optional[list] = None) -> None:
+            out: torch.Tensor, fin=None, att=None, defer: Optional[list] = None, loss=None) -> None:
     a = Ffn()
     a.M, a.H = int(M), int(H)
     a.x, a.ldx = x.data_ptr(), int(x.stride(0))
@@ -409,6 +413,22 @@
         a.fin_gamma, a.fin_beta, a.fin_xhat, a.fin_rstd = (t.data_ptr() for t in fin[:4])
         if len(fin) > 4:
             a.fin_w, a.fin_b, a.fin_dos, a.fin_S, a.fin_Bq = fin[4].data_ptr(), fin[5].data_ptr(), fin[6].data_ptr(), int(fin[7]), int(fin[8])
+    if loss is not None:
+        if fin is None or len(fin) <= 4:
+            raise ValueError("ffn_fwd: loss needs the model head (fin with w, b, dos, S, Bq)")
+        n_dos = int(fin[7]) * int(fin[8])
+        want = dict(y=n_dos // 2, out=1, ddos=n_dos, sse=2)
+        for k, n in want.items():
+            t = loss.get(k)
+            if t is None and k == "sse":
+                continue
+            if t.dtype != torch.float32 or not t.is_contiguous() or t.device != x.device or t.numel() != n:
+                raise ValueError(f"ffn_fwd: loss['{k}'] must be {n} contiguous float32 values on {x.device}")
+        if fin[6].numel() != n_dos or not fin[6].is_contiguous():
+            raise ValueError("ffn_fwd: loss needs a contiguous dos [Bq, S]")
+        a.loss_y, a.loss_out, a.loss_ddos = loss["y"].data_ptr(), loss["out"].data_ptr(), loss["ddos"].data_ptr()
+        a.loss_sse, a.loss_beta = _p(loss.get("sse")), float(loss["beta"])
+        a.loss_cnt = COUNTERS.take(x.device, 1)
     if defer is not None:
         defer.append((a, 16.0 * M * H * H + 4.0 * M * nk_att * H))
         return
diff --git a/dostransformer_amd/train.py b/dostransformer_amd/train.py
--- a/dostransformer_amd/train.py
+++ b/dostransformer_amd/train.py
@@ -115,18 +115,33 @@
     def per_crystal_keys(self) -> bool:
         return self._per_crystal_keys
 
+    def _loss_form(self, B: int, n_global: int) -> str:
+        if self.kind != "phonon":
+            return "launch"
+        if self.dist is not None or int(n_global) != int(B):
+            return "two_phase"
+        cfg = self.model._cfg
+        return "in_fwd" if Fn.loss_in_last_fwd(cfg.H, cfg.T) else "launch"
+
     def _part_a(self, fp, g, m, st_n_global: Optional[int] = None):
         if st_n_global is None:
             st_n_global = m.num_graphs
         model, dev, cfg = self.model, fp.flat.device, self.model._cfg
         B, S = m.num_graphs, cfg.S
+        form = self._loss_form(B, int(st_n_global))
+        pre = {}
+        if self.kind == "phonon":
+            pre["y"] = Fn._f32(g.phdos).reshape(B, S)
+            pre["sse"] = Fn._empty(dev, 2)
+        lt = None
+        if form == "in_fwd":
+            pre["loss_fwd"] = (Fn._empty(dev, 2 * B, S), Fn._empty(dev, 1))
+            lt = dict(y=pre["y"], beta=self.beta, sse=pre["sse"], ddos=pre["loss_fwd"][0], out=pre["loss_fwd"][1])
         dg, xL, ds, (ctx, dos) = model._program_fwd(fp.P, g, m, bump_seed=False,
-                                                    per_crystal_keys=self._per_crystal_keys)
-        st = {"ctx": ctx, "dos": dos, "out": (dg, xL, ds), "B": B, "S": S}
+                                                    per_crystal_keys=self._per_crystal_keys, loss=lt)
+        st = {"ctx": ctx, "dos": dos, "out": (dg, xL, ds), "B": B, "S": S, **pre}
         if self.kind == "phonon":
-            st["y"] = Fn._f32(g.phdos).reshape(B, S)
-            st["sse"] = Fn._empty(dev, 2)
-            st["split_loss"] = self.dist is not None or int(st_n_global) != B
+            st["split_loss"] = form == "two_phase"
             if st["split_loss"]:
                 ops.sse2(dos[:B], dos[B:], st["y"], st["sse"], B * S)
         else:
@@ -136,8 +151,13 @@
     def _part_b(self, fp, m, st, n_global: int):
         dev, cfg = fp.flat.device, self.model._cfg
         B, S, dos = st["B"], st["S"], st["dos"]
-        ddos = Fn._empty(dev, *dos.shape)
-        if self.kind == "phonon":
+        if "loss_fwd" in st:
+            if int(n_global) != B:
+                raise RuntimeError("n_global differs between the two halves of the step")
+            ddos, loss = st["loss_fwd"]
+            loss = loss[0]
+        elif self.kind == "phonon":
+            ddos = Fn._empty(dev, *dos.shape)
             loss = Fn._empty(dev, 1)
             if st["split_loss"] or int(n_global) != B:
                 if not st["split_loss"]:
@@ -148,6 +168,7 @@
                 ops.loss_phonon(dos[:B], dos[B:], st["y"], st["sse"], self.beta, ddos[:B], ddos[B:], loss, B * S)
             loss = loss[0]
         else:
+            ddos = Fn._empty(dev, *dos.shape)
             lp = Fn._empty(dev, B + 1)
             ops.loss_edos(dos[:B], dos[B:], st["y"], self.beta, B, S, n_global, ddos[:B], ddos[B:], lp)
             ops.sum_to(lp, B, lp[B:])
diff --git a/include/dosx.h b/include/dosx.h
--- a/include/dosx.h
+++ b/include/dosx.h
@@ -280,8 +280,11 @@
   int32_t att_Nk, att_Bk, att_Bq, att_Sq, att_qs, att_qb, att_ldx1;
   int32_t att_aligned;
   const int32_t* att_key_ptr;
+  const float* loss_y; float* loss_sse; float* loss_out; float* loss_ddos; int32_t* loss_cnt;
+  float loss_beta;
 } DosxFfn;
 int dosx_ffn_supported(int H);
+int dosx_ffn_loss_supported(int H);
 int dosx_ffn_att_supported(int H, int Nk);
 int dosx_ffn_att_aligned_supported(int H, int Nk);
 int dosx_ffn_fwd(const DosxFfn* a, dosx_stream_t stream);
```

Result: no change. 61570 crystals/s (-0.7%).
